# PRADUMAN-KR/Multimodal-Lip-Sync-Deepfake-Detection-System

Hardware: NVIDIA B200
Metric: windows_per_sec (higher is better)
Workload: dtype bf16

## Files before the change

multimodal-lip-sync-deepfake-detection-system_b200/csrc/bf16_path.cu:

```cuda
#include "forward_common.h"
#include "tok_front.cuh"
#include "tok_fused.cuh"
#include "token_kernels.cuh"
#include "umma_conv.cuh"
#include "stem_ring.cuh"
#include "conv_ring.cuh"

#include <cuda_fp16.h>

#include <algorithm>
#include <cstdio>
#include <cstdlib>
#include <cstring>

using namespace lsd;
using namespace lsdfw;

#define LSD_ENV(name) ([]() -> const char* { static const char* const v_ = getenv(name); return v_; }())

namespace {

uint16_t f2bf(float f) {
  uint32_t u;
  memcpy(&u, &f, 4);
  if ((u & 0x7F800000u) == 0x7F800000u) return (uint16_t)(u >> 16);
  u += 0x7FFFu + ((u >> 16) & 1u);
  return (uint16_t)(u >> 16);
}

BGroup make_group(const ConvP& c, int sh, int sw, bool merge_kt = false) {
  BGroup g;
  g.Cin = c.Cin;
  for (int a = 0; a < c.kt; ++a)
    for (int b = 0; b < c.kh; ++b)
      for (int d = 0; d < c.kw; ++d) {
        BTap t;
        t.orig = (a * c.kh + b) * c.kw + d;
        t.dt = a - c.kt / 2;
        int hp = 0, wp = 0;
        const int oh = b - c.kh / 2, ow = d - c.kw / 2;
        if (sh == 2) { hp = oh & 1; t.dh = (oh - hp) / 2; } else t.dh = oh;
        if (sw == 2) { wp = ow & 1; t.dw = (ow - wp) / 2; } else t.dw = ow;
        const int set = hp * 2 + wp;
        BBand* band = nullptr;
        for (BBand& bb : g.bands)
          if (bb.set == set && (merge_kt || bb.taps[0].dt == t.dt) && (int)bb.taps.size() < UC_MAX_TAPS) band = &bb;
        if (!band) { g.bands.push_back(BBand{set, {}}); band = &g.bands.back(); }
        band->taps.push_back(t);
      }
  g.taps_total = c.kt * c.kh * c.kw;
  g.k16 = c.Cin / 16;
  return g;
}

BGroup make_group_toeplitz(const ConvP& c, int kpix, int dw_units) {
  BGroup g;
  g.Cin = c.Cin;
  g.toeplitz = 1;
  g.k16 = kpix * 4 / 16;
  for (int a = 0; a < c.kt; ++a)
    for (int b = 0; b < c.kh; ++b) {
      BTap t;
      t.orig = a * c.kh + b;
      t.dt = a - c.kt / 2;
      const int oh = b - c.kh / 2;
      const int hp = oh & 1;
      t.dh = (oh - hp) / 2;
      t.dw = dw_units;
      BBand* band = nullptr;
      for (BBand& bb : g.bands)
        if (bb.set == hp && bb.taps[0].dt == t.dt) band = &bb;
      if (!band) { g.bands.push_back(BBand{hp, {}}); band = &g.bands.back(); }
      band->taps.push_back(t);
    }
  g.taps_total = c.kt * c.kh;
  return g;
}

struct Packer {
  lsd_handle* h;
  const std::vector<float>& f32;
  std::vector<uint16_t> w;
  std::vector<float> bias;
  int ds_sh = 2, ds_sw = 2;
  void pack_group(BGroup& g, const ConvP& c, int ntile, int part = 0) {
    g.w_off = w.size();
    const int Cout = c.Cout;
    const float* W = &f32[c.w_off];
    const float* sc = c.has_scale ? &f32[c.scale_off] : nullptr;
    g.slice_stride = (size_t)(c.Cin / 16) * g.taps_total * ntile * 16;
    for (int sl = 0; sl < Cout / ntile; ++sl)
      for (int ch = 0; ch < c.Cin / 16; ++ch)
        for (const BBand& b : g.bands)
          for (const BTap& t : b.taps)
            for (int kc = 0; kc < 2; ++kc)
              for (int nn = 0; nn < ntile; ++nn)
                for (int e = 0; e < 8; ++e) {
                  const int ci = ch * 16 + kc * 8 + e, n = sl * ntile + nn;
                  const float v = W[((size_t)t.orig * c.Cin + ci) * Cout + n] * (sc ? sc[n] : 1.0f);
                  const uint16_t hi = f2bf(v);
                  if (part == 0) w.push_back(hi);
                  else { uint32_t u = (uint32_t)hi << 16; float hf; memcpy(&hf, &u, 4); w.push_back(f2bf(v - hf)); }
                }
  }
  void add_toeplitz(const std::string& name, const std::string& key, int kpix, int dw_units, bool dup_lo = false, bool halves = false) {
    const ConvP& c = h->convs.at(key);
    BLayer L;
    L.Cout = c.Cout;
    L.ntile = c.Cout;
    L.halves = halves;
    L.groups.push_back(make_group_toeplitz(c, kpix, dw_units));
    BGroup& g = L.groups[0];
    g.w_off = w.size();
    const float* W = &f32[c.w_off];
    const float* sc = c.has_scale ? &f32[c.scale_off] : nullptr;
    const int nsl = halves ? 2 : 1, ncol = c.Cout / nsl;
    g.slice_stride = (size_t)g.k16 * g.taps_total * ncol * 16;
    for (int sl = 0; sl < nsl; ++sl)
    for (int ch = 0; ch < g.k16; ++ch)
      for (const BBand& b : g.bands)
        for (const BTap& t : b.taps)
          for (int kc = 0; kc < 2; ++kc)
            for (int n = sl * ncol; n < (sl + 1) * ncol; ++n)
              for (int e = 0; e < 8; ++e) {
                const int k = ch * 16 + kc * 8 + e, j = k / 4, kw = j - 1;
                int ci = k % 4;
                const bool lo_part = dup_lo && ci == 2;
                if (dup_lo) ci = ci < 3 ? 0 : 99;
                float v = 0.f;
                if (ci < c.Cin && kw >= 0 && kw < c.kw) v = W[((size_t)(t.orig * c.kw + kw) * c.Cin + ci) * c.Cout + n] * (sc ? sc[n] : 1.0f);
                const uint16_t hi = f2bf(v);
                if (!lo_part) w.push_back(hi);
                else { uint32_t u = (uint32_t)hi << 16; float hf; memcpy(&hf, &u, 4); w.push_back(f2bf(v - hf)); }
              }
    L.bias_off = bias.size();
    for (int i = 0; i < c.Cout; ++i) bias.push_back(f32[c.shift_off + i]);
    while (w.size() % 64) w.push_back(0);
    h->blayers[name] = L;
  }
  void add(const std::string& name, const std::string& key, int sh, int sw, const std::string& ds_key = "", int ntile = 0, bool split = false,
           bool merge_kt = false, bool halves = false) {
    const ConvP& c = h->convs.at(key);
    BLayer L;
    L.Cout = c.Cout;
    L.ntile = ntile > 0 ? ntile : c.Cout;
    L.halves = halves;
    L.groups.push_back(make_group(c, sh, sw, merge_kt));
    pack_group(L.groups[0], c, halves ? L.ntile / 2 : L.ntile);
    if (split) {
      BGroup g1 = L.groups[0]; g1.src = 2;
      BGroup g2 = make_group(c, sh, sw, merge_kt);
      pack_group(g2, c, L.ntile, 1);
      L.groups.push_back(g1);
      L.groups.push_back(g2);
    }
    L.bias_off = bias.size();
    for (int i = 0; i < c.Cout; ++i) bias.push_back(f32[c.shift_off + i]);
    if (!ds_key.empty()) {
      const ConvP& d = h->convs.at(ds_key);
      const int sh_ds = ds_sh, sw_ds = ds_sw;
      BGroup gd = make_group(d, sh_ds, sw_ds);
      gd.src = 1;
      pack_group(gd, d, L.ntile);
      L.groups.push_back(gd);
      if (split) {
        BGroup g1 = gd; g1.src = 3;
        BGroup g2 = make_group(d, sh_ds, sw_ds); g2.src = 1;
        pack_group(g2, d, L.ntile, 1);
        L.groups.push_back(g1);
        L.groups.push_back(g2);
      }
      for (int i = 0; i < c.Cout; ++i) bias[L.bias_off + i] += f32[d.shift_off + i];
    }
    while (w.size() % 64) w.push_back(0);
    h->blayers[name] = L;
  }
  void add_split(const std::string& name, const std::string& key, int ntile) {
    const ConvP& c = h->convs.at(key);
    BLayer L;
    L.Cout = c.Cout;
    L.ntile = ntile;
    BGroup g0 = make_group(c, 1, 1);
    pack_group(g0, c, ntile, 0);
    BGroup g1 = g0; g1.src = 2;
    BGroup g2 = make_group(c, 1, 1);
    pack_group(g2, c, ntile, 1);
    L.groups = {g0, g1, g2};
    L.bias_off = bias.size();
    for (int i = 0; i < c.Cout; ++i) bias.push_back(f32[c.shift_off + i]);
    while (w.size() % 64) w.push_back(0);
    h->blayers[name] = L;
  }
};

struct PBuf {
  size_t off = 0;
  int C = 0, sets = 1;
  UcGeom g;
  int64_t plane_stride = 0, set_stride = 0, origin = 0;
  size_t bytes() const { return (size_t)sets * set_stride * 2; }
};

constexpr int TILE_MAX = 1024;

PBuf make_pbuf(int C, int sets, UcGeom g) {
  PBuf b;
  b.C = C; b.sets = sets; b.g = g;
  const int64_t gf = ((int64_t)g.SL + 3 * g.RW + 16 + 7) / 8 * 8;
  const int64_t gb = gf + TILE_MAX;
  const int64_t plane_pos = (gf + g.P_total + gb + 7) / 8 * 8;
  b.origin = gf * 8;
  b.plane_stride = plane_pos * 8;
  b.set_stride = b.plane_stride * (C / 8);
  return b;
}

struct BPlan {
  Shapes s;
  Plan f32;
  std::map<std::string, PBuf> pb;
  size_t planar_begin = 0, planar_end = 0;
  UcGeom gt, g33, gta;
  void addp(const char* name, int C, int sets, UcGeom g) {
    PBuf b = make_pbuf(C, sets, g);
    f32.cursor = (f32.cursor + 255) & ~size_t(255);
    b.off = f32.cursor;
    f32.cursor += b.bytes();
    pb[name] = b;
  }
};

void build_plan(const Shapes& s, BPlan& P) {
  P.s = s;
  Plan& p = P.f32;
  const int64_t B = s.B, T = s.T, TA = s.A4;
  p.add("vid", B * T * s.H * s.W * 3);
  p.add("aud", B * s.F * s.Ta);
  p.add("v_feat", B * T * 256);
  p.add("a_feat", B * TA * 256);
  p.add("v_emb", B * T * 256);
  p.add("a_emb", B * TA * 256);
  p.add("a_int", B * T * 256);
  p.add("proj_v", B * T * 768);
  p.add("proj_a", B * T * 768);
  p.add("vcomb", B * T * 1024);
  p.add("acomb", B * T * 1024);
  p.add("a_fint", B * T * 256);
  p.add("gate_in", B * T * 512);
  p.add("gate_h", B * T * 256);
  p.add("fused", B * T * 256);
  p.add("tok", B * (T + 1) * 256);
  p.add("tok_qkv", B * (T + 1) * 768);
  p.add("comb", B * 448);
  P.planar_begin = (p.cursor + 255) & ~size_t(255);
  const int Bn = s.B, Tn = s.T;
  const UcGeom g1 = make_geom(Bn, Tn, s.H1, s.W1), g2 = make_geom(Bn, Tn, s.H2, s.W2), g3 = make_geom(Bn, Tn, s.H3, s.W3),
               g4 = make_geom(Bn, Tn, s.H4, s.W4), gd = make_geom(Bn, s.Td, s.H4, s.W4), gh = make_geom(Bn, Tn, s.Hg, s.Wg);
  const UcGeom gs = make_geom_ex(Bn, Tn, s.Hs, s.Ws, 1, 2, 0, 0, 2);
  P.addp("xs", 8, 2, gs);
  P.addp("xl", 8, 2, gs);
  P.addp("s_out", 64, 1, gs);
  P.addp("x1", 64, 1, g1);
  P.addp("l1a", 64, 1, g1);
  P.addp("y1", 64, 4, g2);
  P.addp("l2a", 128, 1, g2);
  P.addp("y2", 128, 4, g3);
  P.addp("l3a", 256, 1, g3);
  P.addp("y3", 256, 4, g4);
  P.addp("l4a", 256, 1, g4);
  P.addp("y4", 256, 1, g4);
  P.addp("art_a", 128, 1, g4);
  P.addp("art_b", 64, 1, g4);
  P.addp("delta", 256, 1, gd);
  P.addp("artd_a", 128, 1, gd);
  P.addp("artd_b", 64, 1, gd);
  P.addp("hf_f", 32, 4, gh);
  P.addp("hf_b", 64, 1, gh);
  const UcGeom as = make_geom_ex(Bn, 1, s.Fs, s.As, 0, 2, 0, 0, 4);
  auto g2d = [&](int H, int W) { return make_geom_ex(Bn, 1, H, W, 0, 1, 0, 1, 0); };
  P.addp("xa", 8, 2, as);
  for (const char* sfx : {"", "_lo"}) {
    auto nm = [&](const char* n) { return std::string(n) + sfx; };
    P.addp(nm("sa_out").c_str(), 64, 1, as);
    P.addp(nm("a1").c_str(), 64, 1, g2d(s.F1, s.A1));
    P.addp(nm("a1a").c_str(), 64, 1, g2d(s.F1, s.A1));
    P.addp(nm("ya1").c_str(), 64, 4, g2d(s.F2, s.A2));
    P.addp(nm("a2a").c_str(), 128, 1, g2d(s.F2, s.A2));
    P.addp(nm("ya2").c_str(), 128, 4, g2d(s.F3, s.A3));
    P.addp(nm("a3a").c_str(), 256, 1, g2d(s.F3, s.A3));
    P.addp(nm("ya3").c_str(), 256, 4, g2d(s.F4, s.A4));
    P.addp(nm("a4a").c_str(), 256, 1, g2d(s.F4, s.A4));
    P.addp(nm("ya4").c_str(), 256, 1, g2d(s.F4, s.A4));
  }
  P.gt = make_geom_ex(Bn, 1, 1, Tn, 0, 0, 0, 3, 0);
  P.g33 = make_geom_rows(Bn * (Tn + 1));
  P.gta = make_geom_rows(Bn * (int)TA);
  for (const char* sfx : {"", "_lo"}) {
    auto nm = [&](const char* n) { return std::string(n) + sfx; };
    P.addp(nm("afeat_p").c_str(), 256, 1, P.gta);
    for (const char* n : {"vfeat_p", "vemb_p", "aint_p", "afint_p", "att1_p", "att2_p", "blend_p", "fused_p"}) P.addp(nm(n).c_str(), 256, 1, P.gt);
    P.addp(nm("gatein_p").c_str(), 512, 1, P.gt);
    P.addp(nm("mscat_p").c_str(), 768, 1, P.gt);
    P.addp(nm("tokln_p").c_str(), 256, 1, P.g33);
    P.addp(nm("tokatt_p").c_str(), 256, 1, P.g33);
    P.addp(nm("tokff_p").c_str(), 1024, 1, P.g33);
  }
  P.planar_end = p.cursor;
}

struct BCtx {
  lsd_handle* h;
  char* ws;
  const BPlan* P;
  cudaStream_t st;
  int max_ctas = 0;
  __nv_bfloat16* base(const PBuf& b) const { return reinterpret_cast<__nv_bfloat16*>(ws + b.off); }
  __nv_bfloat16* org(const PBuf& b) const { return base(b) + b.origin; }
  float* f(const char* name) const { return reinterpret_cast<float*>(ws + P->f32.find(name)); }
  const float* W(const char* key) const { return h->warena + h->vecs.at(key); }
};

struct UArgs {
  const PBuf* in = nullptr;
  const PBuf* in_ds = nullptr;
  const PBuf* in_lo = nullptr;
  const PBuf* in_ds_lo = nullptr;
  const PBuf* res_lo = nullptr;
  const PBuf* yp_lo = nullptr;
  UcGeom og;
  int act = ACT_NONE;
  const PBuf* yp = nullptr;
  int y_plane_off = 0;
  int y_mode = -1;
  const PBuf* res = nullptr;
  float* y32 = nullptr;
  int y32_ld = 0, y32_outer_stride = -1, y32_row_off = 0;
  const float* res32 = nullptr;
  int res32_ld = 0;
};

int run_umma(const BCtx& c, const std::string& name, const UArgs& a) {
  const BLayer& L = c.h->blayers.at(name);
  const UcGeom& og = a.og;
  if (og.P_total >= ((int64_t)1 << 31) - 1024) return lsd_fail(c.h, LSD_ERR_SHAPE, "%s: more than 2^31 padded positions in one launch (reduce the batch)", name.c_str());
  UmmaConvP p;
  memset(&p, 0, sizeof(p));
  p.w = reinterpret_cast<const __nv_bfloat16*>(c.h->barena);
  p.bias = c.h->bbias + L.bias_off;
  p.Cout = L.ntile;
  const int slices = L.Cout / L.ntile;
  p.act = a.act;
  p.g = og;
  p.cta2 = L.halves ? 1 : 0;
  if (a.y_mode == UC_Y_POOL && p.cta2) return lsd_fail(c.h, LSD_ERR_UNSUPPORTED, "%s: the fused max-pool does not run on CTA pairs (LSD_UMMA_CTA2=0)", name.c_str());
  if (a.yp) {
    p.y_mode = a.y_mode >= 0 ? a.y_mode : (a.yp->sets == 4 ? UC_Y_PARITY : UC_Y_PLAIN);
    p.y = c.org(*a.yp) + (int64_t)a.y_plane_off * a.yp->plane_stride;
    p.y_plane_stride = a.yp->plane_stride; p.y_set_stride = a.yp->set_stride;
    p.g2 = a.yp->g;
    if (a.yp_lo) p.ylo = c.org(*a.yp_lo) + (int64_t)a.y_plane_off * a.yp_lo->plane_stride;
  }
  if (a.y32) {
    p.y32 = a.y32; p.y32_ld = a.y32_ld;
    p.y32_outer_stride = a.y32_outer_stride >= 0 ? a.y32_outer_stride : og.W;
    p.y32_row_off = a.y32_row_off;
  }
  if (a.res) { p.res = c.org(*a.res); p.res_plane_stride = a.res->plane_stride; }
  if (a.res_lo) p.res_lo = c.org(*a.res_lo);
  if (a.res32) { p.res32 = a.res32; p.res32_ld = a.res32_ld; }
  const int mt_cap = L.ntile <= 32 ? 8 : 4;
  const int mt2 = std::max(1, std::min(mt_cap, 256 / L.ntile));
  p.MT = std::max(1, std::min(mt_cap, 512 / L.ntile));
  const int cta_budget = (c.max_ctas > 0 && c.max_ctas < c.h->num_sms) ? c.max_ctas : c.h->num_sms;
  while (p.MT > 1 && ((og.P_total + p.MT * 128 - 1) / (p.MT * 128)) * slices < cta_budget) p.MT /= 2;
  p.nbuf = (p.MT <= mt2 && 2 * p.MT * L.ntile <= 512) ? 2 : 1;
  if (const char* e = LSD_ENV("LSD_UMMA_NBUF")) {
    const int v = atoi(e);
    if (v == 1) p.nbuf = 1;
    if (v == 2 && 2 * L.ntile <= 512) { p.nbuf = 2; p.MT = std::min(p.MT, mt2); }
  }
  p.issuers = std::min(p.MT, 4);
  if (const char* e = LSD_ENV("LSD_UMMA_ISSUERS")) { const int v = atoi(e); if (v >= 1 && v <= 4 && v <= p.MT && p.MT % v == 0 && p.MT / v <= 4) p.issuers = v; }
  uint32_t cols = 32;
  while ((int)cols < p.nbuf * p.MT * L.ntile) cols *= 2;
  p.tmem_cols = cols;
  const int S = p.MT * 128;
  int nb = 0, max_a = 0, max_taps = 0, min_k16 = 1 << 30;
  bool any_toeplitz = false;
  p.ngroups = (int)L.groups.size();
  for (int gi = 0; gi < p.ngroups; ++gi) {
    const BGroup& G = L.groups[gi];
    const PBuf* srcp = G.src == 0 ? a.in : (G.src == 1 ? a.in_ds : (G.src == 2 ? a.in_lo : a.in_ds_lo));
    if (!srcp) return lsd_fail(c.h, LSD_ERR_ARG, "%s: missing input for group %d", name.c_str(), gi);
    const PBuf& src = *srcp;
    UcGroup& ug = p.groups[gi];
    ug.band_begin = nb;
    ug.k16 = G.k16;
    ug.taps_total = G.taps_total;
    ug.w_off = (int64_t)G.w_off;
    ug.slice_stride = (int64_t)G.slice_stride;
    int tap_begin = 0;
    int wkb = 40;
    if (const char* e = LSD_ENV("LSD_UMMA_WKB")) wkb = std::max(8, atoi(e));
    const int tmax = std::max(1, std::min(UC_MAX_TAPS, (wkb * 1024) / (L.ntile * 32)));
    for (const BBand& b : G.bands) {
      const int nt = (int)b.taps.size();
      const int pieces = (nt + tmax - 1) / tmax, per = (nt + pieces - 1) / pieces;
      for (int t0 = 0; t0 < nt; t0 += per) {
        const int t1 = std::min(nt, t0 + per);
        if (nb >= UC_MAX_BANDS) return lsd_fail(c.h, LSD_ERR_UNSUPPORTED, "%s: too many bands", name.c_str());
        UcBand& ub = p.bands[nb++];
        ub.base = c.org(src) + (int64_t)b.set * src.set_stride;
        ub.plane_stride = src.plane_stride;
        ub.toeplitz = G.toeplitz;
        ub.chunk_stride = G.toeplitz ? 16 : 2 * src.plane_stride;
        int mn = INT32_MAX, mx = INT32_MIN;
        for (int j = t0; j < t1; ++j) {
          const BTap& t = b.taps[j];
          const int sft = t.dt * og.SL + t.dh * og.RW + t.dw;
          mn = std::min(mn, sft); mx = std::max(mx, sft);
        }
        ub.start = mn;
        ub.len_extra = mx - mn;
        ub.ntaps = t1 - t0;
        ub.tap_begin = tap_begin;
        for (int j = t0; j < t1; ++j) ub.rel[j - t0] = b.taps[j].dt * og.SL + b.taps[j].dh * og.RW + b.taps[j].dw - mn;
        tap_begin += ub.ntaps;
        max_a = std::max(max_a, G.toeplitz ? (S + ub.len_extra + 1 + 2 * (G.k16 - 1)) * 16 : 2 * (S + ub.len_extra) * 16);
        max_taps = std::max(max_taps, ub.ntaps);
        min_k16 = std::min(min_k16, G.k16);
        any_toeplitz = any_toeplitz || G.toeplitz;
        if (-(int64_t)ub.start * 8 > src.origin || (int64_t)mx * 8 > src.origin)
          return lsd_fail(c.h, LSD_ERR_UNSUPPORTED, "%s: guard zone too small", name.c_str());
      }
    }
    ug.band_end = nb;
  }
  p.nbands = nb;
  const int w_chunk = max_taps * (L.halves ? L.ntile / 2 : L.ntile) * 32;
  if (any_toeplitz) p.kpack = min_k16;
  else {
    bool single_band = true;
    for (int gi = 0; gi < p.ngroups; ++gi) single_band = single_band && (p.groups[gi].band_end - p.groups[gi].band_begin) == 1;
    int stage_kb = single_band ? 64 : 24;
    if (const char* e = LSD_ENV("LSD_UMMA_STAGE_KB")) stage_kb = std::max(8, atoi(e));
    p.kpack = std::max(1, std::min(std::min(8, min_k16), (stage_kb * 1024) / (max_a + w_chunk)));
  }
  p.a_stage_bytes = ((uint32_t)(any_toeplitz ? max_a : max_a * p.kpack) + 127u) & ~127u;
  p.w_stage_bytes = (uint32_t)(w_chunk * p.kpack);
  const uint32_t stage = p.a_stage_bytes + p.w_stage_bytes;
  p.nst_tile = 0;
  for (int gi = 0; gi < p.ngroups; ++gi)
    p.nst_tile += ((p.groups[gi].k16 + p.kpack - 1) / p.kpack) * (p.groups[gi].band_end - p.groups[gi].band_begin);
  const uint32_t prog_bytes = (uint32_t)p.nst_tile * (uint32_t)umma_conv_stage_desc_bytes();
  uint32_t budget = 211u * 1024u;
  if (p.y_mode == UC_Y_POOL) {
    p.pool_ring = (uint32_t)(p.MT * 128 + 128);
    uc_magic(p.pool_ring, p.pool_mR, p.pool_sR);
  }
  const uint32_t pool_bytes = (uint32_t)umma_conv_extra_smem_bytes(p);
  budget -= pool_bytes;
  if (prog_bytes + 2 * stage > budget) return lsd_fail(c.h, LSD_ERR_UNSUPPORTED, "%s: stage program of %u bytes does not fit", name.c_str(), prog_bytes);
  int stages = (int)((budget - prog_bytes) / stage);
  stages = std::max(2, std::min(stages, 8));
  if ((size_t)stages * stage + prog_bytes + pool_bytes + 1024 > 223u * 1024u) return lsd_fail(c.h, LSD_ERR_UNSUPPORTED, "%s: stage of %u bytes does not fit", name.c_str(), stage);
  p.stages = stages;
  double kflop = 0;
  for (const BGroup& G : L.groups) kflop += (double)G.taps_total * G.Cin;
  if (L.groups[0].toeplitz) { const ConvP& cp = c.h->convs.at(name); kflop = (double)cp.kt * cp.kh * cp.kw * cp.Cin; }
  if (const char* e = getenv("LSD_UMMA_SKIP")) p.skip = atoi(e);
  if (const char* why = umma_conv_config_error(p)) return lsd_fail(c.h, LSD_ERR_UNSUPPORTED, "%s: %s", name.c_str(), why);
  {
    uint64_t hkey = 1469598103934665603ull;
    static_assert(sizeof(UmmaConvP) % 8 == 0, "UmmaConvP is hashed in 8-byte words");
    const uint64_t* pw = reinterpret_cast<const uint64_t*>(&p);
    for (size_t i = 0; i < sizeof(p) / 8; ++i) { hkey ^= pw[i]; hkey *= 1099511628211ull; hkey ^= hkey >> 29; }
    auto it = c.h->prog_cache.find(hkey);
    if (it == c.h->prog_cache.end()) {
      const size_t bytes = (size_t)p.nst_tile * sizeof(UcStageDesc);
      if (!c.h->prog_arena) {
        c.h->prog_cap = 16u << 20;
        if (cudaMalloc(&c.h->prog_arena, c.h->prog_cap) != cudaSuccess) return lsd_fail(c.h, LSD_ERR_CUDA, "stage-program arena allocation failed");
        c.h->prog_cursor = 0;
      }
      if (c.h->prog_cursor + bytes > c.h->prog_cap) {
        cudaDeviceSynchronize();
        c.h->prog_cache.clear();
        c.h->prog_cursor = 0;
        ++c.h->generation;
      }
      std::vector<UcStageDesc> host((size_t)p.nst_tile);
      umma_conv_build_program(p, host.data());
      char* dst = c.h->prog_arena + c.h->prog_cursor;
      cudaError_t e = cudaMemcpy(dst, host.data(), bytes, cudaMemcpyHostToDevice);
      if (e != cudaSuccess) return lsd_fail(c.h, LSD_ERR_CUDA, "%s: stage program upload: %s", name.c_str(), cudaGetErrorString(e));
      c.h->prog_cursor += (bytes + 255) & ~size_t(255);
      it = c.h->prog_cache.emplace(hkey, dst).first;
    }
    p.prog = reinterpret_cast<const UcStageDesc*>(it->second);
  }
  static const bool dyn_tiles = LSD_ENV("LSD_UMMA_DYNAMIC") != nullptr;
  if (dyn_tiles && p.y_mode != UC_Y_POOL && !p.cta2) {
    constexpr int kMaxLayers = 512;
    if (!c.h->tile_ctr_arena) {
      if (cudaMalloc(&c.h->tile_ctr_arena, kMaxLayers * 16 * sizeof(unsigned)) != cudaSuccess ||
          cudaMemset(c.h->tile_ctr_arena, 0, kMaxLayers * 16 * sizeof(unsigned)) != cudaSuccess)
        return lsd_fail(c.h, LSD_ERR_CUDA, "tile counter allocation failed");
    }
    auto it = c.h->tile_ctr_idx.find(name);
    if (it == c.h->tile_ctr_idx.end()) {
      if ((int)c.h->tile_ctr_idx.size() >= kMaxLayers) return lsd_fail(c.h, LSD_ERR_UNSUPPORTED, "too many tcgen05 layers");
      it = c.h->tile_ctr_idx.emplace(name, (int)c.h->tile_ctr_idx.size()).first;
    }
    p.tile_ctr = c.h->tile_ctr_arena + (size_t)it->second * 16;
  }
  if (const char* e = getenv("LSD_UMMA_TRACE")) {
    static long long* dbuf = nullptr;
    if (!dbuf) cudaMalloc(&dbuf, 512);
    cudaMemsetAsync(dbuf, 0, 512, c.st);
    p.dbg = dbuf;
    launch_umma_conv(p, slices, c.st, c.h->num_sms, c.max_ctas);
    long long hv[64];
    cudaMemcpyAsync(hv, dbuf, 512, cudaMemcpyDeviceToHost, c.st);
    cudaStreamSynchronize(c.st);
    if (atoi(e) > 0)
      fprintf(stderr, "[umma] %-34s MT=%d N=%d slices=%d stages=%d kpack=%d tiles=%lld | prologue %lld, first-data %lld, mma-issued %lld, acc-done %lld, epi-done %lld, total %lld cycles\n",
              name.c_str(), p.MT, p.Cout, slices, p.stages, p.kpack, hv[7], hv[1] - hv[0], hv[2] - hv[0], hv[3] - hv[0], hv[4] - hv[0], hv[5] - hv[0], hv[6] - hv[0]);
    if (atoi(e) > 1) {
      fprintf(stderr, "        full-wait done at:");
      for (int i = 0; i < 24 && hv[8 + i]; ++i) fprintf(stderr, " %lld", hv[8 + i] - hv[0]);
      fprintf(stderr, "\n        producer issue at:");
      for (int i = 0; i < 24 && hv[32 + i]; ++i) fprintf(stderr, " %lld", hv[32 + i] - hv[0]);
      fprintf(stderr, "\n        copies issued at: ");
      for (int i = 0; i < 8 && hv[56 + i]; ++i) fprintf(stderr, " %lld", hv[56 + i] - hv[0]);
      fprintf(stderr, "\n");
    }
    return 0;
  }
  c.h->prof.begin(c.st, 2.0 * (double)og.N * og.T * og.H * og.W * L.Cout * kflop, name.rfind("visual_encoder.", 0) == 0 ? 2 : 3);
  launch_umma_conv(p, slices, c.st, c.h->num_sms, c.max_ctas);
  c.h->prof.end(c.st);
  return 0;
}

int ring_table(const BCtx& c, const UcGeom& g, bool pool, const lsd_handle::RingTab** out) {
  lsd_handle* h = c.h;
  const void* pool_to = pool ? (const void*)&g : nullptr;
  const int T = g.T, CH = (g.SL + 127) / 128;
  const int64_t G = (int64_t)g.N * CH * T;
  const int budget = (c.max_ctas > 0 && c.max_ctas < h->num_sms) ? c.max_ctas : h->num_sms;
  uint64_t key = 1469598103934665603ull;
  for (uint64_t v : {(uint64_t)g.N, (uint64_t)T, (uint64_t)g.SL, (uint64_t)g.TS, (uint64_t)g.ot, (uint64_t)budget, (uint64_t)(pool_to != nullptr)}) { key ^= v; key *= 1099511628211ull; key ^= key >> 29; }
  auto it = h->ring_tabs.find(key);
  if (it == h->ring_tabs.end()) {
    int grid = budget;
    int64_t Lr = (G + 2 * (int64_t)grid - 1) / (2 * (int64_t)grid);
    if (Lr < 8) { Lr = 8; grid = (int)((G + 2 * Lr - 1) / (2 * Lr)); }
    if (grid < 1) grid = 1;
    std::vector<std::vector<SrStep>> lists((size_t)2 * grid);
    size_t nsteps = 0;
    const int nslots = 2 * grid;
    auto add_range = [&](int sg, int64_t col, int ta, int tb) {
      const int n = (int)(col / CH), sp = (int)(col % CH);
      const int t_first = std::max(ta - 1, 0);
      for (int t_in = t_first; t_in <= tb; ++t_in) {
        SrStep st;
        st.in_pos = (int32_t)(((int64_t)n * g.TS + t_in + g.ot) * g.SL + (int64_t)sp * 128);
        const int t_out = t_in - 1;
        st.flags = SR_ACTIVE | (t_in == t_first ? SR_FIRST : 0u) | ((t_out >= ta && t_out < tb) ? SR_STORE : 0u) |
                   ((uint32_t)std::min(128, g.SL - sp * 128) << 8);
        lists[sg].push_back(st);
      }
    };
    const int64_t ncols = (int64_t)g.N * CH;
    const int64_t rounds = pool_to ? ncols / nslots : 0;
    std::vector<int> col_round((size_t)ncols, 0);
    for (int64_t r = 0; r < rounds; ++r)
      for (int sg = 0; sg < nslots; ++sg) { add_range(sg, r * nslots + sg, 0, T); col_round[(size_t)(r * nslots + sg)] = (int)r; }
    {
      const int64_t col0 = rounds * nslots, Grem = (ncols - col0) * T;
      if (pool_to) Lr = (Grem + nslots - 1) / nslots;
      for (int64_t cc = col0; cc < ncols; ++cc) col_round[(size_t)cc] = (int)rounds;
      for (int sg = 0; sg < nslots && Lr > 0; ++sg) {
        int64_t g0 = (int64_t)sg * Lr;
        const int64_t g1 = std::min(Grem, g0 + Lr);
        while (g0 < g1) {
          const int64_t col = col0 + g0 / T;
          const int ta = (int)(g0 % T), tb = (int)std::min<int64_t>(T, ta + (g1 - g0));
          add_range(sg, col, ta, tb);
          g0 += tb - ta;
        }
      }
    }
    for (int sg = 0; sg < nslots; ++sg) nsteps = std::max(nsteps, lists[sg].size());
    std::vector<SrStep> flat((size_t)2 * grid * nsteps);
    memset(flat.data(), 0, flat.size() * sizeof(SrStep));
    for (int sg = 0; sg < 2 * grid; ++sg) std::copy(lists[sg].begin(), lists[sg].end(), flat.begin() + (size_t)sg * nsteps);
    lsd_handle::RingTab tab;
    tab.nsteps = (int)nsteps; tab.grid = grid;
    if (pool_to) {
      std::vector<std::pair<int64_t, int>> order;
      for (int n = 0; n < g.N; ++n) {
        int rmax = 0;
        for (int sp = 0; sp < CH; ++sp) rmax = std::max(rmax, col_round[(size_t)n * CH + sp]);
        for (int t = 0; t < T; ++t) order.push_back({(int64_t)rmax * (T + 1) + t, n * T + t});
      }
      std::stable_sort(order.begin(), order.end(), [](const std::pair<int64_t, int>& a, const std::pair<int64_t, int>& b) { return a.first < b.first; });
      tab.nfr = (int)((order.size() + grid - 1) / grid) + 1;
      std::vector<int> fl((size_t)grid * tab.nfr, -1);
      for (size_t i = 0; i < order.size(); ++i) fl[(i % grid) * tab.nfr + i / grid] = order[i].second;
      if (cudaMalloc(&tab.frames, fl.size() * sizeof(int)) != cudaSuccess ||
          cudaMemcpy(tab.frames, fl.data(), fl.size() * sizeof(int), cudaMemcpyHostToDevice) != cudaSuccess)
        return lsd_fail(h, LSD_ERR_CUDA, "stem: pool list upload failed");
    }
    if (cudaMalloc(&tab.dev, std::max<size_t>(flat.size(), 1) * sizeof(SrStep)) != cudaSuccess ||
        cudaMemcpy(tab.dev, flat.data(), flat.size() * sizeof(SrStep), cudaMemcpyHostToDevice) != cudaSuccess)
      return lsd_fail(h, LSD_ERR_CUDA, "stem: step table upload failed");
    it = h->ring_tabs.emplace(key, tab).first;
  }
  *out = &it->second;
  return 0;
}

int run_stem_ring(const BCtx& c, const PBuf& xs, const PBuf& so, const PBuf* pool_to = nullptr) {
  lsd_handle* h = c.h;
  const UcGeom& g = xs.g;
  if (g.P_total >= ((int64_t)1 << 31) - 4096) return lsd_fail(h, LSD_ERR_SHAPE, "stem: more than 2^31 padded positions in one launch (reduce the batch)");
  const BLayer& L = h->blayers.at("visual_encoder.stem");
  StemRingP p;
  memset(&p, 0, sizeof(p));
  p.xs[0] = c.org(xs);
  p.xs[1] = c.org(xs) + xs.set_stride;
  p.w = reinterpret_cast<const __nv_bfloat16*>(h->barena) + h->stem_ring_w_off;
  p.bias = h->bbias + L.bias_off;
  p.y = c.org(so);
  p.y_plane_stride = so.plane_stride;
  p.g = g;
  p.ntap[0] = 3; p.ntap[1] = 4;
  for (int t = 0; t < 4; ++t) { p.rel[0][t] = t * g.RW; p.rel[1][t] = t * g.RW; }
  p.start[0] = -g.RW; p.start[1] = -2 * g.RW;
  p.units[0] = 128 + 2 * g.RW + 3; p.units[1] = 128 + 3 * g.RW + 3;
  if ((int64_t)(2 * g.RW + 3) * 8 > xs.origin) return lsd_fail(h, LSD_ERR_UNSUPPORTED, "stem: guard zone too small");
  const int T = g.T, CH = (g.SL + 127) / 128;
  const lsd_handle::RingTab* tab = nullptr;
  if (int trc = ring_table(c, g, pool_to != nullptr, &tab)) return trc;
  p.steps = reinterpret_cast<const SrStep*>(tab->dev);
  p.nsteps = tab->nsteps;
  p.nst = 6;
  if (const char* e = getenv("LSD_SR_SKIP")) p.skip = atoi(e);
  if (pool_to) {
    const size_t need = (size_t)g.N * T;
    if (h->ring_cnt_cap < need) {
      if (h->ring_cnt) { cudaStreamSynchronize(c.st); cudaFree(h->ring_cnt); h->ring_cnt = nullptr; ++h->generation; }
      h->ring_cnt_cap = need * 2;
      if (cudaMalloc(&h->ring_cnt, h->ring_cnt_cap * sizeof(unsigned)) != cudaSuccess) { h->ring_cnt_cap = 0; return lsd_fail(h, LSD_ERR_CUDA, "stem: frame counter allocation failed"); }
    }
    cudaMemsetAsync(h->ring_cnt, 0, need * sizeof(unsigned), c.st);
    p.frame_cnt = h->ring_cnt;
    p.pool_frames = tab->frames;
    p.pool_nfr = tab->nfr;
    p.pool_expected = 4 * CH;
    p.yp = c.org(*pool_to);
    p.yp_plane_stride = pool_to->plane_stride;
    p.gp = pool_to->g;
  }
  while (p.nst > 3 && stem_ring_smem_bytes(p) > 223u * 1024u) --p.nst;
  if (stem_ring_smem_bytes(p) > 223u * 1024u) return lsd_fail(h, LSD_ERR_UNSUPPORTED, "stem: batch too large for the ring kernel (LSD_STEM_RING=0)");
  const ConvP& cp = h->convs.at("visual_encoder.stem");
  h->prof.begin(c.st, 2.0 * (double)g.N * g.T * g.H * g.W * 64.0 * (double)cp.kt * cp.kh * cp.kw * cp.Cin, 2);
  if (getenv("LSD_SR_TRACE")) {
    static long long* dbuf = nullptr;
    constexpr int kDbg = 256 + 4 * 160;
    if (!dbuf) cudaMalloc(&dbuf, kDbg * sizeof(long long));
    cudaMemsetAsync(dbuf, 0, kDbg * sizeof(long long), c.st);
    p.dbg = dbuf;
    launch_stem_ring(p, tab->grid, c.st);
    long long hv[kDbg];
    cudaMemcpyAsync(hv, dbuf, sizeof(hv), cudaMemcpyDeviceToHost, c.st);
    cudaStreamSynchronize(c.st);
    {
      long long g0 = INT64_MAX, g1 = 0, cmin = INT64_MAX, cmax = 0, csum = 0, smax = 0;
      const int nc = std::min(tab->grid, 160);
      for (int i = 0; i < nc; ++i) g0 = std::min(g0, hv[256 + 4 * i]);
      for (int i = 0; i < nc; ++i) {
        const long long* d = hv + 256 + 4 * i;
        g1 = std::max(g1, d[1]); smax = std::max(smax, d[0] - g0);
        const long long cy = d[3] - d[2];
        cmin = std::min(cmin, cy); cmax = std::max(cmax, cy); csum += cy;
      }
      fprintf(stderr, "[sr] %d CTAs x %d steps: kernel span %.1f us (globaltimer), latest CTA start +%.1f us, CTA cycles min %lld avg %lld max %lld\n", nc,
              p.nsteps, (g1 - g0) / 1e3, smax / 1e3, cmin, csum / nc, cmax);
    }
    const long long t0 = hv[0];
    for (int k = 0; k < 32; ++k)
      fprintf(stderr, "[sr] step %2d | prod free %7lld issued %7lld | mma landed %7lld blockfree %7lld issued %7lld | epi complete %7lld back %7lld\n", k + 16,
              hv[(0 * 32 + k) * 2] - t0, hv[(0 * 32 + k) * 2 + 1] - t0, hv[(1 * 32 + k) * 2] - t0, hv[(1 * 32 + k) * 2 + 1] - t0,
              hv[(2 * 32 + k) * 2] - t0, hv[(3 * 32 + k) * 2] - t0, hv[(3 * 32 + k) * 2 + 1] - t0);
    h->prof.end(c.st);
    return 0;
  }
  launch_stem_ring(p, tab->grid, c.st);
  h->prof.end(c.st);
  return 0;
}

int run_conv_ring(const BCtx& c, const std::string& name, int which, const PBuf& x, const PBuf& y, const PBuf* res) {
  lsd_handle* h = c.h;
  const UcGeom& g = x.g;
  if (g.P_total >= ((int64_t)1 << 31) - 4096) return lsd_fail(h, LSD_ERR_SHAPE, "%s: more than 2^31 padded positions in one launch (reduce the batch)", name.c_str());
  const BLayer& L = h->blayers.at(name);
  ConvRingP p;
  memset(&p, 0, sizeof(p));
  p.x = c.org(x);
  p.x_plane_stride = x.plane_stride;
  p.w = reinterpret_cast<const __nv_bfloat16*>(h->barena) + h->l1_ring_w_off[which];
  p.bias = h->bbias + L.bias_off;
  if (res) { p.res = c.org(*res); p.res_plane_stride = res->plane_stride; }
  p.y = c.org(y);
  p.y_plane_stride = y.plane_stride; p.y_set_stride = y.set_stride;
  p.y_mode = y.sets == 4 ? UC_Y_PARITY : UC_Y_PLAIN;
  p.g = g; p.g2 = y.g;
  p.start = -(g.RW + 1);
  p.units = 128 + 2 * g.RW + 2;
  if ((int64_t)(g.RW + 1) * 8 > x.origin) return lsd_fail(h, LSD_ERR_UNSUPPORTED, "%s: guard zone too small", name.c_str());
  const lsd_handle::RingTab* tab = nullptr;
  if (int trc = ring_table(c, g, false, &tab)) return trc;
  p.steps = reinterpret_cast<const SrStep*>(tab->dev);
  p.nsteps = tab->nsteps;
  p.nst = 4;
  if (const char* e = getenv("LSD_SR_SKIP")) p.skip = atoi(e);
  while (p.nst > 1 && conv_ring_smem_bytes(p) > 223u * 1024u) --p.nst;
  if (conv_ring_smem_bytes(p) > 223u * 1024u) return lsd_fail(h, LSD_ERR_UNSUPPORTED, "%s: rows too wide / batch too large for the ring kernel (LSD_L1_RING=0)", name.c_str());
  const ConvP& cp = h->convs.at(name);
  h->prof.begin(c.st, 2.0 * (double)g.N * g.T * g.H * g.W * 64.0 * (double)cp.kt * cp.kh * cp.kw * cp.Cin, 2);
  if (getenv("LSD_CR_TRACE")) {
    static long long* dbuf = nullptr;
    if (!dbuf) cudaMalloc(&dbuf, 4 * 160 * sizeof(long long));
    cudaMemsetAsync(dbuf, 0, 4 * 160 * sizeof(long long), c.st);
    p.dbg = dbuf;
    launch_conv_ring(p, tab->grid, c.st);
    long long hv[4 * 160];
    cudaMemcpyAsync(hv, dbuf, sizeof(hv), cudaMemcpyDeviceToHost, c.st);
    cudaStreamSynchronize(c.st);
    long long g0 = INT64_MAX, g1 = 0, cmin = INT64_MAX, cmax = 0, csum = 0;
    const int nc = std::min(tab->grid, 160);
    for (int i = 0; i < nc; ++i) g0 = std::min(g0, hv[4 * i]);
    for (int i = 0; i < nc; ++i) { g1 = std::max(g1, hv[4 * i + 1]); const long long cy = hv[4 * i + 3] - hv[4 * i + 2]; cmin = std::min(cmin, cy); cmax = std::max(cmax, cy); csum += cy; }
    fprintf(stderr, "[cr] %s: %d CTAs x %d steps (nst %d): kernel span %.1f us, CTA cycles min %lld avg %lld max %lld\n", name.c_str(), nc, p.nsteps, p.nst,
            (g1 - g0) / 1e3, cmin, csum / nc, cmax);
    h->prof.end(c.st);
    return 0;
  }
  launch_conv_ring(p, tab->grid, c.st);
  h->prof.end(c.st);
  return 0;
}

#define RUN(name, ...)                            \
  do {                                            \
    UArgs a_;                                     \
    __VA_ARGS__;                                  \
    if ((rc = run_umma(b, name, a_))) return rc;  \
  } while (0)

#define RUNC(ctx, name, ...)                        \
  do {                                              \
    UArgs a_;                                       \
    __VA_ARGS__;                                    \
    if ((rc = run_umma(ctx, name, a_))) return rc;  \
  } while (0)

#define RUNS(name, ...)                            \
  do {                                             \
    UArgs a_;                                      \
    __VA_ARGS__;                                   \
    if ((rc = run_umma(bs, name, a_))) return rc;  \
  } while (0)

PlanarOut pout(const BCtx& c, const PBuf& p, const PBuf* lo = nullptr, int plane_off = 0) {
  PlanarOut o;
  o.y = c.org(p) + (int64_t)plane_off * p.plane_stride;
  o.ylo = lo ? c.org(*lo) + (int64_t)plane_off * lo->plane_stride : nullptr;
  o.plane_stride = p.plane_stride;
  if (p.g.ow > 0 && p.g.HP == 1) { o.grp = p.g.W; o.grp_stride = p.g.RW; o.off = p.g.ow; }
  else { o.grp = 0; o.grp_stride = 0; o.off = 0; }
  return o;
}

int res_stage_umma(const BCtx& b, const std::string& p, const PBuf& x, const PBuf& mid, const PBuf& y, bool has_ds, int y_mode,
                   const PBuf* x_lo = nullptr, const PBuf* mid_lo = nullptr, const PBuf* y_lo = nullptr) {
  int rc = 0;
  RUN(p + ".conv1", a_.in = &x; a_.in_lo = x_lo; a_.og = mid.g; a_.act = ACT_RELU; a_.yp = &mid; a_.yp_lo = mid_lo);
  if (has_ds) RUN(p + ".conv2", a_.in = &mid; a_.in_lo = mid_lo; a_.in_ds = &x; a_.in_ds_lo = x_lo; a_.og = mid.g; a_.act = ACT_RELU;
                  a_.yp = &y; a_.yp_lo = y_lo; a_.y_mode = y_mode);
  else RUN(p + ".conv2", a_.in = &mid; a_.in_lo = mid_lo; a_.og = mid.g; a_.act = ACT_RELU; a_.yp = &y; a_.yp_lo = y_lo; a_.y_mode = y_mode;
           a_.res = &x; a_.res_lo = x_lo);
  return 0;
}

}

static int pack_tok_fused(lsd_handle* h, const std::vector<float>& f32) {
  std::vector<TfBlock> blocks;
  tf_layer_blocks(blocks);
  std::vector<uint32_t> stage_bytes;
  for (const TfBlock& b : blocks)
    for (int k0 = 0; k0 < b.k16; k0 += b.kps) stage_bytes.push_back((uint32_t)b.kps * (uint32_t)b.N * 32u);
  std::vector<__half> w;
  std::vector<float> vec((size_t)TF_LAYERS * TF_VEC_LAYER + (size_t)(2 * TF_LAYERS + 1) * TF_D, 0.f);
  std::vector<float> cum(TF_D, 0.f);
  float* cum_out = vec.data() + (size_t)TF_LAYERS * TF_VEC_LAYER;
  for (int l = 0; l < TF_LAYERS; ++l) {
    const std::string k = "t" + std::to_string(l);
    const ConvP &cin = h->convs.at(k + ".in"), &cout = h->convs.at(k + ".out"), &cf1 = h->convs.at(k + ".ff1"), &cf2 = h->convs.at(k + ".ff2");
    const size_t w0 = w.size();
    for (const TfBlock& b : blocks) {
      const ConvP& c = b.kind == 0 ? cin : (b.kind == 1 ? cout : (b.kind == 2 ? cf1 : cf2));
      for (int k16 = 0; k16 < b.k16; ++k16)
        for (int pl = 0; pl < 2; ++pl)
          for (int n = 0; n < b.N; ++n)
            for (int e = 0; e < 8; ++e) {
              const int kk = k16 * 16 + pl * 8 + e;
              int co, ci;
              if (b.kind == 0) { co = ((n % 96) / 32) * 256 + (2 * b.idx + n / 96) * 32 + (n % 32); ci = kk; }
              else if (b.kind == 1) { co = n; ci = 64 * b.idx + kk; }
              else if (b.kind == 2) { co = 128 * b.idx + n; ci = kk; }
              else { co = n; ci = 128 * b.idx + kk; }
              w.push_back(__float2half_rn(f32[c.w_off + (size_t)ci * c.Cout + co]));
            }
    }
    if (l == 0) h->tokf_layer_bytes = (uint32_t)((w.size() - w0) * sizeof(__half));
    float* lv = vec.data() + (size_t)l * TF_VEC_LAYER;
    const char* names[4] = {".ln1.w", ".ln1.b", ".ln2.w", ".ln2.b"};
    for (int i = 0; i < 4; ++i) memcpy(lv + 256 * i, &f32[h->vecs.at(k + names[i])], 256 * sizeof(float));
    for (int n = 0; n < 768; ++n) {
      const int hp = n / 192, r = n % 192;
      lv[1024 + n] = f32[cin.shift_off + ((r % 96) / 32) * 256 + (2 * hp + r / 96) * 32 + (r % 32)];
    }
    memcpy(lv + 1024 + 768, &f32[cf1.shift_off], 1024 * sizeof(float));
    memcpy(cum_out + (size_t)(2 * l) * TF_D, cum.data(), TF_D * sizeof(float));
    for (int i = 0; i < TF_D; ++i) cum[i] += f32[cout.shift_off + i];
    memcpy(cum_out + (size_t)(2 * l + 1) * TF_D, cum.data(), TF_D * sizeof(float));
    for (int i = 0; i < TF_D; ++i) cum[i] += f32[cf2.shift_off + i];
  }
  memcpy(cum_out + (size_t)(2 * TF_LAYERS) * TF_D, cum.data(), TF_D * sizeof(float));
  h->tokf_n_stage = (int)stage_bytes.size();
  for (void* q : {(void*)h->tokf_w, (void*)h->tokf_stage_bytes, (void*)h->tokf_vec}) if (q) cudaFree(q);
  h->tokf_w = nullptr; h->tokf_stage_bytes = nullptr; h->tokf_vec = nullptr;
  cudaError_t e = cudaMalloc(&h->tokf_w, w.size() * sizeof(__half));
  if (e == cudaSuccess) e = cudaMemcpy(h->tokf_w, w.data(), w.size() * sizeof(__half), cudaMemcpyHostToDevice);
  if (e == cudaSuccess) e = cudaMalloc(&h->tokf_stage_bytes, stage_bytes.size() * sizeof(uint32_t));
  if (e == cudaSuccess) e = cudaMemcpy(h->tokf_stage_bytes, stage_bytes.data(), stage_bytes.size() * sizeof(uint32_t), cudaMemcpyHostToDevice);
  if (e == cudaSuccess) e = cudaMalloc(&h->tokf_vec, vec.size() * sizeof(float));
  if (e == cudaSuccess) e = cudaMemcpy(h->tokf_vec, vec.data(), vec.size() * sizeof(float), cudaMemcpyHostToDevice);
  if (e != cudaSuccess) return lsd_fail(h, LSD_ERR_CUDA, "pack_tok_fused: %s", cudaGetErrorString(e));
  return 0;
}

static int pack_tok_front(lsd_handle* h, const std::vector<float>& f32) {
  std::vector<__half> w;
  w.reserve((size_t)TFR_K16_TOTAL * 16 * 256);
  auto emit = [&](int k16, auto&& get) {
    for (int k = 0; k < k16; ++k)
      for (int pl = 0; pl < 2; ++pl)
        for (int n = 0; n < 256; ++n)
          for (int e = 0; e < 8; ++e) w.push_back(__float2half_rn(get(k * 16 + pl * 8 + e, n)));
  };
  const ConvP &o0 = h->convs.at("cross.v2a.out"), &o1 = h->convs.at("cross.a2v.out"), &g0 = h->convs.at("cross.gate0"),
              &fu = h->convs.at("cross.fuse"), &pp = h->convs.at("temporal.pre_scale_proj");
  for (const ConvP* o : {&o0, &o1})
    for (int hp = 0; hp < 4; ++hp) emit(4, [&](int ci, int co) { return f32[o->w_off + (size_t)(64 * hp + ci) * 256 + co]; });
  emit(32, [&](int ci, int co) { return f32[g0.w_off + (size_t)ci * 256 + co]; });
  emit(16, [&](int ci, int co) { return f32[fu.w_off + (size_t)ci * 256 + co]; });
  const int ks[3] = {3, 5, 7};
  for (int b = 0; b < 3; ++b) {
    const ConvP& c = h->convs.at("temporal.branch_k" + std::to_string(ks[b]));
    for (int j = 0; j < ks[b]; ++j)
      emit(16, [&](int ci, int co) { return f32[c.w_off + ((size_t)j * 256 + ci) * 256 + co] * (c.has_scale ? f32[c.scale_off + co] : 1.0f); });
    emit(16, [&](int ci, int co) { return f32[pp.w_off + (size_t)(256 * b + ci) * 256 + co]; });
  }
  if (w.size() != (size_t)TFR_N_STAGES * TFR_STAGE_BYTES / sizeof(__half)) return lsd_fail(h, LSD_ERR_WEIGHTS, "pack_tok_front: stream size mismatch");
  std::vector<float> vec(TFR_V_TOTAL, 0.f);
  auto cp = [&](int dst, size_t src, int n) { memcpy(vec.data() + dst, &f32[src], (size_t)n * sizeof(float)); };
  cp(TFR_V_BO0, o0.shift_off, 256); cp(TFR_V_BO1, o1.shift_off, 256); cp(TFR_V_BG0, g0.shift_off, 256);
  cp(TFR_V_WG2, h->vecs.at("cross.gate2.w"), 256); cp(TFR_V_BG2, h->vecs.at("cross.gate2.b"), 1);
  cp(TFR_V_BF, fu.shift_off, 256);
  cp(TFR_V_SH3, h->convs.at("temporal.branch_k3").shift_off, 256); cp(TFR_V_SH5, h->convs.at("temporal.branch_k5").shift_off, 256);
  cp(TFR_V_SH7, h->convs.at("temporal.branch_k7").shift_off, 256);
  cp(TFR_V_BP, pp.shift_off, 256); cp(TFR_V_CLS, h->vecs.at("temporal.cls"), 256);
  for (void* q : {(void*)h->tokfr_w, (void*)h->tokfr_vec}) if (q) cudaFree(q);
  h->tokfr_w = nullptr; h->tokfr_vec = nullptr;
  cudaError_t e = cudaMalloc(&h->tokfr_w, w.size() * sizeof(__half));
  if (e == cudaSuccess) e = cudaMemcpy(h->tokfr_w, w.data(), w.size() * sizeof(__half), cudaMemcpyHostToDevice);
  if (e == cudaSuccess) e = cudaMalloc(&h->tokfr_vec, vec.size() * sizeof(float));
  if (e == cudaSuccess) e = cudaMemcpy(h->tokfr_vec, vec.data(), vec.size() * sizeof(float), cudaMemcpyHostToDevice);
  if (e != cudaSuccess) return lsd_fail(h, LSD_ERR_CUDA, "pack_tok_front: %s", cudaGetErrorString(e));
  return 0;
}

int pack_bf16_weights(lsd_handle* h, const std::vector<float>& f32_arena) {
  Packer P{h, f32_arena, {}, {}};
  memcpy(h->lapw_host, &f32_arena[h->convs.at("art.lap").w_off], sizeof(h->lapw_host));
  h->blayers.clear();
  const int vstr[4] = {1, 2, 2, 2};
  const bool cta2 = !(LSD_ENV("LSD_UMMA_CTA2") && atoi(LSD_ENV("LSD_UMMA_CTA2")) == 0);
  for (int l = 1; l <= 4; ++l) {
    const std::string p = "visual_encoder.layer" + std::to_string(l);
    const int s = vstr[l - 1];
    int nt = l >= 3 ? 128 : 0;
    if (const char* e = getenv(l == 3 ? "LSD_UMMA_NT3" : (l == 4 ? "LSD_UMMA_NT4" : "LSD_UMMA_NTX"))) nt = atoi(e);
    const bool pairs = cta2 && l == 1;
    P.add(p + ".conv1", p + ".conv1", s, s, "", nt, false, l >= 2, pairs);
    P.ds_sh = 2; P.ds_sw = 2;
    P.add(p + ".conv2", p + ".conv2", 1, 1, l == 1 ? "" : p + ".downsample", nt, false, false, pairs);
  }
  P.add_toeplitz("visual_encoder.stem", "visual_encoder.stem", 8, 0, false, cta2);
  for (int cv = 0; cv < 2; ++cv) {
    const ConvP& c = h->convs.at(cv == 0 ? "visual_encoder.layer1.conv1" : "visual_encoder.layer1.conv2");
    h->l1_ring_w_off[cv] = 0;
    if (c.kt != 3 || c.kh != 3 || c.kw != 3 || c.Cin != 64 || c.Cout != 64) continue;
    h->l1_ring_w_off[cv] = P.w.size();
    const float* W = &f32_arena[c.w_off];
    const float* sc = c.has_scale ? &f32_arena[c.scale_off] : nullptr;
    for (int ch = 0; ch < 4; ++ch)
      for (int b = 0; b < 3; ++b)
        for (int d = 0; d < 3; ++d)
          for (int kc = 0; kc < 2; ++kc)
            for (int n = 0; n < 192; ++n)
              for (int e = 0; e < 8; ++e) {
                const int ci = ch * 16 + kc * 8 + e, a = n / 64, co = n % 64;
                P.w.push_back(f2bf(W[((size_t)((a * 3 + b) * 3 + d) * 64 + ci) * 64 + co] * (sc ? sc[co] : 1.0f)));
              }
    while (P.w.size() % 64) P.w.push_back(0);
  }
  {
    const ConvP& c = h->convs.at("visual_encoder.stem");
    h->stem_ring_w_off = 0;
    if (c.kt == 3 && c.kh == 7 && c.kw == 7 && c.Cin == 3 && c.Cout == 64) {
      h->stem_ring_w_off = P.w.size();
      const float* W = &f32_arena[c.w_off];
      const float* sc = c.has_scale ? &f32_arena[c.scale_off] : nullptr;
      for (int set = 0; set < 2; ++set)
        for (int b = 0; b < 7; ++b) {
          if (((b - 3) & 1) != set) continue;
          for (int ch = 0; ch < 2; ++ch)
            for (int kc = 0; kc < 2; ++kc)
              for (int n = 0; n < 192; ++n)
                for (int e = 0; e < 8; ++e) {
                  const int k = ch * 16 + kc * 8 + e, j = k / 4, kw = j - 1, ci = k % 4, a = n / 64, co = n % 64;
                  float v = 0.f;
                  if (ci < 3 && kw >= 0 && kw < 7) v = W[((size_t)((a * 7 + b) * 7 + kw) * 3 + ci) * 64 + co] * (sc ? sc[co] : 1.0f);
                  P.w.push_back(f2bf(v));
                }
        }
      while (P.w.size() % 64) P.w.push_back(0);
    }
  }
  P.add_toeplitz("art.hf0", "art.hf0", 4, 1);
  P.add("art.td0", "art.td0", 1, 1);
  P.add("art.td3", "art.td3", 1, 1);
  P.add("art.hf3", "art.hf3", 2, 2);
  P.add_toeplitz("audio_encoder.stem", "audio_encoder.stem", 8, 0, true);
  const int ash[4] = {1, 2, 2, 2}, asw[4] = {1, 2, 1, 1};
  for (int l = 1; l <= 4; ++l) {
    const std::string p = "audio_encoder.layer" + std::to_string(l);
    P.add(p + ".conv1", p + ".conv1", ash[l - 1], asw[l - 1], "", 0, true);
    P.ds_sh = ash[l - 1]; P.ds_sw = asw[l - 1];
    P.add(p + ".conv2", p + ".conv2", 1, 1, l == 1 ? "" : p + ".downsample", 0, true);
  }
  int wide = 128;
  if (const char* e = LSD_ENV("LSD_UMMA_NTW")) wide = atoi(e);
  int narrow = 64;
  if (const char* e = LSD_ENV("LSD_UMMA_NTN")) narrow = atoi(e);
  for (const char* k : {"projection.visual_proj", "projection.audio_proj", "cross.v2a.out", "cross.a2v.out",
                        "cross.gate0", "cross.fuse", "temporal.branch_k3", "temporal.branch_k5", "temporal.branch_k7",
                        "temporal.pre_scale_proj"})
    P.add_split(k, k, narrow);
  for (const char* k : {"cross.in_v", "cross.in_a", "cross.vcomb", "cross.acomb"}) P.add_split(k, k, wide);
  for (int l = 0; l < 4; ++l)
    for (const char* k : {".in", ".out", ".ff1", ".ff2"})
      P.add_split("t" + std::to_string(l) + k, "t" + std::to_string(l) + k, (k[1] == 'i' || (k[1] == 'f' && k[3] == '1')) ? wide : narrow);
  if (h->barena) { cudaFree(h->barena); h->barena = nullptr; }
  if (h->bbias) { cudaFree(h->bbias); h->bbias = nullptr; }
  cudaError_t e = cudaMalloc(&h->barena, P.w.size() * 2);
  if (e == cudaSuccess) e = cudaMemcpy(h->barena, P.w.data(), P.w.size() * 2, cudaMemcpyHostToDevice);
  if (e == cudaSuccess) e = cudaMalloc(&h->bbias, P.bias.size() * 4);
  if (e == cudaSuccess) e = cudaMemcpy(h->bbias, P.bias.data(), P.bias.size() * 4, cudaMemcpyHostToDevice);
  if (e != cudaSuccess) return lsd_fail(h, LSD_ERR_CUDA, "pack_bf16_weights: %s", cudaGetErrorString(e));
  if (int rc = pack_tok_fused(h, f32_arena)) return rc;
  return pack_tok_front(h, f32_arena);
}

void make_plan_bf16(lsd_handle* h, int B, int T, int H, int W, int F, int Ta, std::vector<Stage>& stages, size_t& bytes) {
  Shapes s;
  if (make_shapes(h, B, T, H, W, F, Ta, s) != 0) { bytes = 0; return; }
  BPlan P;
  build_plan(s, P);
  stages = P.f32.stages;
  bytes = P.f32.cursor;
}

struct Timeline {
  bool on = false;
  std::vector<std::pair<std::string, cudaEvent_t>> marks;
  void mark(cudaStream_t st, const char* name) {
    if (!on) return;
    cudaEvent_t e; cudaEventCreate(&e); cudaEventRecord(e, st);
    marks.emplace_back(name, e);
  }
  void dump() {
    if (!on || marks.empty()) return;
    cudaDeviceSynchronize();
    fprintf(stderr, "[timeline]");
    for (auto& m : marks) { float ms = 0; cudaEventElapsedTime(&ms, marks[0].second, m.second); fprintf(stderr, " %s=%.0f", m.first.c_str(), ms * 1000.0f); }
    fprintf(stderr, " (us)\n");
    for (auto& m : marks) cudaEventDestroy(m.second);
    marks.clear();
  }
};
static Timeline g_tl;

static int audio_encoder_bf16(const BCtx& b, const Shapes& s, bool inputs_ready, const void* audio, int adt) {
  const BPlan& P = *b.P;
  auto pbf = [&](const char* n) -> const PBuf& { return P.pb.at(n); };
  cudaStream_t st = b.st;
  int rc = 0;
  const PBuf &xa = pbf("xa"), &sao = pbf("sa_out"), &a1 = pbf("a1");
  if (inputs_ready) launch_audio_rows(b.f("aud"), LSD_F32, b.org(xa), xa.set_stride, xa.g, s.F, s.Ta, st);
  else launch_audio_rows(audio, adt, b.org(xa), xa.set_stride, xa.g, s.F, s.Ta, st);
  RUN("audio_encoder.stem", a_.in = &xa; a_.og = xa.g; a_.act = ACT_RELU; a_.yp = &sao; a_.yp_lo = &pbf("sa_out_lo"));
  launch_planar_maxpool(b.org(sao), sao.plane_stride, sao.g, b.org(a1), a1.plane_stride, a1.g, 64, st, b.org(pbf("sa_out_lo")), b.org(pbf("a1_lo")));
  if ((rc = res_stage_umma(b, "audio_encoder.layer1", a1, pbf("a1a"), pbf("ya1"), false, UC_Y_PARITY, &pbf("a1_lo"), &pbf("a1a_lo"), &pbf("ya1_lo")))) return rc;
  if ((rc = res_stage_umma(b, "audio_encoder.layer2", pbf("ya1"), pbf("a2a"), pbf("ya2"), true, UC_Y_PARITY_H, &pbf("ya1_lo"), &pbf("a2a_lo"), &pbf("ya2_lo")))) return rc;
  if ((rc = res_stage_umma(b, "audio_encoder.layer3", pbf("ya2"), pbf("a3a"), pbf("ya3"), true, UC_Y_PARITY_H, &pbf("ya2_lo"), &pbf("a3a_lo"), &pbf("ya3_lo")))) return rc;
  if ((rc = res_stage_umma(b, "audio_encoder.layer4", pbf("ya3"), pbf("a4a"), pbf("ya4"), true, UC_Y_PLAIN, &pbf("ya3_lo"), &pbf("a4a_lo"), &pbf("ya4_lo")))) return rc;
  const PBuf& ya4 = pbf("ya4");
  launch_planar_mean2(b.org(ya4), ya4.plane_stride, ya4.g, 256, b.f("a_feat"), 256, 2, pout(b, pbf("afeat_p"), &pbf("afeat_p_lo")), st,
                      b.org(pbf("ya4_lo")));
  return 0;
}

static bool token_front_enabled(int T) {
  const char* e = getenv("LSD_TOK_FRONT");
  return !(e && atoi(e) == 0) && tok_front_supported(T);
}
static int token_path_bf16(const BCtx& b, const Shapes& s, bool combined = false) {
  const BPlan& P = *b.P;
  auto pbf = [&](const char* n) -> const PBuf& { return P.pb.at(n); };
  cudaStream_t st = b.st;
  const int B = s.B, T = s.T, TA = s.A4, NT = T + 1;
  const UcGeom gt = P.gt;
  int rc = 0;
  lsd_handle* h = b.h;
  const bool par = LSD_ENV("LSD_TOK_SERIAL") == nullptr;
  if (par && !h->tok_stream[0]) {
    for (int i = 0; i < 2; ++i)
      if (cudaStreamCreateWithFlags(&h->tok_stream[i], cudaStreamNonBlocking) != cudaSuccess ||
          cudaEventCreateWithFlags(&h->ev_tok_join[i], cudaEventDisableTiming) != cudaSuccess)
        return lsd_fail(h, LSD_ERR_CUDA, "token helper stream creation failed");
    if (cudaEventCreateWithFlags(&h->ev_tok_fork, cudaEventDisableTiming) != cudaSuccess) return lsd_fail(h, LSD_ERR_CUDA, "token helper event creation failed");
  }
  BCtx b1 = b, b2 = b;
  if (par) { b1.st = h->tok_stream[0]; b2.st = h->tok_stream[1]; }
  auto fork = [&](int n) { if (par) { cudaEventRecord(h->ev_tok_fork, st); for (int i = 0; i < n; ++i) cudaStreamWaitEvent(h->tok_stream[i], h->ev_tok_fork, 0); } };
  auto join = [&](int n) { if (par) for (int i = 0; i < n; ++i) { cudaEventRecord(h->ev_tok_join[i], h->tok_stream[i]); cudaStreamWaitEvent(st, h->ev_tok_join[i], 0); } };
  float *pv = b.f("proj_v"), *pa = b.f("proj_a"), *gi = b.f("gate_in");
  if (!combined) {
    fork(1);
    launch_lerp_tokens_p(b.f("a_emb"), b.f("a_int"), B, TA, T, 256, pout(b, pbf("aint_p"), &pbf("aint_p_lo")), b1.st);
    RUNC(b1, "cross.in_a", a_.in = &pbf("aint_p"); a_.in_lo = &pbf("aint_p_lo"); a_.og = gt; a_.y32 = pa; a_.y32_ld = 768);
    RUN("cross.in_v", a_.in = &pbf("vemb_p"); a_.in_lo = &pbf("vemb_p_lo"); a_.og = gt; a_.y32 = pv; a_.y32_ld = 768);
    join(1);
  }
  g_tl.mark(st, "T:inproj");
  float* tok = b.f("tok");
  if (token_front_enabled(T)) {
    TokFrontP fp;
    memset(&fp, 0, sizeof(fp));
    if (combined) {
      fp.v_emb = b.f("vcomb"); fp.pv = fp.v_emb + 256; fp.a_int = b.f("acomb"); fp.pa = fp.a_int + 256;
      fp.ld_e = 1024; fp.ld_p = 1024;
    } else {
      fp.pv = pv; fp.pa = pa; fp.v_emb = b.f("v_emb"); fp.a_int = b.f("a_int");
      fp.ld_e = 256; fp.ld_p = 768;
    }
    fp.gi = gi; fp.fused = b.f("fused"); fp.tok = tok;
    fp.w = reinterpret_cast<const __half*>(h->tokfr_w);
    fp.vec = h->tokfr_vec;
    fp.B = B; fp.T = T;
    tok_front_geometry(T, fp.SL, fp.G, fp.KW);
    if (getenv("LSD_TOKF_TRACE")) {
      static long long* dbuf = nullptr;
      if (!dbuf) cudaMalloc(&dbuf, 256 * sizeof(long long));
      cudaMemsetAsync(dbuf, 0, 256 * sizeof(long long), st);
      fp.dbg = dbuf;
      launch_tok_front(fp, st);
      std::vector<long long> hv(256);
      cudaMemcpyAsync(hv.data(), dbuf, 256 * sizeof(long long), cudaMemcpyDeviceToHost, st);
      cudaStreamSynchronize(st);
      const long long t0 = hv[128];
      fprintf(stderr, "[tokfront] compute (start=0) then (hand-over, next arrival):");
      for (int i = 0; i < 63 && hv[128 + 2 * i + 1]; ++i) fprintf(stderr, " (%lld,%lld)", hv[128 + 2 * i + 1] - t0, hv[128 + 2 * i + 2] ? hv[128 + 2 * i + 2] - t0 : 0);
      fprintf(stderr, "\n[tokfront] mma phases (start, issue-end):");
      for (int i = 0; i < 64 && hv[2 * i + 1]; ++i) fprintf(stderr, " (%lld,%lld)", hv[2 * i] - t0, hv[2 * i + 1] - t0);
      fprintf(stderr, "\n");
      fp.dbg = nullptr;
    } else
    launch_tok_front(fp, st);
    g_tl.mark(st, "T:cross");
  } else {
  fork(1);
  launch_mha_core_p(pv, 768, pa + 256, 768, pa + 512, 768, B, T, T, 8, pout(b, pbf("att1_p"), &pbf("att1_p_lo")), st);
  RUN("cross.v2a.out", a_.in = &pbf("att1_p"); a_.in_lo = &pbf("att1_p_lo"); a_.og = gt; a_.res32 = b.f("v_emb"); a_.res32_ld = 256; a_.y32 = gi; a_.y32_ld = 512;
      a_.yp = &pbf("gatein_p"); a_.yp_lo = &pbf("gatein_p_lo"));
  launch_mha_core_p(pa, 768, pv + 256, 768, pv + 512, 768, B, T, T, 8, pout(b, pbf("att2_p"), &pbf("att2_p_lo")), b1.st);
  RUNC(b1, "cross.a2v.out", a_.in = &pbf("att2_p"); a_.in_lo = &pbf("att2_p_lo"); a_.og = gt; a_.res32 = b.f("a_int"); a_.res32_ld = 256; a_.y32 = gi + 256; a_.y32_ld = 512;
      a_.yp = &pbf("gatein_p"); a_.yp_lo = &pbf("gatein_p_lo"); a_.y_plane_off = 32);
  join(1);
  RUN("cross.gate0", a_.in = &pbf("gatein_p"); a_.in_lo = &pbf("gatein_p_lo"); a_.og = gt; a_.act = ACT_GELU; a_.y32 = b.f("gate_h"); a_.y32_ld = 256);
  launch_gate_blend_p(b.f("gate_h"), b.W("cross.gate2.w"), b.W("cross.gate2.b"), gi, 512, gi + 256, 512, B * T, 256, pout(b, pbf("blend_p"), &pbf("blend_p_lo")), st);
  RUN("cross.fuse", a_.in = &pbf("blend_p"); a_.in_lo = &pbf("blend_p_lo"); a_.og = gt; a_.act = ACT_RELU; a_.y32 = b.f("fused"); a_.y32_ld = 256; a_.yp = &pbf("fused_p"); a_.yp_lo = &pbf("fused_p_lo"));
  g_tl.mark(st, "T:cross");
  fork(2);
  RUNC(b1, "temporal.branch_k5", a_.in = &pbf("fused_p"); a_.in_lo = &pbf("fused_p_lo"); a_.og = gt; a_.act = ACT_GELU; a_.yp = &pbf("mscat_p"); a_.yp_lo = &pbf("mscat_p_lo"); a_.y_plane_off = 32);
  RUNC(b2, "temporal.branch_k3", a_.in = &pbf("fused_p"); a_.in_lo = &pbf("fused_p_lo"); a_.og = gt; a_.act = ACT_GELU; a_.yp = &pbf("mscat_p"); a_.yp_lo = &pbf("mscat_p_lo"); a_.y_plane_off = 0);
  launch_set_cls(b.W("temporal.cls"), tok, B, NT, 256, b2.st);
  RUN("temporal.branch_k7", a_.in = &pbf("fused_p"); a_.in_lo = &pbf("fused_p_lo"); a_.og = gt; a_.act = ACT_GELU; a_.yp = &pbf("mscat_p"); a_.yp_lo = &pbf("mscat_p_lo"); a_.y_plane_off = 64);
  join(2);
  RUN("temporal.pre_scale_proj", a_.in = &pbf("mscat_p"); a_.in_lo = &pbf("mscat_p_lo"); a_.og = gt; a_.res32 = b.f("fused"); a_.res32_ld = 256; a_.y32 = tok; a_.y32_ld = 256;
      a_.y32_outer_stride = NT; a_.y32_row_off = 1);
  }
  const char* fused_env = getenv("LSD_TOK_FUSED");
  const bool fused_off = fused_env && atoi(fused_env) == 0;
  if (!fused_off && tok_fused_supported(NT)) {
    TokFusedP fp;
    memset(&fp, 0, sizeof(fp));
    fp.tok = tok;
    fp.w = reinterpret_cast<const __half*>(h->tokf_w);
    fp.stage_bytes = h->tokf_stage_bytes;
    fp.n_stage_layer = h->tokf_n_stage;
    fp.layer_bytes = h->tokf_layer_bytes;
    fp.vec = h->tokf_vec;
    fp.B = B; fp.NT = NT;
    tok_fused_geometry(NT, fp.SL, fp.G, fp.KW);
    if (getenv("LSD_TOKF_TRACE")) {
      static long long* dbuf = nullptr;
      if (!dbuf) cudaMalloc(&dbuf, 384 * sizeof(long long));
      cudaMemsetAsync(dbuf, 0, 384 * sizeof(long long), st);
      fp.dbg = dbuf;
      launch_tok_fused(fp, st);
      std::vector<long long> hv(384);
      cudaMemcpyAsync(hv.data(), dbuf, 384 * sizeof(long long), cudaMemcpyDeviceToHost, st);
      cudaStreamSynchronize(st);
      const long long t0 = hv[192];
      fprintf(stderr, "[tokf] compute phases (wait-return, hand-over) cycles from start:");
      for (int i = 0; i < 96 && hv[192 + 2 * i + 1]; ++i) fprintf(stderr, " (%lld,%lld)", hv[192 + 2 * i] - t0, hv[192 + 2 * i + 1] - t0);
      fprintf(stderr, "\n[tokf] mma phases (start, issue-end):");
      for (int i = 0; i < 96 && hv[2 * i + 1]; ++i) fprintf(stderr, " (%lld,%lld)", hv[2 * i] - t0, hv[2 * i + 1] - t0);
      fprintf(stderr, "\n");
      return 0;
    }
    launch_tok_fused(fp, st);
    return 0;
  }
  const UcGeom g33 = P.g33;
  for (int l = 0; l < 4; ++l) {
    const std::string k = "t" + std::to_string(l);
    launch_layernorm_p(tok, 256, b.W((k + ".ln1.w").c_str()), b.W((k + ".ln1.b").c_str()), B * NT, 256, pout(b, pbf("tokln_p"), &pbf("tokln_p_lo")), st);
    RUN(k + ".in", a_.in = &pbf("tokln_p"); a_.in_lo = &pbf("tokln_p_lo"); a_.og = g33; a_.y32 = b.f("tok_qkv"); a_.y32_ld = 768);
    const float* qkv = b.f("tok_qkv");
    launch_mha_core_p(qkv, 768, qkv + 256, 768, qkv + 512, 768, B, NT, NT, 8, pout(b, pbf("tokatt_p"), &pbf("tokatt_p_lo")), st);
    RUN(k + ".out", a_.in = &pbf("tokatt_p"); a_.in_lo = &pbf("tokatt_p_lo"); a_.og = g33; a_.res32 = tok; a_.res32_ld = 256; a_.y32 = tok; a_.y32_ld = 256);
    launch_layernorm_p(tok, 256, b.W((k + ".ln2.w").c_str()), b.W((k + ".ln2.b").c_str()), B * NT, 256, pout(b, pbf("tokln_p"), &pbf("tokln_p_lo")), st);
    RUN(k + ".ff1", a_.in = &pbf("tokln_p"); a_.in_lo = &pbf("tokln_p_lo"); a_.og = g33; a_.act = ACT_GELU; a_.yp = &pbf("tokff_p"); a_.yp_lo = &pbf("tokff_p_lo"));
    RUN(k + ".ff2", a_.in = &pbf("tokff_p"); a_.in_lo = &pbf("tokff_p_lo"); a_.og = g33; a_.res32 = tok; a_.res32_ld = 256; a_.y32 = tok; a_.y32_ld = 256);
  }
  return 0;
}


static int ws_prepare(lsd_handle* h, const Shapes& s, const BPlan& P, char* ws, size_t ws_bytes, cudaStream_t st, int slot) {
  const int sig[6] = {s.B, s.T, s.H, s.W, s.F, s.Ta};
  WsSig& mine = h->ws_sig[slot];
  WsSig& other = h->ws_sig[slot ^ 1];
  if (other.ptr) {
    const char* o0 = reinterpret_cast<const char*>(other.ptr);
    if (o0 < ws + ws_bytes && ws < o0 + other.bytes) other.ptr = nullptr;
  }
  if (mine.ptr == ws && mine.bytes == ws_bytes && memcmp(mine.shape, sig, sizeof(sig)) == 0) return 0;
  cudaError_t e = cudaMemsetAsync(ws + P.planar_begin, 0, P.planar_end - P.planar_begin, st);
  if (e != cudaSuccess) return lsd_fail(h, LSD_ERR_CUDA, "workspace init: %s", cudaGetErrorString(e));
  mine.ptr = ws; mine.bytes = ws_bytes; memcpy(mine.shape, sig, sizeof(sig));
  return 0;
}

static int forward_bf16_impl(lsd_handle* h, const Shapes& s, float* logits, const lsd_aux* aux, char* ws, size_t ws_bytes,
                             cudaStream_t st, bool inputs_ready, const void* video, int vdt, int vlayout, const void* audio, int adt,
                             const int32_t* vstarts = nullptr, int n_frames = 0, int pipe_parity = -1) {
  BPlan P;
  build_plan(s, P);
  if (P.f32.cursor > ws_bytes) return lsd_fail(h, LSD_ERR_WORKSPACE, "workspace too small: need %zu bytes, got %zu", P.f32.cursor, ws_bytes);
  h->stages = P.f32.stages;
  h->planar_stages.clear();
  for (const auto& kv : P.pb) {
    const PBuf& b = kv.second;
    PlanarStage ps;
    ps.off = b.off; ps.C = b.C; ps.sets = b.sets; ps.plane_stride = b.plane_stride; ps.set_stride = b.set_stride; ps.origin = b.origin;
    ps.N = b.g.N; ps.T = b.g.T; ps.H = b.g.H; ps.W = b.g.W; ps.ot = b.g.ot; ps.oh = b.g.oh; ps.hp_extra = b.g.HP - b.g.H - b.g.oh;
    ps.ow = b.g.ow; ps.wp_extra = b.g.RW - b.g.W - b.g.ow;
    h->planar_stages[kv.first] = ps;
  }
  int rc0 = 0;
  if ((rc0 = ws_prepare(h, s, P, ws, ws_bytes, st, pipe_parity == 1 ? 1 : 0))) return rc0;
  BCtx b{h, ws, &P, st};
  const int B = s.B, T = s.T, TA = s.A4, NT = T + 1;
  auto& pb = P.pb;
  int rc = 0;
  if (!h->side_stream) {
    if (cudaStreamCreateWithFlags(&h->side_stream, cudaStreamNonBlocking) != cudaSuccess || cudaEventCreateWithFlags(&h->ev_fork, cudaEventDisableTiming) != cudaSuccess ||
        cudaEventCreateWithFlags(&h->ev_join, cudaEventDisableTiming) != cudaSuccess || cudaEventCreateWithFlags(&h->ev_start, cudaEventDisableTiming) != cudaSuccess ||
        cudaEventCreateWithFlags(&h->ev_audio, cudaEventDisableTiming) != cudaSuccess)
      return lsd_fail(h, LSD_ERR_CUDA, "side stream creation failed");
  }
  cudaStream_t sst = h->side_stream;
  BCtx bs{h, ws, &P, sst};
  bs.max_ctas = h->num_sms / 2;
  if (const char* e = LSD_ENV("LSD_SIDE_CTAS")) bs.max_ctas = atoi(e);
  int art_ctas = bs.max_ctas;
  if (const char* e = LSD_ENV("LSD_ART_CTAS")) art_ctas = atoi(e);
  if (const char* e = LSD_ENV("LSD_MAIN_CTAS")) { b.max_ctas = atoi(e); bs.max_ctas = h->num_sms - b.max_ctas; }
  const bool audio_early = LSD_ENV("LSD_AUDIO_LATE") == nullptr;
  const bool tcomb = token_front_enabled(T);
  auto audio_tokens = [&](const BCtx& c) -> int {
    int rc = 0;
    launch_lerp_tokens_p(c.f("a_feat"), c.f("a_fint"), B, TA, T, 256, pout(c, pb["afint_p"], &pb["afint_p_lo"]), c.st);
    RUNC(c, "cross.acomb", a_.in = &pb["afint_p"]; a_.in_lo = &pb["afint_p_lo"]; a_.og = P.gt; a_.y32 = c.f("acomb"); a_.y32_ld = 1024);
    if (aux && aux->audio_tokens) RUNC(c, "projection.audio_proj", a_.in = &pb["afeat_p"]; a_.in_lo = &pb["afeat_p_lo"]; a_.og = P.gta; a_.y32 = c.f("a_emb"); a_.y32_ld = 256);
    return 0;
  };
  g_tl.on = LSD_ENV("LSD_TIMELINE") != nullptr;
  g_tl.mark(st, "start");
  const bool audio_after_rows = LSD_ENV("LSD_AUDIO_AFTER_ROWS") && atoi(LSD_ENV("LSD_AUDIO_AFTER_ROWS")) != 0;
  if (audio_early && !audio_after_rows) {
    cudaEventRecord(h->ev_start, st);
    cudaStreamWaitEvent(sst, h->ev_start, 0);
    if ((rc = audio_encoder_bf16(bs, s, inputs_ready, audio, adt))) return rc;
    if (tcomb && (rc = audio_tokens(bs))) return rc;
    g_tl.mark(sst, "S:audio_enc");
    cudaEventRecord(h->ev_audio, sst);
  }
  const PBuf &xs = pb["xs"], &xl = pb["xl"], &so = pb["s_out"], &x1 = pb["x1"];
  const float* lapw = h->warena + h->convs.at("art.lap").w_off;
  if (vstarts) launch_video_rows(video, vdt, vlayout, lapw, h->lapw_host, b.org(xs), b.org(xl), xs.set_stride, xs.g, s.H, s.W, st, h->num_sms, vstarts, n_frames);
  else if (inputs_ready) launch_video_rows(b.f("vid"), LSD_F32, LSD_NDHWC, lapw, h->lapw_host, b.org(xs), b.org(xl), xs.set_stride, xs.g, s.H, s.W, st, h->num_sms);
  else launch_video_rows(video, vdt, vlayout, lapw, h->lapw_host, b.org(xs), b.org(xl), xs.set_stride, xs.g, s.H, s.W, st, h->num_sms);
  g_tl.mark(st, "M:video_rows");
  if (audio_early && audio_after_rows) {
    cudaEventRecord(h->ev_start, st);
    cudaStreamWaitEvent(sst, h->ev_start, 0);
    if ((rc = audio_encoder_bf16(bs, s, inputs_ready, audio, adt))) return rc;
    if (tcomb && (rc = audio_tokens(bs))) return rc;
    g_tl.mark(sst, "S:audio_enc");
    cudaEventRecord(h->ev_audio, sst);
  }
  const bool hf_early = LSD_ENV("LSD_HF_EARLY") != nullptr;
  float* comb = b.f("comb");
  PlanarOut none{nullptr, nullptr, 0, 0, 0, 0};
  const PBuf& hf = pb["hf_f"];
  if (hf_early) {
    cudaEventRecord(h->ev_fork, st);
    cudaStreamWaitEvent(sst, h->ev_fork, 0);
    RUNS("art.hf0", a_.in = &xl; a_.og = xl.g; a_.act = ACT_RELU; a_.yp = &hf);
    RUNS("art.hf3", a_.in = &hf; a_.og = hf.g; a_.act = ACT_RELU; a_.yp = &pb["hf_b"]);
    launch_planar_mean2(bs.org(pb["hf_b"]), pb["hf_b"].plane_stride, hf.g, 64, comb + 384, 448, 1, none, sst);
    g_tl.mark(sst, "S:hf3");
  }
  {
    int chunk = 0;
    if (const char* e = LSD_ENV("LSD_STEM_CHUNK")) chunk = atoi(e);
    static const bool fuse_env = LSD_ENV("LSD_STEM_POOL_FUSE") && atoi(LSD_ENV("LSD_STEM_POOL_FUSE")) != 0;
    const bool fuse_pool = fuse_env && !h->blayers.at("visual_encoder.stem").halves && !(xs.g.H & 1) && !(xs.g.W & 1) && x1.g.H * 2 == xs.g.H && x1.g.W * 2 == xs.g.W && 2 * xs.g.RW + 2 <= 128;
    static const bool ring_env = !(LSD_ENV("LSD_STEM_RING") && atoi(LSD_ENV("LSD_STEM_RING")) == 0);
    const bool ring = ring_env && h->stem_ring_w_off != 0 && !fuse_env && (chunk <= 0 || chunk >= B) && 128 + 3 * xs.g.RW + 3 <= 640;
    static const bool pool_inline = LSD_ENV("LSD_STEM_POOL_INLINE") && atoi(LSD_ENV("LSD_STEM_POOL_INLINE")) != 0;
    if (ring && pool_inline && x1.g.H * 2 == xs.g.H && x1.g.W * 2 == xs.g.W) {
      if ((rc = run_stem_ring(b, xs, so, &x1))) return rc;
      g_tl.mark(st, "M:stem");
    } else if (ring) {
      if ((rc = run_stem_ring(b, xs, so))) return rc;
      g_tl.mark(st, "M:stem");
      launch_planar_maxpool(b.org(so), so.plane_stride, so.g, b.org(x1), x1.plane_stride, x1.g, 64, st);
    } else if (fuse_pool && (chunk <= 0 || chunk >= B)) {
      RUN("visual_encoder.stem", a_.in = &xs; a_.og = xs.g; a_.act = ACT_RELU; a_.yp = &x1; a_.y_mode = UC_Y_POOL);
      g_tl.mark(st, "M:stem");
    } else if (chunk <= 0 || chunk >= B) {
      RUN("visual_encoder.stem", a_.in = &xs; a_.og = xs.g; a_.act = ACT_RELU; a_.yp = &so);
      g_tl.mark(st, "M:stem");
      launch_planar_maxpool(b.org(so), so.plane_stride, so.g, b.org(x1), x1.plane_stride, x1.g, 64, st);
    } else {
      auto view = [&](const PBuf& full, int n0, int nb) {
        PBuf v = full;
        v.g = make_geom_ex(nb, full.g.T, full.g.H, full.g.W, full.g.ot, full.g.oh, full.g.HP - full.g.H - full.g.oh, full.g.ow,
                           full.g.RW - full.g.W - full.g.ow);
        v.origin = full.origin + (int64_t)n0 * full.g.TS * full.g.SL * 8;
        return v;
      };
      for (int n0 = 0; n0 < B; n0 += chunk) {
        const int nb = std::min(chunk, B - n0);
        const PBuf xs_v = view(xs, n0, nb), so_v = view(so, n0, nb), x1_v = view(x1, n0, nb);
        RUN("visual_encoder.stem", a_.in = &xs_v; a_.og = xs_v.g; a_.act = ACT_RELU; a_.yp = &so_v);
        launch_planar_maxpool(b.org(so_v), so_v.plane_stride, so_v.g, b.org(x1_v), x1_v.plane_stride, x1_v.g, 64, st);
      }
      g_tl.mark(st, "M:stem");
    }
  }
  g_tl.mark(st, "M:maxpool");
  {
    static const bool l1_ring = LSD_ENV("LSD_L1_RING") && atoi(LSD_ENV("LSD_L1_RING")) != 0;
    if (l1_ring && h->l1_ring_w_off[0] && h->l1_ring_w_off[1] && 128 + 2 * x1.g.RW + 2 <= 512) {
      if ((rc = run_conv_ring(b, "visual_encoder.layer1.conv1", 0, x1, pb["l1a"], nullptr))) return rc;
      if ((rc = run_conv_ring(b, "visual_encoder.layer1.conv2", 1, pb["l1a"], pb["y1"], &x1))) return rc;
    } else if ((rc = res_stage_umma(b, "visual_encoder.layer1", x1, pb["l1a"], pb["y1"], false, UC_Y_PARITY))) return rc;
  }
  g_tl.mark(st, "M:layer1");
  if ((rc = res_stage_umma(b, "visual_encoder.layer2", pb["y1"], pb["l2a"], pb["y2"], true, UC_Y_PARITY))) return rc;
  g_tl.mark(st, "M:layer2");
  if ((rc = res_stage_umma(b, "visual_encoder.layer3", pb["y2"], pb["l3a"], pb["y3"], true, UC_Y_PARITY))) return rc;
  g_tl.mark(st, "M:layer3");
  if ((rc = res_stage_umma(b, "visual_encoder.layer4", pb["y3"], pb["l4a"], pb["y4"], true, UC_Y_PLAIN))) return rc;
  g_tl.mark(st, "M:layer4");
  b.max_ctas = 0;
  const PBuf& y4 = pb["y4"];
  launch_planar_mean2(b.org(y4), y4.plane_stride, y4.g, 256, b.f("v_feat"), 256, 0, pout(b, pb["vfeat_p"], &pb["vfeat_p_lo"]), st);
  cudaEventRecord(h->ev_fork, st);
  cudaStreamWaitEvent(sst, h->ev_fork, 0);
  const bool skip_art = LSD_ENV("LSD_SKIP_ART") != nullptr;
  bs.max_ctas = art_ctas;
  if (!skip_art) {
  RUNS("art.td0", a_.in = &y4; a_.og = y4.g; a_.act = ACT_RELU; a_.yp = &pb["art_a"]);
  RUNS("art.td3", a_.in = &pb["art_a"]; a_.og = y4.g; a_.act = ACT_RELU; a_.yp = &pb["art_b"]);
  launch_planar_mean2(bs.org(pb["art_b"]), pb["art_b"].plane_stride, y4.g, 64, comb + 256, 448, 1, none, sst);
  g_tl.mark(sst, "S:td_feat");
  const PBuf& dl = pb["delta"];
  if (T > 1) launch_planar_delta(bs.org(y4), y4.plane_stride, y4.g, bs.org(dl), dl.plane_stride, dl.g, 256, sst);
  RUNS("art.td0", a_.in = &dl; a_.og = dl.g; a_.act = ACT_RELU; a_.yp = &pb["artd_a"]);
  RUNS("art.td3", a_.in = &pb["artd_a"]; a_.og = dl.g; a_.act = ACT_RELU; a_.yp = &pb["artd_b"]);
  launch_planar_mean2(bs.org(pb["artd_b"]), pb["artd_b"].plane_stride, dl.g, 64, comb + 320, 448, 1, none, sst);
  g_tl.mark(sst, "S:td_delta");
  if (!hf_early) {
    const bool hf_par = LSD_ENV("LSD_HF_SERIAL") == nullptr;
    cudaStream_t hst = sst;
    if (hf_par) {
      if (!h->side2_stream) {
        if (cudaStreamCreateWithFlags(&h->side2_stream, cudaStreamNonBlocking) != cudaSuccess || cudaEventCreateWithFlags(&h->ev_join2, cudaEventDisableTiming) != cudaSuccess)
          return lsd_fail(h, LSD_ERR_CUDA, "second side stream creation failed");
      }
      hst = h->side2_stream;
      cudaStreamWaitEvent(hst, h->ev_fork, 0);
    }
    BCtx bh = bs;
    bh.st = hst;
    if (const char* e = LSD_ENV("LSD_HF_CTAS")) bh.max_ctas = atoi(e);
    RUNC(bh, "art.hf0", a_.in = &xl; a_.og = xl.g; a_.act = ACT_RELU; a_.yp = &hf);
    g_tl.mark(hst, "S:hf0");
    RUNC(bh, "art.hf3", a_.in = &hf; a_.og = hf.g; a_.act = ACT_RELU; a_.yp = &pb["hf_b"]);
    launch_planar_mean2(bh.org(pb["hf_b"]), pb["hf_b"].plane_stride, hf.g, 64, comb + 384, 448, 1, none, hst);
    g_tl.mark(hst, "S:hf3");
    if (hf_par) {
      cudaEventRecord(h->ev_join2, hst);
      cudaStreamWaitEvent(sst, h->ev_join2, 0);
    }
  }
  }
  cudaEventRecord(h->ev_join, sst);
  cudaStream_t tst = st;
  if (pipe_parity >= 0) {
    cudaEventRecord(h->ev_front[pipe_parity], st);
    cudaStreamWaitEvent(h->tail_stream, h->ev_front[pipe_parity], 0);
    tst = h->tail_stream;
  }
  {
  BCtx b{h, ws, &P, tst};
  cudaStream_t st = tst;
  if (!audio_early) { if ((rc = audio_encoder_bf16(b, s, inputs_ready, audio, adt))) return rc; }
  const UcGeom gt = P.gt;
  if (tcomb) {
    if (!audio_early) { if ((rc = audio_tokens(b))) return rc; }
    RUN("cross.vcomb", a_.in = &pb["vfeat_p"]; a_.in_lo = &pb["vfeat_p_lo"]; a_.og = gt; a_.y32 = b.f("vcomb"); a_.y32_ld = 1024);
    if (audio_early) cudaStreamWaitEvent(st, h->ev_audio, 0);
  } else {
    RUN("projection.visual_proj", a_.in = &pb["vfeat_p"]; a_.in_lo = &pb["vfeat_p_lo"]; a_.og = gt; a_.yp = &pb["vemb_p"]; a_.yp_lo = &pb["vemb_p_lo"]; a_.y32 = b.f("v_emb"); a_.y32_ld = 256);
    if (audio_early) cudaStreamWaitEvent(st, h->ev_audio, 0);
    RUN("projection.audio_proj", a_.in = &pb["afeat_p"]; a_.in_lo = &pb["afeat_p_lo"]; a_.og = P.gta; a_.y32 = b.f("a_emb"); a_.y32_ld = 256);
  }
  g_tl.mark(st, "T:proj");
  if ((rc = token_path_bf16(b, s, tcomb))) return rc;
  float* tok = b.f("tok");
  g_tl.mark(st, "T:tokens");
  cudaStreamWaitEvent(st, h->ev_join, 0);
  HeadW hw;
  auto cw = [&](const char* key) { return h->warena + h->convs.at(key).w_off; };
  auto cb = [&](const char* key) { return h->warena + h->convs.at(key).shift_off; };
  hw.w0 = cw("art.fuse0"); hw.b0 = cb("art.fuse0"); hw.w2 = cw("art.fuse2"); hw.b2 = cb("art.fuse2");
  hw.wc = cw("head.fc0"); hw.bc = cb("head.fc0");
  hw.lng = b.W("head.ln.w"); hw.lnb = b.W("head.ln.b"); hw.wo = b.W("head.out.w"); hw.bo = b.W("head.out.b");
  launch_head(tok, (int64_t)NT * 256, comb, hw, logits, B, st);
  g_tl.mark(st, "T:head");
  g_tl.dump();
  if (aux) {
    const size_t tb = (size_t)B * T * 256 * sizeof(float);
    if (aux->visual_tokens) {
      if (tcomb) launch_copy_rows(b.f("vcomb"), 1024, aux->visual_tokens, 256, B * T, 256, st);
      else cudaMemcpyAsync(aux->visual_tokens, b.f("v_emb"), tb, cudaMemcpyDeviceToDevice, st);
    }
    if (aux->audio_tokens) cudaMemcpyAsync(aux->audio_tokens, b.f("a_emb"), (size_t)B * TA * 256 * sizeof(float), cudaMemcpyDeviceToDevice, st);
    if (aux->fused_tokens) cudaMemcpyAsync(aux->fused_tokens, b.f("fused"), tb, cudaMemcpyDeviceToDevice, st);
    if (aux->cls_output) launch_copy_rows(tok, (int64_t)NT * 256, aux->cls_output, 256, B, 256, st);
  }
  if (pipe_parity >= 0) cudaEventRecord(h->ev_tail_done[pipe_parity], st);
  }
  return 0;
}

int planar_stage_read(lsd_handle* h, const char* name, const char* name_lo, const char* ws, float* out, int64_t out_elems, int Hf, int Wf,
                      cudaStream_t st) {
  auto it = h->planar_stages.find(name);
  if (it == h->planar_stages.end()) return lsd_fail(h, LSD_ERR_ARG, "unknown planar stage %s", name);
  const PlanarStage& ps = it->second;
  const PlanarStage* pl = nullptr;
  if (name_lo && *name_lo) {
    auto il = h->planar_stages.find(name_lo);
    if (il == h->planar_stages.end()) return lsd_fail(h, LSD_ERR_ARG, "unknown planar stage %s", name_lo);
    pl = &il->second;
  }
  const UcGeom g = make_geom_ex(ps.N, ps.T, ps.H, ps.W, ps.ot, ps.oh, ps.hp_extra, ps.ow, ps.wp_extra);
  if (ps.sets == 1) { Hf = ps.H; Wf = ps.W; }
  if ((int64_t)ps.N * ps.T * Hf * Wf * ps.C != out_elems) return lsd_fail(h, LSD_ERR_SHAPE, "stage %s holds %lld elements", name, (long long)ps.N * ps.T * Hf * Wf * ps.C);
  const __nv_bfloat16* x = reinterpret_cast<const __nv_bfloat16*>(ws + ps.off) + ps.origin;
  const __nv_bfloat16* xlo = pl ? reinterpret_cast<const __nv_bfloat16*>(ws + pl->off) + pl->origin : nullptr;
  launch_unpack_planar_any(x, xlo, ps.plane_stride, ps.set_stride, g, ps.C, ps.sets, Hf, Wf, out, st);
  return 0;
}

int ensure_pipeline(lsd_handle* h) {
  if (h->tail_stream) return 0;
  if (cudaStreamCreateWithFlags(&h->tail_stream, cudaStreamNonBlocking) != cudaSuccess) return lsd_fail(h, LSD_ERR_CUDA, "tail stream creation failed");
  for (int i = 0; i < 2; ++i)
    if (cudaEventCreateWithFlags(&h->ev_front[i], cudaEventDisableTiming) != cudaSuccess ||
        cudaEventCreateWithFlags(&h->ev_tail_done[i], cudaEventDisableTiming) != cudaSuccess)
      return lsd_fail(h, LSD_ERR_CUDA, "pipeline event creation failed");
  return 0;
}

static int subpath_begin(lsd_handle* h, const Shapes& s, BPlan& P, char* ws, size_t ws_bytes, cudaStream_t st) {
  build_plan(s, P);
  if (P.f32.cursor > ws_bytes) return lsd_fail(h, LSD_ERR_WORKSPACE, "workspace too small: need %zu bytes, got %zu", P.f32.cursor, ws_bytes);
  h->stages = P.f32.stages;
  if (int rc = ws_prepare(h, s, P, ws, ws_bytes, st, 0)) return rc;
  return 0;
}

size_t audio_encoder_bf16_bytes(lsd_handle* h, int B, int F, int Ta) {
  Shapes s;
  if (make_shapes(h, B, 1, 16, 16, F, Ta, s) != 0) return 0;
  BPlan P;
  build_plan(s, P);
  return P.f32.cursor + 256;
}

int audio_encoder_bf16_run(lsd_handle* h, int B, int F, int Ta, const void* audio, int adt, float* feats_out, char* ws, size_t ws_bytes,
                           cudaStream_t st) {
  Shapes s;
  int rc = make_shapes(h, B, 1, 16, 16, F, Ta, s);
  if (rc) return rc;
  BPlan P;
  if ((rc = subpath_begin(h, s, P, ws, ws_bytes, st))) return rc;
  BCtx b{h, ws, &P, st};
  if ((rc = audio_encoder_bf16(b, s, false, audio, adt))) return rc;
  cudaMemcpyAsync(feats_out, b.f("a_feat"), (size_t)B * s.A4 * 256 * sizeof(float), cudaMemcpyDeviceToDevice, st);
  return 0;
}

size_t token_path_bf16_bytes(lsd_handle* h, int B, int T, int TA) {
  Shapes s;
  if (make_shapes(h, B, T, 16, 16, 16, 8 * TA, s) != 0) return 0;
  BPlan P;
  build_plan(s, P);
  return P.f32.cursor + 256;
}

int token_path_bf16_run(lsd_handle* h, int B, int T, int TA, const float* v_emb, const float* a_emb, float* fused_out, float* cls_out,
                        char* ws, size_t ws_bytes, cudaStream_t st) {
  Shapes s;
  int rc = make_shapes(h, B, T, 16, 16, 16, 8 * TA, s);
  if (rc) return rc;
  if (s.A4 != TA) return lsd_fail(h, LSD_ERR_SHAPE, "lsd_token_path: unsupported audio token count %d", TA);
  BPlan P;
  if ((rc = subpath_begin(h, s, P, ws, ws_bytes, st))) return rc;
  BCtx b{h, ws, &P, st};
  cudaMemcpyAsync(b.f("a_emb"), a_emb, (size_t)B * TA * 256 * sizeof(float), cudaMemcpyDeviceToDevice, st);
  launch_lerp_tokens_p(v_emb, b.f("v_emb"), B, T, T, 256, pout(b, P.pb.at("vemb_p"), &P.pb.at("vemb_p_lo")), st);
  if ((rc = token_path_bf16(b, s))) return rc;
  if (fused_out) cudaMemcpyAsync(fused_out, b.f("fused"), (size_t)B * T * 256 * sizeof(float), cudaMemcpyDeviceToDevice, st);
  if (cls_out) launch_copy_rows(b.f("tok"), (int64_t)(T + 1) * 256, cls_out, 256, B, 256, st);
  return 0;
}

int forward_bf16(lsd_handle* h, int B, int T, int H, int W, int F, int Ta, const void* video, int vdt, int vlayout,
                 const void* audio, int adt, float* logits, const lsd_aux* aux, char* ws, size_t ws_bytes, cudaStream_t st,
                 bool inputs_ready) {
  Shapes s;
  int rc = make_shapes(h, B, T, H, W, F, Ta, s);
  if (rc) return rc;
  return forward_bf16_impl(h, s, logits, aux, ws, ws_bytes, st, inputs_ready, video, vdt, vlayout, audio, adt);
}

int score_batch_bf16(lsd_handle* h, const uint8_t* track, int n_frames, const int32_t* d_vstarts, const int32_t* d_astarts,
                     const float* mel_full, int Ta_full, int nb, int T, int H, int W, int F, int Ta, float* logits, char* ws,
                     size_t ws_bytes, cudaStream_t st, int pipe_parity) {
  Shapes s;
  int rc = make_shapes(h, nb, T, H, W, F, Ta, s);
  if (rc) return rc;
  BPlan P;
  build_plan(s, P);
  if (P.f32.cursor > ws_bytes) return lsd_fail(h, LSD_ERR_WORKSPACE, "workspace too small: need %zu bytes, got %zu", P.f32.cursor, ws_bytes);
  BCtx b{h, ws, &P, st};
  launch_gather_audio(mel_full, F, Ta_full, d_astarts, b.f("aud"), nb, Ta, st);
  if (video_rows_bulk_ok(track, LSD_U8, LSD_NDHWC, W))
    return forward_bf16_impl(h, s, logits, nullptr, ws, ws_bytes, st, true, track, LSD_U8, LSD_NDHWC, nullptr, 0, d_vstarts, n_frames, pipe_parity);
  launch_gather_windows_u8(track, n_frames, d_vstarts, b.f("vid"), nb, T, H * W * 3, st);
  return forward_bf16_impl(h, s, logits, nullptr, ws, ws_bytes, st, true, nullptr, 0, 0, nullptr, 0, nullptr, 0, pipe_parity);
}
```

multimodal-lip-sync-deepfake-detection-system_b200/csrc/umma_conv.cu:

```cuda
#include "umma_conv.cuh"
#include "token_kernels.cuh"

#include <algorithm>
#include <cstdio>
#include <cstdlib>
#include <cstring>

#include "lsd_kernels.h"
#include "umma.cuh"

namespace lsd {

using namespace umma;

struct F8 { float v[8]; };
__device__ __noinline__ F8 gelu8(F8 x) {
#pragma unroll
  for (int e = 0; e < 8; ++e) x.v[e] = 0.5f * x.v[e] * (1.0f + erff(x.v[e] * 0.70710678118654752f));
  return x;
}

__device__ __forceinline__ float uc_act(float v, int act) {
  if (act == ACT_RELU) return fmaxf(v, 0.0f);
  if (act == ACT_GELU) return 0.5f * v * (1.0f + erff(v * 0.70710678118654752f));
  return v;
}

__device__ __forceinline__ uint32_t uc_div(uint32_t n, uint32_t m, int s) { return (uint32_t)(((uint64_t)n * m) >> (31 + s)); }
__device__ __forceinline__ bool uc_decode(const UcGeom& g, int64_t P, int& n, int& t, int& h, int& w) {
  if (P < 0 || P >= g.P_total) return false;
  const uint32_t Pu = (uint32_t)P;
  const uint32_t S = uc_div(Pu, g.mSL, g.sSL);
  const int r = (int)(Pu - S * (uint32_t)g.SL);
  const int row = (int)uc_div((uint32_t)r, g.mRW, g.sRW), col = r - row * g.RW;
  n = (int)uc_div(S, g.mTS, g.sTS);
  t = (int)(S - (uint32_t)n * (uint32_t)g.TS) - g.ot;
  h = row - g.oh; w = col - g.ow;
  return (unsigned)t < (unsigned)g.T && (unsigned)h < (unsigned)g.H && (unsigned)w < (unsigned)g.W && n < g.N;
}

__device__ __forceinline__ int64_t uc_flat(const UcGeom& g, int n, int t, int h, int w) {
  return (((int64_t)n * g.TS + t + g.ot) * g.HP + h + g.oh) * g.RW + w + g.ow;
}

__device__ __forceinline__ uint4 pack8(const float* v) {
  uint4 o;
  __nv_bfloat162* ob = reinterpret_cast<__nv_bfloat162*>(&o);
#pragma unroll
  for (int e = 0; e < 4; ++e) ob[e] = __floats2bfloat162_rn(v[2 * e], v[2 * e + 1]);
  return o;
}
__device__ __forceinline__ uint4 pack8_relu(const float* v) {
  uint4 o;
  uint32_t* ow = reinterpret_cast<uint32_t*>(&o);
#pragma unroll
  for (int e = 0; e < 4; ++e) asm("cvt.rn.relu.bf16x2.f32 %0, %1, %2;" : "=r"(ow[e]) : "f"(v[2 * e + 1]), "f"(v[2 * e]));
  return o;
}
__device__ __forceinline__ void unpack8(const uint4& r, float* v) {
  const __nv_bfloat162* rb = reinterpret_cast<const __nv_bfloat162*>(&r);
#pragma unroll
  for (int e = 0; e < 4; ++e) { const float2 f = __bfloat1622float2(rb[e]); v[2 * e] = f.x; v[2 * e + 1] = f.y; }
}

constexpr int UC_TQ = 8;
constexpr int UC_CTR_DONE = 8;
constexpr int UC_THREADS = 512;
constexpr int UC_PROD_WARPS = 4, UC_MMA_WARP0 = 4, UC_MMA_WARPS = 4, UC_EPI_WARP0 = 8, UC_EPI_WARPS = 8;

#define UC_MMA(...) do { if constexpr (CTA2) mma2_bf16_ss_pred(__VA_ARGS__); else mma_bf16_ss_pred(__VA_ARGS__); } while (0)
#define UC_COMMIT(...) do { if constexpr (CTA2) mma2_commit_pred(__VA_ARGS__); else mma_commit_pred(__VA_ARGS__); } while (0)
template <int MODE>
__global__ void __launch_bounds__(UC_THREADS, 1) umma_conv_kernel(const __grid_constant__ UmmaConvP p) {
  constexpr bool GENERIC = MODE == 1, POOL = MODE == 2, CTA2 = MODE == 3;
  extern __shared__ __align__(1024) uint8_t smem[];
  __shared__ uint64_t full_bar[8], empty_bar[8], tfull_bar[2], tempty_bar[2];
  __shared__ uint64_t full2_bar[8], tempty2_bar[2];
  __shared__ uint64_t tq_full[UC_TQ], tq_empty[UC_TQ];
  __shared__ int tq_tile[UC_TQ];
  __shared__ uint32_t tmem_base_s;
  __shared__ __align__(16) float bias_s[256];
  const int tid = threadIdx.x, warp = tid >> 5, lane = tid & 31;
  const bool dbg = p.dbg != nullptr && blockIdx.x == 0 && blockIdx.y == 0;
  if (dbg && tid == 0) p.dbg[0] = clock64();
  const int S = p.MT * 128;
  const uint32_t stage_bytes = p.a_stage_bytes + p.w_stage_bytes;
  const int num_tiles = (int)((p.g.P_total + S - 1) / S);
  const uint32_t cta_rank = CTA2 ? cluster_ctarank() : 0u;
  const int slice = blockIdx.y, ch0 = slice * p.Cout;
  const int bcols = CTA2 ? p.Cout >> 1 : p.Cout;
  const uint32_t buf_cols = (uint32_t)(p.MT * p.Cout);
  int tile_first = blockIdx.x, tile_step = gridDim.x, tile_end = num_tiles;
  int64_t pbase = 0, emit_lo = 0, emit_hi = 0;
  if constexpr (POOL) {
    const int64_t per = (p.g.P_total + gridDim.x - 1) / gridDim.x;
    emit_lo = min((int64_t)blockIdx.x * per, p.g.P_total);
    emit_hi = min(emit_lo + per, p.g.P_total);
    pbase = max((int64_t)0, emit_lo - (2 * p.g.RW + 2));
    tile_first = 0; tile_step = 1;
    tile_end = emit_hi > emit_lo ? (int)((emit_hi - pbase + S - 1) / S) : 0;
  }
  if constexpr (CTA2) {
    tile_first = blockIdx.x >> 1; tile_step = gridDim.x >> 1; tile_end = (num_tiles + 1) >> 1;
  }
  auto tile_p0 = [&](int tile) -> int64_t {
    if constexpr (CTA2) return (int64_t)min(2 * tile + (int)cta_rank, num_tiles - 1) * S;
    return pbase + (int64_t)tile * S;
  };
  const int tile_start = tile_first < tile_end ? tile_first : -1;

  const int n_issuers = p.issuers;
  if (tid == 0) {
    for (int i = 0; i < p.stages; ++i) { mbar_init(&full_bar[i], 1); mbar_init(&empty_bar[i], n_issuers); }
    for (int i = 0; i < 2; ++i) { mbar_init(&tfull_bar[i], n_issuers); mbar_init(&tempty_bar[i], UC_EPI_WARPS); mbar_init(&tempty2_bar[i], UC_EPI_WARPS); }
    for (int i = 0; i < p.stages; ++i) mbar_init(&full2_bar[i], 1);
    for (int i = 0; i < UC_TQ; ++i) { mbar_init(&tq_full[i], 1); mbar_init(&tq_empty[i], (uint32_t)(min(UC_PROD_WARPS, p.stages) - 1 + n_issuers + UC_EPI_WARPS)); }
    fence_barrier_init();
  }
  if (warp == UC_EPI_WARP0) {
    if constexpr (CTA2) { tmem_alloc2(&tmem_base_s, p.tmem_cols); tmem_relinquish2(); }
    else { tmem_alloc(&tmem_base_s, p.tmem_cols); tmem_relinquish(); }
  }
  for (int i = tid; i < p.Cout; i += UC_THREADS) bias_s[i] = p.bias ? p.bias[ch0 + i] : 0.0f;
  uint8_t* const bias_a = smem + (size_t)p.stages * stage_bytes + (((size_t)p.nst_tile * sizeof(UcStageDesc) + 127) & ~(size_t)127);
  uint8_t* const bias_b = bias_a + 2048;
  uint8_t* const lean_end = bias_b + (size_t)bcols * 32u;
  if constexpr (!GENERIC) {
    for (int i = tid; i < 128; i += UC_THREADS) reinterpret_cast<uint4*>(bias_a)[i] = make_uint4(0x3F803F80u, 0x00003F80u, 0u, 0u);
    for (int i = tid; i < 2 * bcols; i += UC_THREADS) {
      uint4 o = make_uint4(0u, 0u, 0u, 0u);
      if (i < bcols && p.bias) {
        const float b = p.bias[ch0 + (int)cta_rank * bcols + i];
        const __nv_bfloat16 hi = __float2bfloat16_rn(b);
        const float r1 = b - __bfloat162float(hi);
        const __nv_bfloat16 mid = __float2bfloat16_rn(r1);
        const __nv_bfloat16 lo = __float2bfloat16_rn(r1 - __bfloat162float(mid));
        o.x = (uint32_t)__bfloat16_as_ushort(hi) | ((uint32_t)__bfloat16_as_ushort(mid) << 16);
        o.y = (uint32_t)__bfloat16_as_ushort(lo);
      }
      reinterpret_cast<uint4*>(bias_b)[i] = o;
    }
    fence_proxy_async_smem();
  }
  UcStageDesc* prog = reinterpret_cast<UcStageDesc*>(smem + (size_t)p.stages * stage_bytes);
  {
    const uint4* psrc = reinterpret_cast<const uint4*>(p.prog);
    uint4* pdst = reinterpret_cast<uint4*>(prog);
    for (int i = tid; i < p.nst_tile * 4; i += UC_THREADS) pdst[i] = psrc[i];
  }
  tc_fence_before();
  if constexpr (CTA2) cluster_sync_all();
  else __syncthreads();
  tc_fence_after();
  const uint32_t tmem_base = tmem_base_s;
  if (dbg && tid == 0) p.dbg[1] = clock64();
  const bool dyn = p.tile_ctr != nullptr;
  auto tq_read = [&](int seq) -> int {
    const int slot = (seq - 1) % UC_TQ;
    mbar_wait(&tq_full[slot], (uint32_t)((seq - 1) / UC_TQ) & 1u);
    const int t = *reinterpret_cast<volatile int*>(&tq_tile[slot]);
    __syncwarp();
    if (lane == 0) mbar_arrive(&tq_empty[slot]);
    return t;
  };

  if (warp < UC_PROD_WARPS) {
    const int npw = min(UC_PROD_WARPS, p.stages);
    if (warp >= npw) goto done;
    const uint32_t smem_base = smem_u32(smem);
    const uint64_t slice64 = CTA2 ? (uint64_t)cta_rank : (uint64_t)slice;
    int k = 0;
    int seq = 0;
    for (int tile = tile_start; tile >= 0; k += p.nst_tile) {
      unsigned claim = 0;
      if (dyn && warp == 0 && lane == 0) claim = atomicAdd(p.tile_ctr + slice, 1u);
      const uint64_t p0_bytes = (uint64_t)tile_p0(tile) * 16u;
      for (int si = ((warp - k) % npw + npw) % npw; si < p.nst_tile; si += npw) {
        const int kk = k + si;
        const int stage = kk % p.stages;
        const uint32_t ph = (uint32_t)(kk / p.stages) & 1u;
        const UcStageDesc& d = prog[si];
        const uint32_t counts = d.counts;
        const uint32_t n_a = counts & 0xffu, n_all = n_a + ((counts >> 8) & 0xffu);
        const bool is_a = (uint32_t)lane < n_a;
        const bool mine = (uint32_t)lane < n_all;
        const uint32_t j = is_a ? ((uint32_t)lane >> 1) : ((uint32_t)lane - n_a);
        const uint32_t sa = smem_base + (uint32_t)stage * stage_bytes;
        const uint64_t gsrc = is_a ? d.a_src + p0_bytes + (uint64_t)j * d.chunk_stride_b + (uint64_t)(lane & 1) * d.plane_stride_b
                                   : d.w_src + slice64 * d.w_slice_stride_b + (uint64_t)j * (uint64_t)d.w_src_step;
        const uint32_t dst = is_a ? sa + (uint32_t)lane * d.bytesA : sa + p.a_stage_bytes + j * d.w_dst_step;
        const uint32_t nbytes = is_a ? d.bytesA : d.w_copy_bytes;
        const uint32_t tx_bytes = d.tx_bytes;
        mbar_wait(&empty_bar[stage], ph ^ 1u);
        if (dbg && lane == 0 && tile == (int)blockIdx.x && si < 24) p.dbg[32 + si] = clock64();
        if (lane == 0) mbar_arrive_expect_tx(&full_bar[stage], tx_bytes);
        __syncwarp();
        if (mine) bulk_s2(dst, reinterpret_cast<const void*>(gsrc), nbytes, &full_bar[stage]);
        __syncwarp();
        if (dbg && lane == 0 && tile == (int)blockIdx.x && si < 8) p.dbg[56 + si] = clock64();
      }
      ++seq;
      if (!dyn) {
        tile += tile_step;
        if (tile >= tile_end) tile = -1;
      } else if (warp == 0) {
        int nt = 0;
        if (lane == 0) {
          nt = (int)gridDim.x + (int)claim;
          if (nt >= num_tiles) nt = -1;
          const int slot = (seq - 1) % UC_TQ;
          mbar_wait(&tq_empty[slot], ((uint32_t)((seq - 1) / UC_TQ) & 1u) ^ 1u);
          *reinterpret_cast<volatile int*>(&tq_tile[slot]) = nt;
          mbar_arrive(&tq_full[slot]);
        }
        tile = __shfl_sync(0xffffffffu, nt, 0);
      } else {
        tile = tq_read(seq);
      }
    }
  } else if (warp < UC_MMA_WARP0 + UC_MMA_WARPS) {
    if (warp - UC_MMA_WARP0 >= n_issuers) goto done;
    if constexpr (CTA2) {
      if (cta_rank != 0) {
        if (warp != UC_MMA_WARP0) goto done;
        int stage = 0;
        uint32_t ph = 0;
        for (int tile = tile_first; tile < tile_end; tile += tile_step)
          for (int si = 0; si < p.nst_tile; ++si) {
            mbar_wait(&full_bar[stage], ph);
            if (lane == 0) mbar_arrive_cluster(mapa_shared(smem_u32(&full2_bar[stage]), 0u));
            __syncwarp();
            if (++stage == p.stages) { stage = 0; ph ^= 1u; }
          }
        goto done;
      }
    }
    const int warp_u = __shfl_sync(0xffffffffu, warp, 0);
    const int mt_n = p.MT / n_issuers;
    const int mt_lo = (warp_u - UC_MMA_WARP0) * mt_n;
    const uint32_t idesc = idesc_bf16(CTA2 ? 256 : 128, p.Cout);
    const uint32_t smem_base = smem_u32(smem);
    const uint64_t desc_hi64 = ((uint64_t)8 << 32) | ((uint64_t)1 << 46);
    const uint32_t b_lbo = (uint32_t)bcols << 16;
    const uint32_t tap_w = (uint32_t)bcols * 2u;
    const uint32_t leader = elect_one() ? 1u : 0u;
    int stage = 0, lt = 0, dbg_it = 0;
    uint32_t ph = 0;
    for (int tile = tile_first; tile < tile_end; ++lt, tile = dyn ? (__any_sync(0xffffffffu, tq_read(lt) >= 0) ? 0 : tile_end) : tile + tile_step) {
      const int buf = p.nbuf == 2 ? (lt & 1) : 0;
      const uint32_t use = p.nbuf == 2 ? ((uint32_t)lt >> 1) : (uint32_t)lt;
      const uint32_t tb = tmem_base + (uint32_t)buf * buf_cols + (uint32_t)(mt_lo * p.Cout);
      mbar_wait(&tempty_bar[buf], (use & 1u) ^ 1u);
      if constexpr (CTA2) mbar_wait_cluster(&tempty2_bar[buf], (use & 1u) ^ 1u);
      tc_fence_after();
      uint32_t acc = 0;
      if constexpr (!GENERIC) {
        const uint64_t da = desc_hi64 | (uint64_t)(smem_u32(bias_a) >> 4);
        const uint64_t db = desc_hi64 | (uint64_t)((smem_u32(bias_b) >> 4) | b_lbo);
        UC_MMA(tb, da, db, idesc, 0u, leader);
        if (mt_n > 1) UC_MMA(tb + (uint32_t)p.Cout, da, db, idesc, 0u, leader);
        if (mt_n > 2) {
          UC_MMA(tb + 2u * (uint32_t)p.Cout, da, db, idesc, 0u, leader);
          UC_MMA(tb + 3u * (uint32_t)p.Cout, da, db, idesc, 0u, leader);
        }
        acc = 1u;
      }
      for (int gi = 0; gi < p.ngroups; ++gi) {
        const int k16 = p.groups[gi].k16, b0 = p.groups[gi].band_begin, b1 = p.groups[gi].band_end;
        for (int c0 = 0; c0 < k16; c0 += p.kpack) {
          const int nc = min(p.kpack, k16 - c0);
          for (int b = b0; b < b1; ++b) {
            const UcBand& bd = p.bands[b];
            const int ntaps = bd.ntaps;
            const uint32_t unitsA = (uint32_t)(S + bd.len_extra);
            const uint32_t a_lbo = (bd.toeplitz ? 1u : unitsA) << 16;
            const uint32_t a_chunk = bd.toeplitz ? 2u : 2u * unitsA;
            const uint32_t w_chunk = (uint32_t)ntaps * tap_w;
            mbar_wait(&full_bar[stage], ph);
            if constexpr (CTA2) mbar_wait_cluster(&full2_bar[stage], ph);
            tc_fence_after();
            if (dbg && warp == UC_MMA_WARP0 && lane == 0 && acc == 0 && lt == 0) p.dbg[2] = clock64();
            if (dbg && warp == UC_MMA_WARP0 && lane == 0 && lt == 0 && dbg_it < 24) p.dbg[8 + dbg_it++] = clock64();
            const uint32_t sa = ((smem_base + (uint32_t)stage * stage_bytes) >> 4) + (uint32_t)mt_lo * 128u;
            const uint32_t sw = ((smem_base + (uint32_t)stage * stage_bytes + p.a_stage_bytes) >> 4) | b_lbo;
            if (ntaps == 1) {
              uint32_t at = (sa | a_lbo) + (uint32_t)bd.rel[0], wj = sw;
#pragma unroll 1
              for (int j = 0; j < nc; ++j, at += a_chunk, wj += w_chunk) {
                const uint64_t da = desc_hi64 | (uint64_t)at, db = desc_hi64 | (uint64_t)wj;
                UC_MMA(tb, da, db, idesc, acc, leader);
                if (mt_n > 1) UC_MMA(tb + (uint32_t)p.Cout, da + 128u, db, idesc, acc, leader);
                acc = 1u;
              }
            } else
            for (int j = 0; j < nc; ++j) {
              const uint32_t aj = (sa + (uint32_t)j * a_chunk) | a_lbo;
              uint32_t wj = sw + (uint32_t)j * w_chunk;
#pragma unroll 1
              for (int tp = 0; tp < ntaps; ++tp) {
                const uint32_t at = aj + (uint32_t)bd.rel[tp];
                const uint64_t da = desc_hi64 | (uint64_t)at, db = desc_hi64 | (uint64_t)wj;
                UC_MMA(tb, da, db, idesc, acc, leader);
                if (mt_n > 1) UC_MMA(tb + (uint32_t)p.Cout, da + 128u, db, idesc, acc, leader);
                if (mt_n > 2) {
                  UC_MMA(tb + 2u * (uint32_t)p.Cout, da + 256u, db, idesc, acc, leader);
                  UC_MMA(tb + 3u * (uint32_t)p.Cout, da + 384u, db, idesc, acc, leader);
                }
                acc = 1u;
                wj += tap_w;
              }
            }
            UC_COMMIT(&empty_bar[stage], leader);
            if (++stage == p.stages) { stage = 0; ph ^= 1u; }
          }
        }
      }
      UC_COMMIT(&tfull_bar[buf], leader);
      if (dbg && warp == UC_MMA_WARP0 && lane == 0 && lt == 0) p.dbg[3] = clock64();
    }
  } else {
    const int quarter = warp & 3;
    const int half = (warp - UC_EPI_WARP0) >> 2;
    const float act_lo = p.act == ACT_RELU ? 0.0f : -INFINITY;
    const int rowt = quarter * 32 + lane;
    int lt = 0;
    uint8_t* const ring = lean_end;
    int2* const pool_dst = reinterpret_cast<int2*>(ring + (size_t)p.pool_ring * 128u);
    for (int tile = tile_start; tile >= 0; ++lt, tile = dyn ? tq_read(lt) : (tile + tile_step < tile_end ? tile + tile_step : -1)) {
      const int buf = p.nbuf == 2 ? (lt & 1) : 0;
      const uint32_t use = p.nbuf == 2 ? ((uint32_t)lt >> 1) : (uint32_t)lt;
      const uint32_t tb = tmem_base + (uint32_t)buf * buf_cols + ((uint32_t)(quarter * 32) << 16);
      const int64_t P0 = tile_p0(tile);
      mbar_wait(&tfull_bar[buf], use & 1u);
      tc_fence_after();
      if (dbg && warp == UC_EPI_WARP0 && lane == 0 && lt == 0) p.dbg[4] = clock64();
      const bool split_m = !GENERIC && p.MT >= 2;
      const bool split_c = !split_m && (GENERIC || (p.Cout & 63) == 0);
      const int m_end = (!split_m && (!split_c || POOL) && half == 1) ? 0 : p.MT;
      for (int m = split_m ? half : 0; m < m_end; m += split_m ? 2 : 1) {
        const int64_t P = P0 + (int64_t)m * 128 + rowt;
        int n = 0, t = 0, h = 0, w = 0;
        const bool valid = (p.skip & 8) ? true : uc_decode(p.g, P, n, t, h, w);
        const bool inrange = P < p.g.P_total;
        const int64_t outer = valid ? ((int64_t)n * p.g.T + t) * p.g.H + h : 0;
        int64_t dst = P * 8;
        if (valid && p.y_mode == UC_Y_PARITY)
          dst = (int64_t)((h & 1) * 2 + (w & 1)) * p.y_set_stride + uc_flat(p.g2, n, t, h >> 1, w >> 1) * 8;
        else if (valid && p.y_mode == UC_Y_PARITY_H)
          dst = (int64_t)((h & 1) * 2) * p.y_set_stride + uc_flat(p.g2, n, t, h >> 1, w) * 8;
        const bool store_planar = ((p.y_mode == UC_Y_PLAIN && inrange) || (p.y_mode >= UC_Y_PARITY && valid)) && !(p.skip & 4);
        const int cbeg = split_c ? half * (p.Cout >> 1) : 0, cend = split_c ? cbeg + (p.Cout >> 1) : p.Cout;
        if constexpr (POOL) {
          const uint32_t rel = (uint32_t)(P - pbase);
          const uint32_t slot = rel - uc_div(rel, p.pool_mR, p.pool_sR) * p.pool_ring;
          const bool emit = valid && (h & 1) && (w & 1) && P >= emit_lo && P < emit_hi;
          pool_dst[m * 128 + rowt] = make_int2(emit ? (int)uc_flat(p.g2, n, t, h >> 1, w >> 1) : -1, (int)slot);
          uint8_t* const rrow = ring + (size_t)slot * 128u;
          const uint32_t sw = slot & 7u;
          const uint32_t vmask = valid ? 0xffffffffu : 0u;
          uint32_t ta = tb + (uint32_t)(m * p.Cout);
#pragma unroll 1
          for (int c = 0; c < 64; c += 32, ta += 32) {
            float v[32];
            tmem_ld32(ta, v);
            tmem_ld_wait();
#pragma unroll
            for (int q = 0; q < 4; ++q) {
              uint4 o = pack8_relu(v + 8 * q);
              o.x &= vmask; o.y &= vmask; o.z &= vmask; o.w &= vmask;
              if (!(p.skip & 32)) *reinterpret_cast<uint4*>(rrow + ((((uint32_t)(c >> 3) + q) ^ sw) << 4)) = o;
            }
          }
        } else if constexpr (!GENERIC) {
          char* yp = reinterpret_cast<char*>(p.y + (int64_t)((ch0 + cbeg) >> 3) * p.y_plane_stride + dst);
          const char* rp = reinterpret_cast<const char*>(p.res + (int64_t)((ch0 + cbeg) >> 3) * p.res_plane_stride + P * 8);
          const int64_t yps = p.y_plane_stride * 2, rps = p.res_plane_stride * 2;
          const bool has_res = p.res != nullptr;
          const bool relu = p.act == ACT_RELU;
          const uint32_t vmask = valid ? 0xffffffffu : 0u;
          uint32_t ta = tb + (uint32_t)(m * p.Cout + cbeg);
#pragma unroll 1
          for (int c = cbeg; c < cend; c += 32, yp += 4 * yps, rp += 4 * rps, ta += 32) {
            float v[32];
            uint4 rr[4];
            tmem_ld32(ta, v);
            if (has_res) {
#pragma unroll
              for (int q = 0; q < 4; ++q) rr[q] = valid ? *reinterpret_cast<const uint4*>(rp + q * rps) : make_uint4(0, 0, 0, 0);
            }
            tmem_ld_wait();
            if (has_res) {
#pragma unroll
              for (int q = 0; q < 4; ++q) {
                float f[8];
                unpack8(rr[q], f);
#pragma unroll
                for (int e = 0; e < 8; ++e) v[8 * q + e] += f[e];
              }
            }
            if (store_planar) {
#pragma unroll
              for (int q = 0; q < 4; ++q) {
                uint4 o = relu ? pack8_relu(v + 8 * q) : pack8(v + 8 * q);
                o.x &= vmask; o.y &= vmask; o.z &= vmask; o.w &= vmask;
                *reinterpret_cast<uint4*>(yp + q * yps) = o;
              }
            }
          }
        } else {
        const float* r32row = p.res32 ? p.res32 + (outer * p.g.W + w) * p.res32_ld + ch0 : nullptr;
        float* y32row = p.y32 ? p.y32 + (outer * p.y32_outer_stride + w + p.y32_row_off) * p.y32_ld + ch0 : nullptr;
        const bool use_res = valid && p.res != nullptr, use_lo = use_res && p.res_lo != nullptr, use_r32 = valid && p.res32 != nullptr;
#pragma unroll 1
        for (int c0 = cbeg; c0 < cend; c0 += 32) {
          float v[32];
          uint4 pre[8];
          tmem_ld32(tb + (uint32_t)(m * p.Cout + c0), v);
          if (use_res) {
            const int64_t roff = (int64_t)((ch0 + c0) >> 3) * p.res_plane_stride + P * 8;
#pragma unroll
            for (int q = 0; q < 4; ++q) pre[q] = *reinterpret_cast<const uint4*>(p.res + roff + (int64_t)q * p.res_plane_stride);
            if (use_lo) {
#pragma unroll
              for (int q = 0; q < 4; ++q) pre[4 + q] = *reinterpret_cast<const uint4*>(p.res_lo + roff + (int64_t)q * p.res_plane_stride);
            }
          } else if (use_r32) {
#pragma unroll
            for (int q = 0; q < 8; ++q) pre[q] = *reinterpret_cast<const uint4*>(r32row + c0 + 4 * q);
          }
          tmem_ld_wait();
#pragma unroll
          for (int q = 0; q < 4; ++q) {
            const int c = c0 + 8 * q;
            F8 x;
#pragma unroll
            for (int e = 0; e < 8; ++e) x.v[e] = v[8 * q + e];
            if (valid) {
              const float4 b0 = *reinterpret_cast<const float4*>(&bias_s[c]);
              const float4 b1 = *reinterpret_cast<const float4*>(&bias_s[c + 4]);
              x.v[0] += b0.x; x.v[1] += b0.y; x.v[2] += b0.z; x.v[3] += b0.w; x.v[4] += b1.x; x.v[5] += b1.y; x.v[6] += b1.z; x.v[7] += b1.w;
              if (use_res) {
                float f[8];
                unpack8(pre[q], f);
#pragma unroll
                for (int e = 0; e < 8; ++e) x.v[e] += f[e];
                if (use_lo) {
                  unpack8(pre[4 + q], f);
#pragma unroll
                  for (int e = 0; e < 8; ++e) x.v[e] += f[e];
                }
              } else if (use_r32) {
                const uint4 q0 = pre[2 * q], q1 = pre[2 * q + 1];
                x.v[0] += __uint_as_float(q0.x); x.v[1] += __uint_as_float(q0.y); x.v[2] += __uint_as_float(q0.z); x.v[3] += __uint_as_float(q0.w);
                x.v[4] += __uint_as_float(q1.x); x.v[5] += __uint_as_float(q1.y); x.v[6] += __uint_as_float(q1.z); x.v[7] += __uint_as_float(q1.w);
              }
              if (p.act == ACT_GELU) {
                x = gelu8(x);
              } else {
#pragma unroll
                for (int e = 0; e < 8; ++e) x.v[e] = fmaxf(x.v[e], act_lo);
              }
              if (y32row) {
                float4* o = reinterpret_cast<float4*>(y32row + c);
                o[0] = make_float4(x.v[0], x.v[1], x.v[2], x.v[3]);
                o[1] = make_float4(x.v[4], x.v[5], x.v[6], x.v[7]);
              }
            } else {
#pragma unroll
              for (int e = 0; e < 8; ++e) x.v[e] = 0.0f;
            }
            if (store_planar) {
              const uint4 hi4 = pack8(x.v);
              const int64_t off = (int64_t)((ch0 + c) >> 3) * p.y_plane_stride + dst;
              *reinterpret_cast<uint4*>(p.y + off) = hi4;
              if (p.ylo) {
                float hf[8];
                unpack8(hi4, hf);
#pragma unroll
                for (int e = 0; e < 8; ++e) hf[e] = x.v[e] - hf[e];
                *reinterpret_cast<uint4*>(p.ylo + off) = pack8(hf);
              }
            }
          }
        }
        }
      }
      tc_fence_before();
      __syncwarp();
      if (lane == 0) {
        if (CTA2 && cta_rank != 0) mbar_arrive_cluster(mapa_shared(smem_u32(&tempty2_bar[buf]), 0u));
        else mbar_arrive(&tempty_bar[buf]);
      }
      if constexpr (POOL) {
        asm volatile("bar.sync 1, 256;" ::: "memory");
        const int etid = tid - UC_EPI_WARP0 * 32;
        const int RW = p.g.RW, R = (int)p.pool_ring, sS = 31 - __clz(S);
        for (int idx = etid; idx < ((p.skip & 16) ? 0 : S * 8); idx += UC_EPI_WARPS * 32) {
          const int pos = idx & (S - 1), q = idx >> sS;
          const int2 d = pool_dst[pos];
          if (d.x < 0) continue;
          __nv_bfloat162 mx[4];
#pragma unroll
          for (int e = 0; e < 4; ++e) mx[e] = __floats2bfloat162_rn(0.0f, 0.0f);
#pragma unroll
          for (int a = 0; a < 3; ++a)
#pragma unroll
            for (int bb = 0; bb < 3; ++bb) {
              int sn = d.y - a * RW - bb;
              sn += sn < 0 ? R : 0;
              const uint4 r = *reinterpret_cast<const uint4*>(ring + (size_t)sn * 128u + (((uint32_t)q ^ ((uint32_t)sn & 7u)) << 4));
              const __nv_bfloat162* rb = reinterpret_cast<const __nv_bfloat162*>(&r);
#pragma unroll
              for (int e = 0; e < 4; ++e) mx[e] = __hmax2(mx[e], rb[e]);
            }
          *reinterpret_cast<uint4*>(p.y + (int64_t)((ch0 >> 3) + q) * p.y_plane_stride + (int64_t)d.x * 8) = *reinterpret_cast<const uint4*>(mx);
        }
        asm volatile("bar.sync 1, 256;" ::: "memory");
      }
      if (dbg && warp == UC_EPI_WARP0 && lane == 0 && lt == 0) p.dbg[5] = clock64();
    }
  }
done:
  tc_fence_before();
  if constexpr (CTA2) cluster_sync_all();
  else __syncthreads();
  if (warp == UC_EPI_WARP0) {
    if constexpr (CTA2) tmem_dealloc2(tmem_base, p.tmem_cols);
    else tmem_dealloc(tmem_base, p.tmem_cols);
  }
  if (dyn && tid == 0) {
    __threadfence();
    const unsigned n_ctas = gridDim.x * gridDim.y;
    if (atomicAdd(p.tile_ctr + UC_CTR_DONE, 1u) == n_ctas - 1) {
      for (unsigned y = 0; y < gridDim.y; ++y) p.tile_ctr[y] = 0;
      p.tile_ctr[UC_CTR_DONE] = 0;
      __threadfence();
    }
  }
  if (dbg && tid == 0) { p.dbg[6] = clock64(); p.dbg[7] = num_tiles; }
}

void umma_conv_build_program(const UmmaConvP& p, UcStageDesc* out) {
  const int S = p.MT * 128;
  const int bcols = p.cta2 ? p.Cout / 2 : p.Cout;
  int s = 0;
  for (int gi = 0; gi < p.ngroups; ++gi) {
    const UcGroup& g = p.groups[gi];
    for (int c0 = 0; c0 < g.k16; c0 += p.kpack) {
      const int nc = std::min(p.kpack, g.k16 - c0);
      for (int b = g.band_begin; b < g.band_end; ++b, ++s) {
        const UcBand& bd = p.bands[b];
        UcStageDesc d;
        const uint32_t bytesW = (uint32_t)bd.ntaps * (uint32_t)bcols * 32u;
        d.bytesA = bd.toeplitz ? (uint32_t)(S + bd.len_extra + 1 + 2 * (nc - 1)) * 16u : (uint32_t)(S + bd.len_extra) * 16u;
        uint32_t n_a = bd.toeplitz ? 1u : 2u * (uint32_t)nc;
        const bool w_merged = (g.band_end - g.band_begin) == 1;
        uint32_t n_w = w_merged ? 1u : (uint32_t)nc;
        d.w_copy_bytes = w_merged ? (uint32_t)nc * bytesW : bytesW;
        d.w_dst_step = bytesW;
        if (p.skip & 1) n_a = 0;
        if (p.skip & 2) n_w = 0;
        d.tx_bytes = n_a * d.bytesA + (n_w ? (uint32_t)nc * bytesW : 0u);
        d.a_src = reinterpret_cast<uint64_t>(bd.base + (int64_t)c0 * bd.chunk_stride + (int64_t)bd.start * 8);
        d.chunk_stride_b = (uint64_t)bd.chunk_stride * 2u;
        d.plane_stride_b = (uint64_t)bd.plane_stride * 2u;
        d.w_src = reinterpret_cast<uint64_t>(p.w + g.w_off + ((int64_t)c0 * g.taps_total + bd.tap_begin) * (int64_t)bcols * 16);
        d.w_slice_stride_b = (uint64_t)g.slice_stride * 2u;
        d.w_src_step = (uint32_t)g.taps_total * (uint32_t)bcols * 32u;
        d.counts = n_a | (n_w << 8) | ((uint32_t)b << 16) | ((uint32_t)nc << 24);
        out[s] = d;
      }
    }
  }
}

size_t umma_conv_smem_bytes(const UmmaConvP& p) {
  size_t b = (size_t)p.stages * (p.a_stage_bytes + p.w_stage_bytes) + (size_t)p.nst_tile * sizeof(UcStageDesc) + 1024;
  return b + umma_conv_extra_smem_bytes(p);
}
int umma_conv_stage_desc_bytes() { return (int)sizeof(UcStageDesc); }
size_t umma_conv_pool_smem_bytes(int MT) { return (size_t)(MT * 128 + 128) * 128u + (size_t)MT * 128 * sizeof(int2); }
static bool uc_is_generic(const UmmaConvP& p);
size_t umma_conv_extra_smem_bytes(const UmmaConvP& p) {
  if (uc_is_generic(p)) return 0;
  size_t b = 128 + 2048 + (size_t)(p.cta2 ? p.Cout / 2 : p.Cout) * 32u;
  if (p.y_mode == UC_Y_POOL) b += 128 + umma_conv_pool_smem_bytes(p.MT);
  return b;
}

static bool uc_is_generic(const UmmaConvP& p) {
  return p.y32 || p.res32 || p.ylo || p.res_lo || p.act == ACT_GELU || p.y_mode == UC_Y_NONE || (p.Cout & 31);
}
const char* umma_conv_config_error(const UmmaConvP& p) {
  if (2 * p.kpack + p.kpack > 32) return "K chunks per stage exceed the producer lanes";
  if (p.res && p.res32) return "bf16 and fp32 residuals are mutually exclusive";
  if (uc_is_generic(p) && (p.Cout & 63)) return "the generic epilogue needs a column slice that is a multiple of 64";
  if (p.MT / p.issuers > 4 || p.MT % p.issuers) return "unsupported M-tiles per issuing warp";
  if (p.cta2 && (uc_is_generic(p) || p.y_mode == UC_Y_POOL || (p.Cout & 31) || p.tile_ctr)) return "CTA pairs need the lean epilogue, a multiple of 32 columns and the static tile walk";
  if (p.y_mode == UC_Y_POOL) {
    if (uc_is_generic(p) || p.res || p.act != ACT_RELU || p.Cout != 64 || p.tile_ctr) return "fused max-pool needs the lean epilogue, ReLU, 64 columns and the static tile walk";
    if ((p.g.H & 1) || (p.g.W & 1) || p.g2.H * 2 != p.g.H || p.g2.W * 2 != p.g.W || 2 * p.g.RW + 2 > 128) return "fused max-pool: unsupported geometry";
    if (p.pool_ring != (uint32_t)(p.MT * 128 + 128) || (p.MT & (p.MT - 1))) return "fused max-pool: ring size mismatch";
  }
  return nullptr;
}

cudaError_t umma_conv_device_init() {
  cudaError_t e = cudaFuncSetAttribute(umma_conv_kernel<0>, cudaFuncAttributeMaxDynamicSharedMemorySize, 223 * 1024);
  if (e == cudaSuccess) e = cudaFuncSetAttribute(umma_conv_kernel<1>, cudaFuncAttributeMaxDynamicSharedMemorySize, 223 * 1024);
  if (e == cudaSuccess) e = cudaFuncSetAttribute(umma_conv_kernel<2>, cudaFuncAttributeMaxDynamicSharedMemorySize, 223 * 1024);
  if (e == cudaSuccess) e = cudaFuncSetAttribute(umma_conv_kernel<3>, cudaFuncAttributeMaxDynamicSharedMemorySize, 223 * 1024);
  if (e == cudaSuccess) e = video_rows_device_init();
  return e;
}

void launch_umma_conv(const UmmaConvP& p, int n_slices, cudaStream_t s, int num_sms, int max_ctas) {
  if (const char* why = umma_conv_config_error(p)) { fprintf(stderr, "umma_conv: %s\n", why); abort(); }
  const int S = p.MT * 128;
  const int tiles = (int)((p.g.P_total + S - 1) / S);
  const int budget = (max_ctas > 0 && max_ctas < num_sms) ? max_ctas : num_sms;
  int gx = (budget + n_slices - 1) / n_slices;
  gx = gx < 1 ? 1 : (gx > tiles ? tiles : gx);
  const bool generic = uc_is_generic(p);
  if (p.cta2) {
    if (n_slices != 1) { fprintf(stderr, "umma_conv: CTA pairs take one column slice\n"); abort(); }
    const int pairs = (tiles + 1) / 2;
    int gp = budget / 2;
    gp = gp < 1 ? 1 : (gp > pairs ? pairs : gp);
    cudaLaunchConfig_t cfg = {};
    cfg.gridDim = dim3(2 * gp, 1, 1);
    cfg.blockDim = dim3(UC_THREADS, 1, 1);
    cfg.dynamicSmemBytes = umma_conv_smem_bytes(p);
    cfg.stream = s;
    cudaLaunchAttribute at[1];
    at[0].id = cudaLaunchAttributeClusterDimension;
    at[0].val.clusterDim.x = 2; at[0].val.clusterDim.y = 1; at[0].val.clusterDim.z = 1;
    cfg.attrs = at; cfg.numAttrs = 1;
    cudaLaunchKernelEx(&cfg, umma_conv_kernel<3>, p);
    count_launch();
    return;
  }
  if (generic) umma_conv_kernel<1><<<dim3(gx, n_slices), UC_THREADS, umma_conv_smem_bytes(p), s>>>(p);
  else if (p.y_mode == UC_Y_POOL) umma_conv_kernel<2><<<dim3(gx, n_slices), UC_THREADS, umma_conv_smem_bytes(p), s>>>(p);
  else umma_conv_kernel<0><<<dim3(gx, n_slices), UC_THREADS, umma_conv_smem_bytes(p), s>>>(p);
  count_launch();
}

__global__ void pack_planar_kernel(const float* __restrict__ x, __nv_bfloat16* __restrict__ y, int64_t plane_stride, int64_t set_stride,
                                   UcGeom g, UcGeom g2, int C, int parity, int64_t total) {
  const int64_t i = (int64_t)blockIdx.x * blockDim.x + threadIdx.x;
  if (i >= total) return;
  const int64_t npos = (int64_t)g.N * g.T * g.H * g.W;
  const int chunk = (int)(i / npos);
  int64_t r = i - (int64_t)chunk * npos;
  const int w = (int)(r % g.W); r /= g.W;
  const int h = (int)(r % g.H); r /= g.H;
  const int t = (int)(r % g.T);
  const int n = (int)(r / g.T);
  const float* src = x + ((((int64_t)n * g.T + t) * g.H + h) * g.W + w) * C + chunk * 8;
  float v[8];
#pragma unroll
  for (int e = 0; e < 8; ++e) v[e] = src[e];
  int64_t dst;
  if (parity) dst = (int64_t)((h & 1) * 2 + (w & 1)) * set_stride + uc_flat(g2, n, t, h >> 1, w >> 1) * 8;
  else dst = uc_flat(g, n, t, h, w) * 8;
  *reinterpret_cast<uint4*>(y + (int64_t)chunk * plane_stride + dst) = pack8(v);
}
void launch_pack_planar(const float* x, __nv_bfloat16* y, int64_t plane_stride, int64_t set_stride, UcGeom g, UcGeom g2, int C,
                        int parity, cudaStream_t s) {
  const int64_t total = (int64_t)g.N * g.T * g.H * g.W * (C / 8);
  if (total == 0) return;
  pack_planar_kernel<<<(unsigned)((total + 255) / 256), 256, 0, s>>>(x, y, plane_stride, set_stride, g, g2, C, parity, total);
  count_launch();
}

__global__ void unpack_planar_kernel(const __nv_bfloat16* __restrict__ x, int64_t plane_stride, UcGeom g, int C, float* __restrict__ y,
                                     int ld, int64_t total) {
  const int64_t i = (int64_t)blockIdx.x * blockDim.x + threadIdx.x;
  if (i >= total) return;
  const int nch = C / 8;
  const int chunk = (int)(i % nch);
  int64_t r = i / nch;
  const int64_t row = r;
  const int w = (int)(r % g.W); r /= g.W;
  const int h = (int)(r % g.H); r /= g.H;
  const int t = (int)(r % g.T);
  const int n = (int)(r / g.T);
  const uint4 v = *reinterpret_cast<const uint4*>(x + (int64_t)chunk * plane_stride + uc_flat(g, n, t, h, w) * 8);
  float f[8];
  unpack8(v, f);
  float4* o = reinterpret_cast<float4*>(y + row * ld + chunk * 8);
  o[0] = make_float4(f[0], f[1], f[2], f[3]);
  o[1] = make_float4(f[4], f[5], f[6], f[7]);
}
void launch_unpack_planar(const __nv_bfloat16* x, int64_t plane_stride, UcGeom g, int C, float* y, int ld, cudaStream_t s) {
  const int64_t total = (int64_t)g.N * g.T * g.H * g.W * (C / 8);
  if (total == 0) return;
  unpack_planar_kernel<<<(unsigned)((total + 255) / 256), 256, 0, s>>>(x, plane_stride, g, C, y, ld, total);
  count_launch();
}

__global__ void unpack_planar_any_kernel(const __nv_bfloat16* __restrict__ x, const __nv_bfloat16* __restrict__ xlo, int64_t plane_stride,
                                         int64_t set_stride, UcGeom g, int C, int sets, int Hf, int Wf, float* __restrict__ y, int64_t total) {
  const int64_t i = (int64_t)blockIdx.x * blockDim.x + threadIdx.x;
  if (i >= total) return;
  const int nch = C / 8;
  const int chunk = (int)(i % nch);
  int64_t r = i / nch;
  const int64_t row = r;
  const int w = (int)(r % Wf); r /= Wf;
  const int h = (int)(r % Hf); r /= Hf;
  const int t = (int)(r % g.T);
  const int n = (int)(r / g.T);
  int64_t src;
  if (sets == 1) src = uc_flat(g, n, t, h, w) * 8;
  else if (Wf == g.W) src = (int64_t)((h & 1) * 2) * set_stride + uc_flat(g, n, t, h >> 1, w) * 8;
  else src = (int64_t)((h & 1) * 2 + (w & 1)) * set_stride + uc_flat(g, n, t, h >> 1, w >> 1) * 8;
  src += (int64_t)chunk * plane_stride;
  float f[8];
  unpack8(*reinterpret_cast<const uint4*>(x + src), f);
  if (xlo) {
    float fl[8];
    unpack8(*reinterpret_cast<const uint4*>(xlo + src), fl);
#pragma unroll
    for (int e = 0; e < 8; ++e) f[e] += fl[e];
  }
  float4* o = reinterpret_cast<float4*>(y + row * C + chunk * 8);
  o[0] = make_float4(f[0], f[1], f[2], f[3]);
  o[1] = make_float4(f[4], f[5], f[6], f[7]);
}
void launch_unpack_planar_any(const __nv_bfloat16* x, const __nv_bfloat16* xlo, int64_t plane_stride, int64_t set_stride, UcGeom g, int C, int sets,
                              int Hf, int Wf, float* y, cudaStream_t s) {
  const int64_t total = (int64_t)g.N * g.T * Hf * Wf * (C / 8);
  if (total == 0) return;
  unpack_planar_any_kernel<<<(unsigned)((total + 255) / 256), 256, 0, s>>>(x, xlo, plane_stride, set_stride, g, C, sets, Hf, Wf, y, total);
  count_launch();
}

__global__ void planar_mean_kernel(const __nv_bfloat16* __restrict__ x, int64_t plane_stride, UcGeom g, float* __restrict__ y, int ld,
                                   int per_window) {
  __shared__ float part[256][9];
  const int row = blockIdx.x, chunk = blockIdx.y, tid = threadIdx.x;
  const int count = per_window ? g.T * g.H * g.W : g.H * g.W;
  const int n = per_window ? row : row / g.T;
  const int t0 = per_window ? 0 : row % g.T;
  float acc[8] = {0, 0, 0, 0, 0, 0, 0, 0};
  for (int i = tid; i < count; i += blockDim.x) {
    const int w = i % g.W;
    const int r = i / g.W;
    const int h = r % g.H;
    const int t = t0 + r / g.H;
    const uint4 v = *reinterpret_cast<const uint4*>(x + (int64_t)chunk * plane_stride + uc_flat(g, n, t, h, w) * 8);
    float f[8];
    unpack8(v, f);
#pragma unroll
    for (int e = 0; e < 8; ++e) acc[e] += f[e];
  }
#pragma unroll
  for (int e = 0; e < 8; ++e) part[tid][e] = acc[e];
  __syncthreads();
  for (int sft = blockDim.x >> 1; sft > 0; sft >>= 1) {
    if (tid < sft) {
#pragma unroll
      for (int e = 0; e < 8; ++e) part[tid][e] += part[tid + sft][e];
    }
    __syncthreads();
  }
  if (tid < 8) y[(int64_t)row * ld + chunk * 8 + tid] = part[0][tid] / (float)count;
}
void launch_planar_mean(const __nv_bfloat16* x, int64_t plane_stride, UcGeom g, int C, float* y, int ld, int per_window, cudaStream_t s) {
  const int rows = per_window ? g.N : g.N * g.T;
  if (rows == 0) return;
  const int count = per_window ? g.T * g.H * g.W : g.H * g.W;
  int threads = 32;
  while (threads < 256 && threads < count) threads <<= 1;
  planar_mean_kernel<<<dim3(rows, C / 8), threads, 0, s>>>(x, plane_stride, g, y, ld, per_window);
  count_launch();
}

__global__ void planar_delta_kernel(const __nv_bfloat16* __restrict__ x, int64_t xs, UcGeom g, __nv_bfloat16* __restrict__ d, int64_t ds,
                                    UcGeom gd, int64_t total) {
  const int64_t i = (int64_t)blockIdx.x * blockDim.x + threadIdx.x;
  if (i >= total) return;
  const int64_t npos = (int64_t)gd.N * gd.T * gd.H * gd.W;
  const int chunk = (int)(i / npos);
  int64_t r = i - (int64_t)chunk * npos;
  const int w = (int)(r % gd.W); r /= gd.W;
  const int h = (int)(r % gd.H); r /= gd.H;
  const int t = (int)(r % gd.T);
  const int n = (int)(r / gd.T);
  float a[8], b[8], o[8];
  unpack8(*reinterpret_cast<const uint4*>(x + (int64_t)chunk * xs + uc_flat(g, n, t + 1, h, w) * 8), a);
  unpack8(*reinterpret_cast<const uint4*>(x + (int64_t)chunk * xs + uc_flat(g, n, t, h, w) * 8), b);
#pragma unroll
  for (int e = 0; e < 8; ++e) o[e] = a[e] - b[e];
  *reinterpret_cast<uint4*>(d + (int64_t)chunk * ds + uc_flat(gd, n, t, h, w) * 8) = pack8(o);
}
void launch_planar_delta(const __nv_bfloat16* x, int64_t x_plane_stride, UcGeom g, __nv_bfloat16* d, int64_t d_plane_stride, UcGeom gd,
                         int C, cudaStream_t s) {
  const int64_t total = (int64_t)gd.N * gd.T * gd.H * gd.W * (C / 8);
  if (total == 0) return;
  planar_delta_kernel<<<(unsigned)((total + 255) / 256), 256, 0, s>>>(x, x_plane_stride, g, d, d_plane_stride, gd, total);
  count_launch();
}

__global__ void __launch_bounds__(256) planar_maxpool_kernel(const __nv_bfloat16* __restrict__ x, int64_t xs, UcGeom gi, __nv_bfloat16* __restrict__ y,
                                                             int64_t ys, UcGeom go, const __nv_bfloat16* __restrict__ xlo,
                                                             __nv_bfloat16* __restrict__ ylo) {
  const int frame = blockIdx.x, chunk = blockIdx.y;
  const int n = frame / go.T, t = frame - n * go.T;
  const int lane = threadIdx.x & 31, warp = threadIdx.x >> 5, nwarps = blockDim.x >> 5;
  const __nv_bfloat16* xc = x + (int64_t)chunk * xs + uc_flat(gi, n, t, 0, 0) * 8;
  const __nv_bfloat16* xlc = xlo ? xlo + (int64_t)chunk * xs + uc_flat(gi, n, t, 0, 0) * 8 : nullptr;
  __nv_bfloat16* yc = y + (int64_t)chunk * ys + uc_flat(go, n, t, 0, 0) * 8;
  __nv_bfloat16* ylc = ylo ? ylo + (int64_t)chunk * ys + uc_flat(go, n, t, 0, 0) * 8 : nullptr;
  auto ld = [&](int pos, float* f) {
    unpack8(*reinterpret_cast<const uint4*>(xc + pos * 8), f);
    if (xlc) {
      float fl[8];
      unpack8(*reinterpret_cast<const uint4*>(xlc + pos * 8), fl);
#pragma unroll
      for (int e = 0; e < 8; ++e) f[e] += fl[e];
    }
  };
  const int nseg = (gi.W + 31) >> 5;
  const int npairs = go.H * nseg;
  for (int pair = warp; pair < npairs; pair += nwarps) {
    const int h = pair / nseg, seg = pair - h * nseg;
    const int c = seg * 32 + lane;
    float mv[8], ml[8];
#pragma unroll
    for (int e = 0; e < 8; ++e) mv[e] = ml[e] = -INFINITY;
    const bool extra_left = lane == 0 && seg > 0;
#pragma unroll
    for (int dh = 0; dh < 3; ++dh) {
      const int hi = 2 * h - 1 + dh;
      if ((unsigned)hi >= (unsigned)gi.H) continue;
      float f[8];
      if (c < gi.W) {
        ld(hi * gi.RW + c, f);
#pragma unroll
        for (int e = 0; e < 8; ++e) mv[e] = fmaxf(mv[e], f[e]);
      }
      if (extra_left) {
        ld(hi * gi.RW + c - 1, f);
#pragma unroll
        for (int e = 0; e < 8; ++e) ml[e] = fmaxf(ml[e], f[e]);
      }
    }
    const int w = seg * 16 + lane;
    float m[8];
#pragma unroll
    for (int e = 0; e < 8; ++e) {
      const float a = __shfl_sync(0xffffffffu, mv[e], (2 * lane) & 31);
      const float b = __shfl_sync(0xffffffffu, mv[e], (2 * lane + 1) & 31);
      const float cl = __shfl_sync(0xffffffffu, mv[e], (2 * lane - 1) & 31);
      const float left = lane == 0 ? ml[e] : cl;
      m[e] = fmaxf(fmaxf(a, b), left);
    }
    if (lane < 16 && w < go.W) {
      const int dst = (h * go.RW + w) * 8;
      const uint4 hi4 = pack8(m);
      *reinterpret_cast<uint4*>(yc + dst) = hi4;
      if (ylc) {
        float hf[8], lo[8];
        unpack8(hi4, hf);
#pragma unroll
        for (int e = 0; e < 8; ++e) lo[e] = m[e] - hf[e];
        *reinterpret_cast<uint4*>(ylc + dst) = pack8(lo);
      }
    }
  }
}
__global__ void __launch_bounds__(256) planar_maxpool_bf16_kernel(const __nv_bfloat16* __restrict__ x, int64_t xs, UcGeom gi,
                                                                  __nv_bfloat16* __restrict__ y, int64_t ys, UcGeom go) {
  const int frame = blockIdx.x, chunk = blockIdx.y;
  const int n = frame / go.T, t = frame - n * go.T;
  const int lane = threadIdx.x & 31, warp = threadIdx.x >> 5, nwarps = blockDim.x >> 5;
  const uint4* xc = reinterpret_cast<const uint4*>(x + (int64_t)chunk * xs + uc_flat(gi, n, t, 0, 0) * 8);
  uint4* yc = reinterpret_cast<uint4*>(y + (int64_t)chunk * ys + uc_flat(go, n, t, 0, 0) * 8);
  const uint32_t NINF2 = 0xFF80FF80u;
  auto mx4 = [](uint4 a, uint4 b) {
    uint4 r;
    __nv_bfloat162 t0 = __hmax2(*reinterpret_cast<__nv_bfloat162*>(&a.x), *reinterpret_cast<__nv_bfloat162*>(&b.x));
    __nv_bfloat162 t1 = __hmax2(*reinterpret_cast<__nv_bfloat162*>(&a.y), *reinterpret_cast<__nv_bfloat162*>(&b.y));
    __nv_bfloat162 t2 = __hmax2(*reinterpret_cast<__nv_bfloat162*>(&a.z), *reinterpret_cast<__nv_bfloat162*>(&b.z));
    __nv_bfloat162 t3 = __hmax2(*reinterpret_cast<__nv_bfloat162*>(&a.w), *reinterpret_cast<__nv_bfloat162*>(&b.w));
    r.x = *reinterpret_cast<uint32_t*>(&t0); r.y = *reinterpret_cast<uint32_t*>(&t1);
    r.z = *reinterpret_cast<uint32_t*>(&t2); r.w = *reinterpret_cast<uint32_t*>(&t3);
    return r;
  };
  const int nseg = (gi.W + 31) >> 5;
  const int npairs = go.H * nseg;
  for (int pair = warp; pair < npairs; pair += nwarps) {
    const int h = pair / nseg, seg = pair - h * nseg;
    const int c = seg * 32 + lane;
    uint4 mv = make_uint4(NINF2, NINF2, NINF2, NINF2), ml = mv;
    const bool extra_left = lane == 0 && seg > 0;
#pragma unroll
    for (int dh = 0; dh < 3; ++dh) {
      const int hi = 2 * h - 1 + dh;
      if ((unsigned)hi >= (unsigned)gi.H) continue;
      if (c < gi.W) mv = mx4(mv, xc[hi * gi.RW + c]);
      if (extra_left) ml = mx4(ml, xc[hi * gi.RW + c - 1]);
    }
    const int sa = (2 * lane) & 31, sb = (2 * lane + 1) & 31, sc = (2 * lane - 1) & 31;
    uint4 a, b, cl;
    a.x = __shfl_sync(0xffffffffu, mv.x, sa); a.y = __shfl_sync(0xffffffffu, mv.y, sa);
    a.z = __shfl_sync(0xffffffffu, mv.z, sa); a.w = __shfl_sync(0xffffffffu, mv.w, sa);
    b.x = __shfl_sync(0xffffffffu, mv.x, sb); b.y = __shfl_sync(0xffffffffu, mv.y, sb);
    b.z = __shfl_sync(0xffffffffu, mv.z, sb); b.w = __shfl_sync(0xffffffffu, mv.w, sb);
    cl.x = __shfl_sync(0xffffffffu, mv.x, sc); cl.y = __shfl_sync(0xffffffffu, mv.y, sc);
    cl.z = __shfl_sync(0xffffffffu, mv.z, sc); cl.w = __shfl_sync(0xffffffffu, mv.w, sc);
    if (lane == 0) cl = ml;
    const int w = seg * 16 + lane;
    if (lane < 16 && w < go.W) yc[h * go.RW + w] = mx4(mx4(a, b), cl);
  }
}

__global__ void __launch_bounds__(192) planar_maxpool_direct_kernel(const __nv_bfloat16* __restrict__ x, int64_t xs, UcGeom gi,
                                                                    __nv_bfloat16* __restrict__ y, int64_t ys, UcGeom go) {
  const int frame = blockIdx.x, chunk = blockIdx.y;
  const int n = frame / go.T, t = frame - n * go.T;
  const uint4* xc = reinterpret_cast<const uint4*>(x + (int64_t)chunk * xs + uc_flat(gi, n, t, 0, 0) * 8);
  uint4* yc = reinterpret_cast<uint4*>(y + (int64_t)chunk * ys + uc_flat(go, n, t, 0, 0) * 8);
  const uint32_t NINF2 = 0xFF80FF80u;
  const int total = go.H * go.W;
  for (int o = threadIdx.x; o < total; o += blockDim.x) {
    const int h = o / go.W, w = o - h * go.W;
    uint4 v[9];
#pragma unroll
    for (int dh = 0; dh < 3; ++dh)
#pragma unroll
      for (int dw = 0; dw < 3; ++dw) {
        const int hi = 2 * h - 1 + dh, wi = 2 * w - 1 + dw;
        v[dh * 3 + dw] = ((unsigned)hi < (unsigned)gi.H && (unsigned)wi < (unsigned)gi.W) ? xc[hi * gi.RW + wi] : make_uint4(NINF2, NINF2, NINF2, NINF2);
      }
    uint32_t* m = reinterpret_cast<uint32_t*>(&v[0]);
#pragma unroll
    for (int k = 1; k < 9; ++k) {
      const uint32_t* r = reinterpret_cast<const uint32_t*>(&v[k]);
#pragma unroll
      for (int e = 0; e < 4; ++e) {
        const __nv_bfloat162 q = __hmax2(*reinterpret_cast<const __nv_bfloat162*>(&m[e]), *reinterpret_cast<const __nv_bfloat162*>(&r[e]));
        m[e] = *reinterpret_cast<const uint32_t*>(&q);
      }
    }
    yc[h * go.RW + w] = v[0];
  }
}

void launch_planar_maxpool(const __nv_bfloat16* x, int64_t x_plane_stride, UcGeom gi, __nv_bfloat16* y, int64_t y_plane_stride, UcGeom go,
                           int C, cudaStream_t s, const __nv_bfloat16* xlo, __nv_bfloat16* ylo) {
  const int frames = go.N * go.T;
  if (frames == 0 || go.H * go.W == 0) return;
  static const bool warp_rows = getenv("LSD_POOL_WARP_ROWS") != nullptr;
  if (!xlo && !ylo && !warp_rows) planar_maxpool_direct_kernel<<<dim3((unsigned)frames, (unsigned)(C / 8)), 192, 0, s>>>(x, x_plane_stride, gi, y, y_plane_stride, go);
  else if (!xlo && !ylo) planar_maxpool_bf16_kernel<<<dim3((unsigned)frames, (unsigned)(C / 8)), 256, 0, s>>>(x, x_plane_stride, gi, y, y_plane_stride, go);
  else planar_maxpool_kernel<<<dim3((unsigned)frames, (unsigned)(C / 8)), 256, 0, s>>>(x, x_plane_stride, gi, y, y_plane_stride, go, xlo, ylo);
  count_launch();
}

constexpr int VR_ROWS = 8;
template <typename T> __device__ __forceinline__ float vr_norm(float x) { return x; }
template <> __device__ __forceinline__ float vr_norm<uint8_t>(float x) { return x / 255.0f; }
template <typename T, int LAYOUT>
__global__ void __launch_bounds__(256) video_rows_kernel(const T* __restrict__ video, const float* __restrict__ lapw,
                                                         __nv_bfloat16* __restrict__ xs, __nv_bfloat16* __restrict__ xl, int64_t set_stride,
                                                         UcGeom g, int Tn, int H, int W, int bands, float inv_div) {
  extern __shared__ float tile[];
  const int tx = threadIdx.x, ty = threadIdx.y;
  const int WP2 = W + 2, per_c = (VR_ROWS + 2) * WP2;
  const int band = blockIdx.x % bands;
  const int nt = blockIdx.x / bands;
  const int t = nt % Tn, n = nt / Tn;
  const int h0 = band * VR_ROWS;
  __shared__ float lw[81];
  if (ty == 0 && tx < 27) { lw[tx] = lapw[tx]; lw[tx + 27] = lapw[tx + 27]; lw[tx + 54] = lapw[tx + 54]; }
  for (int r = ty; r < VR_ROWS + 2; r += 8) {
    const int hh = h0 + r - 1;
    const bool rin = (unsigned)hh < (unsigned)H;
    if (LAYOUT == 0) {
      const T* rp0 = video + ((((int64_t)n * 3) * Tn + t) * H + (rin ? hh : 0)) * W;
      const int64_t cstride = (int64_t)Tn * H * W;
      for (int col0 = 0; col0 < WP2; col0 += 128) {
        float vals[3][4];
#pragma unroll
        for (int c = 0; c < 3; ++c)
#pragma unroll
          for (int k = 0; k < 4; ++k) {
            const int ww = col0 + tx + 32 * k - 1;
            vals[c][k] = (rin && (unsigned)ww < (unsigned)W) ? vr_norm<T>((float)rp0[c * cstride + ww]) : 0.f;
          }
#pragma unroll
        for (int c = 0; c < 3; ++c)
#pragma unroll
          for (int k = 0; k < 4; ++k) {
            const int col = col0 + tx + 32 * k;
            if (col < WP2) tile[c * per_c + r * WP2 + col] = vals[c][k];
          }
      }
    } else {
      const T* rp = video + (((int64_t)nt * H + (rin ? hh : 0)) * W) * 3;
      for (int e0 = 0; e0 < 3 * WP2; e0 += 256) {
        float vals[8];
#pragma unroll
        for (int k = 0; k < 8; ++k) {
          const int e = e0 + tx + 32 * k, col = e / 3, c = e - col * 3, ww = col - 1;
          vals[k] = (rin && e < 3 * WP2 && (unsigned)ww < (unsigned)W) ? vr_norm<T>((float)rp[ww * 3 + c]) : 0.f;
        }
#pragma unroll
        for (int k = 0; k < 8; ++k) {
          const int e = e0 + tx + 32 * k, col = e / 3, c = e - col * 3;
          if (e < 3 * WP2) tile[c * per_c + r * WP2 + col] = vals[k];
        }
      }
    }
  }
// ... 431 lines not shown
```

multimodal-lip-sync-deepfake-detection-system_b200/csrc/umma_conv.cuh:

```cuda
#pragma once
#include <cuda_bf16.h>
#include <cuda_runtime.h>
#include <stdint.h>

namespace lsd {

constexpr int UC_MAX_BANDS = 16;
constexpr int UC_MAX_TAPS = 12;
constexpr int UC_MAX_GROUPS = 6;

struct UcBand {
  const __nv_bfloat16* base;
  int64_t plane_stride;
  int64_t chunk_stride;
  int start;
  int len_extra;
  int ntaps;
  int tap_begin;
  int toeplitz;
  int rel[UC_MAX_TAPS];
};

struct UcGroup {
  int band_begin, band_end;
  int k16;
  int taps_total;
  int64_t w_off;
  int64_t slice_stride;
};

enum UcOut { UC_Y_NONE = 0, UC_Y_PLAIN = 1, UC_Y_PARITY = 2, UC_Y_PARITY_H = 3, UC_Y_POOL = 4 };

struct UcGeom {
  int N, T, H, W;
  int TS, ot, HP, oh, RW, ow, SL;
  int64_t P_total;
  uint32_t mSL, mRW, mTS;
  int sSL, sRW, sTS;
};

inline void uc_magic(uint32_t d, uint32_t& m, int& s) {
  s = 0;
  while (((uint64_t)1 << s) < d) ++s;
  m = (uint32_t)((((uint64_t)1 << (31 + s)) / d) + 1);
}

struct alignas(16) UcStageDesc {
  uint64_t a_src;
  uint64_t w_src;
  uint64_t chunk_stride_b;
  uint64_t plane_stride_b;
  uint64_t w_slice_stride_b;
  uint32_t bytesA;
  uint32_t w_copy_bytes;
  uint32_t w_dst_step;
  uint32_t w_src_step;
  uint32_t tx_bytes;
  uint32_t counts;
};
static_assert(sizeof(UcStageDesc) == 64, "UcStageDesc must be 64 bytes");

struct UmmaConvP {
  const __nv_bfloat16* w;
  const float* bias;
  const __nv_bfloat16* res;
  const __nv_bfloat16* res_lo;
  int64_t res_plane_stride;
  const float* res32;
  int res32_ld;
  __nv_bfloat16* y;
  __nv_bfloat16* ylo;
  int64_t y_plane_stride, y_set_stride;
  int y_mode;
  float* y32;
  int y32_ld;
  int y32_outer_stride, y32_row_off;
  int act;
  int Cout;
  int MT, stages, ngroups, nbands;
  int issuers;
  int nbuf;
  long long* dbg;
  unsigned* tile_ctr;
  const UcStageDesc* prog;
  int nst_tile;
  int skip;
  int kpack;
  uint32_t a_stage_bytes, w_stage_bytes, tmem_cols;
  uint32_t pool_ring, pool_mR;
  int pool_sR;
  int cta2;
  UcGeom g;
  UcGeom g2;
  UcGroup groups[UC_MAX_GROUPS];
  UcBand bands[UC_MAX_BANDS];
};

size_t umma_conv_smem_bytes(const UmmaConvP& p);
int umma_conv_stage_desc_bytes();
size_t umma_conv_extra_smem_bytes(const UmmaConvP& p);
size_t umma_conv_pool_smem_bytes(int MT);
void umma_conv_build_program(const UmmaConvP& p, UcStageDesc* out);
const char* umma_conv_config_error(const UmmaConvP& p);
void launch_umma_conv(const UmmaConvP& p, int n_slices, cudaStream_t s, int num_sms, int max_ctas = 0);
cudaError_t umma_conv_device_init();
cudaError_t video_rows_device_init();

void launch_pack_planar(const float* x, __nv_bfloat16* y, int64_t plane_stride, int64_t set_stride, UcGeom g, UcGeom g2, int C,
                        int parity, cudaStream_t s);
void launch_unpack_planar(const __nv_bfloat16* x, int64_t plane_stride, UcGeom g, int C, float* y, int ld, cudaStream_t s);
void launch_unpack_planar_any(const __nv_bfloat16* x, const __nv_bfloat16* xlo, int64_t plane_stride, int64_t set_stride, UcGeom g, int C, int sets,
                              int Hf, int Wf, float* y, cudaStream_t s);
void launch_planar_mean(const __nv_bfloat16* x, int64_t plane_stride, UcGeom g, int C, float* y, int ld, int per_window, cudaStream_t s);
void launch_planar_delta(const __nv_bfloat16* x, int64_t x_plane_stride, UcGeom g, __nv_bfloat16* d, int64_t d_plane_stride, UcGeom gd,
                         int C, cudaStream_t s);
void launch_planar_maxpool(const __nv_bfloat16* x, int64_t x_plane_stride, UcGeom gi, __nv_bfloat16* y, int64_t y_plane_stride, UcGeom go,
                           int C, cudaStream_t s, const __nv_bfloat16* xlo = nullptr, __nv_bfloat16* ylo = nullptr);

void launch_video_rows(const void* video, int dtype, int layout, const float* lapw, const float* lapw_host, __nv_bfloat16* xs, __nv_bfloat16* xl,
                       int64_t set_stride, UcGeom g, int H, int W, cudaStream_t s, int num_sms, const int32_t* starts = nullptr, int n_frames = 0);
bool video_rows_bulk_ok(const void* video, int dtype, int layout, int W);

inline UcGeom make_geom_ex(int N, int T, int H, int W, int tpad, int oh, int hp_extra, int ow, int wp_extra) {
  UcGeom g;
  g.N = N; g.T = T; g.H = H; g.W = W;
  g.TS = T + tpad; g.ot = tpad;
  g.HP = H + oh + hp_extra; g.oh = oh;
  g.RW = W + ow + wp_extra; g.ow = ow;
  g.SL = g.HP * g.RW;
  g.P_total = ((int64_t)N * g.TS + tpad) * g.SL;
  uc_magic((uint32_t)g.SL, g.mSL, g.sSL);
  uc_magic((uint32_t)g.RW, g.mRW, g.sRW);
  uc_magic((uint32_t)g.TS, g.mTS, g.sTS);
  return g;
}
inline UcGeom make_geom(int N, int T, int H, int W) { return make_geom_ex(N, T, H, W, 1, 1, 0, 1, 0); }
inline UcGeom make_geom_rows(int rows) { return make_geom_ex(1, 1, 1, rows, 0, 0, 0, 0, 0); }

}
```

Baseline: 24710.

## Fold small spatial maps of layer3/layer4 into per-position conv slices

For residual stages whose spatial map is tiny (H*W ≤ 36), activations are stored as one set per spatial position and each output position becomes its own slice. Each slice gets its own stage program that issues only the in-bounds taps. The (batch,time) axis becomes the GEMM row dimension, and the kernel's main loop batches temporal taps per stage. This aims to stop wasting MMA rows and loads on padded halo positions in the late, small-map layers. In exchange it adds many more slices and larger per-launch parameters, and the stage-program arena grows.

```diff
diff --git a/multimodal-lip-sync-deepfake-detection-system_b200/csrc/bf16_path.cu b/multimodal-lip-sync-deepfake-detection-system_b200/csrc/bf16_path.cu
--- a/multimodal-lip-sync-deepfake-detection-system_b200/csrc/bf16_path.cu
+++ b/multimodal-lip-sync-deepfake-detection-system_b200/csrc/bf16_path.cu
@@ -9,9 +9,11 @@
 #include <cuda_fp16.h>
 
 #include <algorithm>
+#include <array>
 #include <cstdio>
 #include <cstdlib>
 #include <cstring>
+#include <functional>
 
 using namespace lsd;
 using namespace lsdfw;
@@ -175,6 +177,37 @@
     while (w.size() % 64) w.push_back(0);
     h->blayers[name] = L;
   }
+  void add_fold(const std::string& name, const std::string& key, const std::string& ds_key, int ntile) {
+    const ConvP& c = h->convs.at(key);
+    if (c.kt != 3 || c.kh != 3 || c.kw != 3 || c.Cout % ntile) return;
+    BLayer L;
+    L.Cout = c.Cout;
+    L.ntile = ntile;
+    BGroup g;
+    g.Cin = c.Cin;
+    g.taps_total = 27;
+    g.k16 = c.Cin / 16;
+    for (int b = 0; b < 3; ++b)
+      for (int d = 0; d < 3; ++d) {
+        BBand band{b * 3 + d, {}};
+        for (int a = 0; a < 3; ++a) band.taps.push_back(BTap{(a * 3 + b) * 3 + d, a - 1, b - 1, d - 1});
+        g.bands.push_back(band);
+      }
+    pack_group(g, c, ntile);
+    L.groups.push_back(g);
+    L.bias_off = bias.size();
+    for (int i = 0; i < c.Cout; ++i) bias.push_back(f32[c.shift_off + i]);
+    if (!ds_key.empty()) {
+      const ConvP& d = h->convs.at(ds_key);
+      BGroup gd = make_group(d, 1, 1);
+      gd.src = 1;
+      pack_group(gd, d, ntile);
+      L.groups.push_back(gd);
+      for (int i = 0; i < c.Cout; ++i) bias[L.bias_off + i] += f32[d.shift_off + i];
+    }
+    while (w.size() % 64) w.push_back(0);
+    h->blayers[name] = L;
+  }
   void add_split(const std::string& name, const std::string& key, int ntile) {
     const ConvP& c = h->convs.at(key);
     BLayer L;
@@ -215,8 +248,14 @@
   return b;
 }
 
+bool fold_route(int H, int W) {
+  static const bool off = LSD_ENV("LSD_FOLD") && atoi(LSD_ENV("LSD_FOLD")) == 0;
+  return !off && H * W <= 36;
+}
+
 struct BPlan {
   Shapes s;
+  bool fold3 = false, fold4 = false;
   Plan f32;
   std::map<std::string, PBuf> pb;
   size_t planar_begin = 0, planar_end = 0;
@@ -264,10 +303,13 @@
   P.addp("l1a", 64, 1, g1);
   P.addp("y1", 64, 4, g2);
   P.addp("l2a", 128, 1, g2);
-  P.addp("y2", 128, 4, g3);
-  P.addp("l3a", 256, 1, g3);
-  P.addp("y3", 256, 4, g4);
-  P.addp("l4a", 256, 1, g4);
+  P.fold3 = fold_route(s.H3, s.W3);
+  P.fold4 = fold_route(s.H4, s.W4);
+  const UcGeom gr = make_geom_ex(Bn, Tn, 1, 1, 1, 0, 0, 0, 0);
+  if (P.fold3) P.addp("y2", 128, s.H2 * s.W2, gr); else P.addp("y2", 128, 4, g3);
+  if (P.fold3) P.addp("l3a", 256, s.H3 * s.W3, gr); else P.addp("l3a", 256, 1, g3);
+  if (P.fold4) P.addp("y3", 256, s.H3 * s.W3, gr); else P.addp("y3", 256, 4, g4);
+  if (P.fold4) P.addp("l4a", 256, s.H4 * s.W4, gr); else P.addp("l4a", 256, 1, g4);
   P.addp("y4", 256, 1, g4);
   P.addp("art_a", 128, 1, g4);
   P.addp("art_b", 64, 1, g4);
@@ -339,6 +381,39 @@
   int res32_ld = 0;
 };
 
+int stage_program(const BCtx& c, const std::string& name, UmmaConvP& p, const std::function<void(std::vector<UcStageDesc>&)>& build,
+                  std::initializer_list<uint64_t> salt = {}) {
+  uint64_t hkey = 1469598103934665603ull;
+  for (uint64_t v : salt) { hkey ^= v; hkey *= 1099511628211ull; hkey ^= hkey >> 29; }
+  static_assert(sizeof(UmmaConvP) % 8 == 0, "UmmaConvP is hashed in 8-byte words");
+  const uint64_t* pw = reinterpret_cast<const uint64_t*>(&p);
+  for (size_t i = 0; i < sizeof(p) / 8; ++i) { hkey ^= pw[i]; hkey *= 1099511628211ull; hkey ^= hkey >> 29; }
+  auto it = c.h->prog_cache.find(hkey);
+  if (it == c.h->prog_cache.end()) {
+    std::vector<UcStageDesc> host;
+    build(host);
+    const size_t bytes = host.size() * sizeof(UcStageDesc);
+    if (!c.h->prog_arena) {
+      c.h->prog_cap = 64u << 20;
+      if (cudaMalloc(&c.h->prog_arena, c.h->prog_cap) != cudaSuccess) return lsd_fail(c.h, LSD_ERR_CUDA, "stage-program arena allocation failed");
+      c.h->prog_cursor = 0;
+    }
+    if (c.h->prog_cursor + bytes > c.h->prog_cap) {
+      cudaDeviceSynchronize();
+      c.h->prog_cache.clear();
+      c.h->prog_cursor = 0;
+      ++c.h->generation;
+    }
+    char* dst = c.h->prog_arena + c.h->prog_cursor;
+    cudaError_t e = cudaMemcpy(dst, host.data(), bytes, cudaMemcpyHostToDevice);
+    if (e != cudaSuccess) return lsd_fail(c.h, LSD_ERR_CUDA, "%s: stage program upload: %s", name.c_str(), cudaGetErrorString(e));
+    c.h->prog_cursor += (bytes + 255) & ~size_t(255);
+    it = c.h->prog_cache.emplace(hkey, dst).first;
+  }
+  p.prog = reinterpret_cast<const UcStageDesc*>(it->second);
+  return 0;
+}
+
 int run_umma(const BCtx& c, const std::string& name, const UArgs& a) {
   const BLayer& L = c.h->blayers.at(name);
   const UcGeom& og = a.og;
@@ -358,6 +433,7 @@
     p.y = c.org(*a.yp) + (int64_t)a.y_plane_off * a.yp->plane_stride;
     p.y_plane_stride = a.yp->plane_stride; p.y_set_stride = a.yp->set_stride;
     p.g2 = a.yp->g;
+    p.ymap_W = og.W;
     if (a.yp_lo) p.ylo = c.org(*a.yp_lo) + (int64_t)a.y_plane_off * a.yp_lo->plane_stride;
   }
   if (a.y32) {
@@ -470,35 +546,8 @@
   if (L.groups[0].toeplitz) { const ConvP& cp = c.h->convs.at(name); kflop = (double)cp.kt * cp.kh * cp.kw * cp.Cin; }
   if (const char* e = getenv("LSD_UMMA_SKIP")) p.skip = atoi(e);
   if (const char* why = umma_conv_config_error(p)) return lsd_fail(c.h, LSD_ERR_UNSUPPORTED, "%s: %s", name.c_str(), why);
-  {
-    uint64_t hkey = 1469598103934665603ull;
-    static_assert(sizeof(UmmaConvP) % 8 == 0, "UmmaConvP is hashed in 8-byte words");
-    const uint64_t* pw = reinterpret_cast<const uint64_t*>(&p);
-    for (size_t i = 0; i < sizeof(p) / 8; ++i) { hkey ^= pw[i]; hkey *= 1099511628211ull; hkey ^= hkey >> 29; }
-    auto it = c.h->prog_cache.find(hkey);
-    if (it == c.h->prog_cache.end()) {
-      const size_t bytes = (size_t)p.nst_tile * sizeof(UcStageDesc);
-      if (!c.h->prog_arena) {
-        c.h->prog_cap = 16u << 20;
-        if (cudaMalloc(&c.h->prog_arena, c.h->prog_cap) != cudaSuccess) return lsd_fail(c.h, LSD_ERR_CUDA, "stage-program arena allocation failed");
-        c.h->prog_cursor = 0;
-      }
-      if (c.h->prog_cursor + bytes > c.h->prog_cap) {
-        cudaDeviceSynchronize();
-        c.h->prog_cache.clear();
-        c.h->prog_cursor = 0;
-        ++c.h->generation;
-      }
-      std::vector<UcStageDesc> host((size_t)p.nst_tile);
-      umma_conv_build_program(p, host.data());
-      char* dst = c.h->prog_arena + c.h->prog_cursor;
-      cudaError_t e = cudaMemcpy(dst, host.data(), bytes, cudaMemcpyHostToDevice);
-      if (e != cudaSuccess) return lsd_fail(c.h, LSD_ERR_CUDA, "%s: stage program upload: %s", name.c_str(), cudaGetErrorString(e));
-      c.h->prog_cursor += (bytes + 255) & ~size_t(255);
-      it = c.h->prog_cache.emplace(hkey, dst).first;
-    }
-    p.prog = reinterpret_cast<const UcStageDesc*>(it->second);
-  }
+  if (int rc = stage_program(c, name, p, [&](std::vector<UcStageDesc>& v) { v.resize((size_t)p.nst_tile); umma_conv_build_program(p, v.data()); }))
+    return rc;
   static const bool dyn_tiles = LSD_ENV("LSD_UMMA_DYNAMIC") != nullptr;
   if (dyn_tiles && p.y_mode != UC_Y_POOL && !p.cta2) {
     constexpr int kMaxLayers = 512;
@@ -798,6 +847,128 @@
   return 0;
 }
 
+int run_umma_fold(const BCtx& c, const std::string& name, const PBuf& x, int Hi, int Wi, int stride, const PBuf* x_ds, int Hd, int Wd,
+                  int Ho, int Wo, const PBuf& yp, int y_mode) {
+  const auto itL = c.h->blayers.find(name + "#fold");
+  if (itL == c.h->blayers.end()) return lsd_fail(c.h, LSD_ERR_UNSUPPORTED, "%s: no weights packed for the folded route (LSD_FOLD=0)", name.c_str());
+  const BLayer& L = itL->second;
+  const UcGeom& og = x.g;
+  if (og.P_total >= ((int64_t)1 << 31) - 1024) return lsd_fail(c.h, LSD_ERR_SHAPE, "%s: more than 2^31 rows in one launch (reduce the batch)", name.c_str());
+  if ((L.groups.size() == 2) != (x_ds != nullptr) || x.sets != Hi * Wi || (x_ds && x_ds->sets != Hd * Wd))
+    return lsd_fail(c.h, LSD_ERR_ARG, "%s: folded inputs do not match the layer", name.c_str());
+  UmmaConvP p;
+  memset(&p, 0, sizeof(p));
+  p.w = reinterpret_cast<const __nv_bfloat16*>(c.h->barena);
+  p.bias = c.h->bbias + L.bias_off;
+  p.Cout = L.ntile;
+  p.act = ACT_RELU;
+  p.g = og;
+  p.fold = 1;
+  p.y_mode = y_mode;
+  p.y = c.org(yp);
+  p.y_plane_stride = yp.plane_stride; p.y_set_stride = yp.set_stride;
+  p.g2 = yp.g;
+  p.ymap_W = Wo;
+  int mt = 2;
+  if (const char* e = LSD_ENV("LSD_FOLD_MT")) mt = std::max(1, std::min(4, atoi(e)));
+  p.MT = (int)std::max<int64_t>(1, std::min<int64_t>(mt, (og.P_total + 127) / 128));
+  p.nbuf = 1;
+  p.issuers = std::min(p.MT, 4);
+  uint32_t cols = 32;
+  while ((int)cols < p.MT * L.ntile) cols *= 2;
+  p.tmem_cols = cols;
+  const int S = p.MT * 128;
+  const PBuf* srcs[2] = {&x, x_ds};
+  p.ngroups = (int)L.groups.size();
+  p.nbands = p.ngroups;
+  int max_a = 0, max_w = 0, min_k16 = 1 << 30;
+  for (int gi = 0; gi < p.ngroups; ++gi) {
+    const BGroup& G = L.groups[gi];
+    UcGroup& ug = p.groups[gi];
+    ug.band_begin = gi; ug.band_end = gi + 1;
+    ug.k16 = G.k16; ug.taps_total = G.taps_total;
+    ug.w_off = (int64_t)G.w_off; ug.slice_stride = (int64_t)G.slice_stride;
+    UcBand& ub = p.bands[gi];
+    const PBuf& src = *srcs[gi];
+    ub.base = c.org(src);
+    ub.plane_stride = src.plane_stride;
+    ub.chunk_stride = 2 * src.plane_stride;
+    ub.ntaps = gi == 0 ? 3 : 1;
+    ub.start = gi == 0 ? -1 : 0;
+    ub.len_extra = gi == 0 ? 2 : 0;
+    for (int j = 0; j < ub.ntaps; ++j) ub.rel[j] = j;
+    if ((int64_t)8 > src.origin) return lsd_fail(c.h, LSD_ERR_UNSUPPORTED, "%s: guard zone too small", name.c_str());
+    max_a = std::max(max_a, 2 * (S + ub.len_extra) * 16);
+    max_w = std::max(max_w, ub.ntaps * L.ntile * 32);
+    min_k16 = std::min(min_k16, G.k16);
+  }
+  p.kpack = std::max(1, std::min(std::min(8, min_k16), (48 * 1024) / (max_a + max_w)));
+  p.a_stage_bytes = ((uint32_t)(max_a * p.kpack) + 127u) & ~127u;
+  p.w_stage_bytes = (uint32_t)(max_w * p.kpack);
+  const int cslices = L.Cout / L.ntile;
+  std::vector<std::array<int, 3>> pos;
+  auto inb = [&](int o, int k, int n) { const int i = stride * o + k - 1; return i >= 0 && i < n; };
+  for (int ho = 0; ho < Ho; ++ho)
+    for (int wo = 0; wo < Wo; ++wo) {
+      int nq = 0;
+      for (int kh = 0; kh < 3; ++kh)
+        for (int kw = 0; kw < 3; ++kw) nq += inb(ho, kh, Hi) && inb(wo, kw, Wi);
+      pos.push_back({-nq, ho, wo});
+    }
+  std::stable_sort(pos.begin(), pos.end(), [](const std::array<int, 3>& a, const std::array<int, 3>& b) { return a[0] < b[0]; });
+  const int nslices = (int)pos.size() * cslices;
+  if (nslices > UC_MAX_FSLICES || Ho > 255 || Wo > 255) return lsd_fail(c.h, LSD_ERR_UNSUPPORTED, "%s: map too large for the folded route", name.c_str());
+  auto chunks = [&](int k16) { return (k16 + p.kpack - 1) / p.kpack; };
+  int off = 0;
+  for (int i = 0; i < nslices; ++i) {
+    const auto& q = pos[(size_t)(i / cslices)];
+    const int nst = -q[0] * chunks(p.groups[0].k16) + (x_ds ? chunks(p.groups[1].k16) : 0);
+    p.fslice[i] = UcFoldSlice{(uint16_t)off, (uint16_t)nst, (uint8_t)q[1], (uint8_t)q[2], (uint8_t)(i % cslices), 0};
+    p.nst_tile = std::max(p.nst_tile, nst);
+    off += nst;
+  }
+  if (off > 65535) return lsd_fail(c.h, LSD_ERR_UNSUPPORTED, "%s: folded stage programs too long", name.c_str());
+  const uint32_t stage = p.a_stage_bytes + p.w_stage_bytes;
+  const uint32_t prog_bytes = (uint32_t)p.nst_tile * (uint32_t)umma_conv_stage_desc_bytes();
+  const uint32_t budget = 211u * 1024u - (uint32_t)umma_conv_extra_smem_bytes(p);
+  if (prog_bytes + 2 * stage > budget) return lsd_fail(c.h, LSD_ERR_UNSUPPORTED, "%s: stage program of %u bytes does not fit", name.c_str(), prog_bytes);
+  p.stages = std::max(2, std::min((int)((budget - prog_bytes) / stage), 8));
+  if (const char* e = getenv("LSD_UMMA_SKIP")) p.skip = atoi(e);
+  if (const char* why = umma_conv_config_error(p)) return lsd_fail(c.h, LSD_ERR_UNSUPPORTED, "%s: %s", name.c_str(), why);
+  auto build = [&](std::vector<UcStageDesc>& v) {
+    for (int i = 0; i < nslices; ++i) {
+      const UcFoldSlice& f = p.fslice[i];
+      for (int kh = 0; kh < 3; ++kh)
+        for (int kw = 0; kw < 3; ++kw) {
+          if (!inb(f.h, kh, Hi) || !inb(f.w, kw, Wi)) continue;
+          UcBand bq = p.bands[0];
+          bq.base = c.org(x) + (int64_t)((stride * f.h + kh - 1) * Wi + stride * f.w + kw - 1) * x.set_stride;
+          bq.tap_begin = (kh * 3 + kw) * 3;
+          for (int c0 = 0; c0 < p.groups[0].k16; c0 += p.kpack) v.push_back(umma_conv_stage(p, p.groups[0], bq, 0, c0, f.col));
+        }
+      if (x_ds) {
+        UcBand bd = p.bands[1];
+        bd.base = c.org(*x_ds) + (int64_t)(2 * f.h * Wd + 2 * f.w) * x_ds->set_stride;
+        for (int c0 = 0; c0 < p.groups[1].k16; c0 += p.kpack) v.push_back(umma_conv_stage(p, p.groups[1], bd, 1, c0, f.col));
+      }
+    }
+  };
+  if (int rc = stage_program(c, name + "#fold", p, build, {(uint64_t)Hi, (uint64_t)Wi, (uint64_t)stride, (uint64_t)Hd, (uint64_t)Wd,
+                                                          (uint64_t)x.set_stride, (uint64_t)(x_ds ? x_ds->set_stride : 0)})) return rc;
+  double kflop = 0;
+  for (const BGroup& G : L.groups) kflop += (double)G.taps_total * G.Cin;
+  c.h->prof.begin(c.st, 2.0 * (double)og.N * og.T * Ho * Wo * L.Cout * kflop, 2);
+  launch_umma_conv(p, nslices, c.st, c.h->num_sms, c.max_ctas);
+  c.h->prof.end(c.st);
+  return 0;
+}
+
+int res_stage_fold(const BCtx& b, const std::string& p, const PBuf& x, int Hi, int Wi, const PBuf& mid, int Ho, int Wo, const PBuf& y, int y_mode) {
+  int rc = 0;
+  if ((rc = run_umma_fold(b, p + ".conv1", x, Hi, Wi, 2, nullptr, 0, 0, Ho, Wo, mid, UC_Y_FOLD))) return rc;
+  return run_umma_fold(b, p + ".conv2", mid, Ho, Wo, 1, &x, Hi, Wi, Ho, Wo, y, y_mode);
+}
+
 }
 
 static int pack_tok_fused(lsd_handle* h, const std::vector<float>& f32) {
@@ -913,6 +1084,12 @@
     P.add(p + ".conv1", p + ".conv1", s, s, "", nt, false, l >= 2, pairs);
     P.ds_sh = 2; P.ds_sw = 2;
     P.add(p + ".conv2", p + ".conv2", 1, 1, l == 1 ? "" : p + ".downsample", nt, false, false, pairs);
+    if (l >= 3) {
+      int fnt = 128;
+      if (const char* e = LSD_ENV("LSD_FOLD_NT")) fnt = atoi(e) == 256 ? 256 : 128;
+      P.add_fold(p + ".conv1#fold", p + ".conv1", "", fnt);
+      P.add_fold(p + ".conv2#fold", p + ".conv2", p + ".downsample", fnt);
+    }
   }
   P.add_toeplitz("visual_encoder.stem", "visual_encoder.stem", 8, 0, false, cta2);
   for (int cv = 0; cv < 2; ++cv) {
@@ -1323,11 +1500,15 @@
     } else if ((rc = res_stage_umma(b, "visual_encoder.layer1", x1, pb["l1a"], pb["y1"], false, UC_Y_PARITY))) return rc;
   }
   g_tl.mark(st, "M:layer1");
-  if ((rc = res_stage_umma(b, "visual_encoder.layer2", pb["y1"], pb["l2a"], pb["y2"], true, UC_Y_PARITY))) return rc;
+  if ((rc = res_stage_umma(b, "visual_encoder.layer2", pb["y1"], pb["l2a"], pb["y2"], true, P.fold3 ? UC_Y_FOLD : UC_Y_PARITY))) return rc;
   g_tl.mark(st, "M:layer2");
-  if ((rc = res_stage_umma(b, "visual_encoder.layer3", pb["y2"], pb["l3a"], pb["y3"], true, UC_Y_PARITY))) return rc;
+  if (P.fold3) rc = res_stage_fold(b, "visual_encoder.layer3", pb["y2"], s.H2, s.W2, pb["l3a"], s.H3, s.W3, pb["y3"], UC_Y_FOLD);
+  else rc = res_stage_umma(b, "visual_encoder.layer3", pb["y2"], pb["l3a"], pb["y3"], true, P.fold4 ? UC_Y_FOLD : UC_Y_PARITY);
+  if (rc) return rc;
   g_tl.mark(st, "M:layer3");
-  if ((rc = res_stage_umma(b, "visual_encoder.layer4", pb["y3"], pb["l4a"], pb["y4"], true, UC_Y_PLAIN))) return rc;
+  if (P.fold4) rc = res_stage_fold(b, "visual_encoder.layer4", pb["y3"], s.H3, s.W3, pb["l4a"], s.H4, s.W4, pb["y4"], UC_Y_MAP);
+  else rc = res_stage_umma(b, "visual_encoder.layer4", pb["y3"], pb["l4a"], pb["y4"], true, UC_Y_PLAIN);
+  if (rc) return rc;
   g_tl.mark(st, "M:layer4");
   b.max_ctas = 0;
   const PBuf& y4 = pb["y4"];
diff --git a/multimodal-lip-sync-deepfake-detection-system_b200/csrc/umma_conv.cu b/multimodal-lip-sync-deepfake-detection-system_b200/csrc/umma_conv.cu
--- a/multimodal-lip-sync-deepfake-detection-system_b200/csrc/umma_conv.cu
+++ b/multimodal-lip-sync-deepfake-detection-system_b200/csrc/umma_conv.cu
@@ -87,7 +87,10 @@
   const uint32_t stage_bytes = p.a_stage_bytes + p.w_stage_bytes;
   const int num_tiles = (int)((p.g.P_total + S - 1) / S);
   const uint32_t cta_rank = CTA2 ? cluster_ctarank() : 0u;
-  const int slice = blockIdx.y, ch0 = slice * p.Cout;
+  const int slice = blockIdx.y;
+  const bool fold = p.fold != 0;
+  const int nst = fold ? (int)p.fslice[slice].nst : p.nst_tile;
+  const int ch0 = (fold ? (int)p.fslice[slice].col : slice) * p.Cout;
   const int bcols = CTA2 ? p.Cout >> 1 : p.Cout;
   const uint32_t buf_cols = (uint32_t)(p.MT * p.Cout);
   int tile_first = blockIdx.x, tile_step = gridDim.x, tile_end = num_tiles;
@@ -144,9 +147,9 @@
   }
   UcStageDesc* prog = reinterpret_cast<UcStageDesc*>(smem + (size_t)p.stages * stage_bytes);
   {
-    const uint4* psrc = reinterpret_cast<const uint4*>(p.prog);
+    const uint4* psrc = reinterpret_cast<const uint4*>(p.prog + (fold ? (int)p.fslice[slice].prog_off : 0));
     uint4* pdst = reinterpret_cast<uint4*>(prog);
-    for (int i = tid; i < p.nst_tile * 4; i += UC_THREADS) pdst[i] = psrc[i];
+    for (int i = tid; i < nst * 4; i += UC_THREADS) pdst[i] = psrc[i];
   }
   tc_fence_before();
   if constexpr (CTA2) cluster_sync_all();
@@ -171,11 +174,11 @@
     const uint64_t slice64 = CTA2 ? (uint64_t)cta_rank : (uint64_t)slice;
     int k = 0;
     int seq = 0;
-    for (int tile = tile_start; tile >= 0; k += p.nst_tile) {
+    for (int tile = tile_start; tile >= 0; k += nst) {
       unsigned claim = 0;
       if (dyn && warp == 0 && lane == 0) claim = atomicAdd(p.tile_ctr + slice, 1u);
       const uint64_t p0_bytes = (uint64_t)tile_p0(tile) * 16u;
-      for (int si = ((warp - k) % npw + npw) % npw; si < p.nst_tile; si += npw) {
+      for (int si = ((warp - k) % npw + npw) % npw; si < nst; si += npw) {
         const int kk = k + si;
         const int stage = kk % p.stages;
         const uint32_t ph = (uint32_t)(kk / p.stages) & 1u;
@@ -226,7 +229,7 @@
         int stage = 0;
         uint32_t ph = 0;
         for (int tile = tile_first; tile < tile_end; tile += tile_step)
-          for (int si = 0; si < p.nst_tile; ++si) {
+          for (int si = 0; si < nst; ++si) {
             mbar_wait(&full_bar[stage], ph);
             if (lane == 0) mbar_arrive_cluster(mapa_shared(smem_u32(&full2_bar[stage]), 0u));
             __syncwarp();
@@ -265,55 +268,51 @@
         }
         acc = 1u;
       }
-      for (int gi = 0; gi < p.ngroups; ++gi) {
-        const int k16 = p.groups[gi].k16, b0 = p.groups[gi].band_begin, b1 = p.groups[gi].band_end;
-        for (int c0 = 0; c0 < k16; c0 += p.kpack) {
-          const int nc = min(p.kpack, k16 - c0);
-          for (int b = b0; b < b1; ++b) {
-            const UcBand& bd = p.bands[b];
-            const int ntaps = bd.ntaps;
-            const uint32_t unitsA = (uint32_t)(S + bd.len_extra);
-            const uint32_t a_lbo = (bd.toeplitz ? 1u : unitsA) << 16;
-            const uint32_t a_chunk = bd.toeplitz ? 2u : 2u * unitsA;
-            const uint32_t w_chunk = (uint32_t)ntaps * tap_w;
-            mbar_wait(&full_bar[stage], ph);
-            if constexpr (CTA2) mbar_wait_cluster(&full2_bar[stage], ph);
-            tc_fence_after();
-            if (dbg && warp == UC_MMA_WARP0 && lane == 0 && acc == 0 && lt == 0) p.dbg[2] = clock64();
-            if (dbg && warp == UC_MMA_WARP0 && lane == 0 && lt == 0 && dbg_it < 24) p.dbg[8 + dbg_it++] = clock64();
-            const uint32_t sa = ((smem_base + (uint32_t)stage * stage_bytes) >> 4) + (uint32_t)mt_lo * 128u;
-            const uint32_t sw = ((smem_base + (uint32_t)stage * stage_bytes + p.a_stage_bytes) >> 4) | b_lbo;
-            if (ntaps == 1) {
-              uint32_t at = (sa | a_lbo) + (uint32_t)bd.rel[0], wj = sw;
+      for (int si = 0; si < nst; ++si) {
+        const uint32_t counts = __shfl_sync(0xffffffffu, prog[si].counts, 0);
+        const int b = (int)((counts >> 16) & 0xffu), nc = (int)(counts >> 24);
+        const UcBand& bd = p.bands[b];
+        const int ntaps = bd.ntaps;
+        const uint32_t unitsA = (uint32_t)(S + bd.len_extra);
+        const uint32_t a_lbo = (bd.toeplitz ? 1u : unitsA) << 16;
+        const uint32_t a_chunk = bd.toeplitz ? 2u : 2u * unitsA;
+        const uint32_t w_chunk = (uint32_t)ntaps * tap_w;
+        mbar_wait(&full_bar[stage], ph);
+        if constexpr (CTA2) mbar_wait_cluster(&full2_bar[stage], ph);
+        tc_fence_after();
+        if (dbg && warp == UC_MMA_WARP0 && lane == 0 && acc == 0 && lt == 0) p.dbg[2] = clock64();
+        if (dbg && warp == UC_MMA_WARP0 && lane == 0 && lt == 0 && dbg_it < 24) p.dbg[8 + dbg_it++] = clock64();
+        const uint32_t sa = ((smem_base + (uint32_t)stage * stage_bytes) >> 4) + (uint32_t)mt_lo * 128u;
+        const uint32_t sw = ((smem_base + (uint32_t)stage * stage_bytes + p.a_stage_bytes) >> 4) | b_lbo;
+        if (ntaps == 1) {
+          uint32_t at = (sa | a_lbo) + (uint32_t)bd.rel[0], wj = sw;
 #pragma unroll 1
-              for (int j = 0; j < nc; ++j, at += a_chunk, wj += w_chunk) {
-                const uint64_t da = desc_hi64 | (uint64_t)at, db = desc_hi64 | (uint64_t)wj;
-                UC_MMA(tb, da, db, idesc, acc, leader);
-                if (mt_n > 1) UC_MMA(tb + (uint32_t)p.Cout, da + 128u, db, idesc, acc, leader);
-                acc = 1u;
-              }
-            } else
-            for (int j = 0; j < nc; ++j) {
-              const uint32_t aj = (sa + (uint32_t)j * a_chunk) | a_lbo;
-              uint32_t wj = sw + (uint32_t)j * w_chunk;
+          for (int j = 0; j < nc; ++j, at += a_chunk, wj += w_chunk) {
+            const uint64_t da = desc_hi64 | (uint64_t)at, db = desc_hi64 | (uint64_t)wj;
+            UC_MMA(tb, da, db, idesc, acc, leader);
+            if (mt_n > 1) UC_MMA(tb + (uint32_t)p.Cout, da + 128u, db, idesc, acc, leader);
+            acc = 1u;
+          }
+        } else
+        for (int j = 0; j < nc; ++j) {
+          const uint32_t aj = (sa + (uint32_t)j * a_chunk) | a_lbo;
+          uint32_t wj = sw + (uint32_t)j * w_chunk;
 #pragma unroll 1
-              for (int tp = 0; tp < ntaps; ++tp) {
-                const uint32_t at = aj + (uint32_t)bd.rel[tp];
-                const uint64_t da = desc_hi64 | (uint64_t)at, db = desc_hi64 | (uint64_t)wj;
-                UC_MMA(tb, da, db, idesc, acc, leader);
-                if (mt_n > 1) UC_MMA(tb + (uint32_t)p.Cout, da + 128u, db, idesc, acc, leader);
-                if (mt_n > 2) {
-                  UC_MMA(tb + 2u * (uint32_t)p.Cout, da + 256u, db, idesc, acc, leader);
-                  UC_MMA(tb + 3u * (uint32_t)p.Cout, da + 384u, db, idesc, acc, leader);
-                }
-                acc = 1u;
-                wj += tap_w;
-              }
+          for (int tp = 0; tp < ntaps; ++tp) {
+            const uint32_t at = aj + (uint32_t)bd.rel[tp];
+            const uint64_t da = desc_hi64 | (uint64_t)at, db = desc_hi64 | (uint64_t)wj;
+            UC_MMA(tb, da, db, idesc, acc, leader);
+            if (mt_n > 1) UC_MMA(tb + (uint32_t)p.Cout, da + 128u, db, idesc, acc, leader);
+            if (mt_n > 2) {
+              UC_MMA(tb + 2u * (uint32_t)p.Cout, da + 256u, db, idesc, acc, leader);
+              UC_MMA(tb + 3u * (uint32_t)p.Cout, da + 384u, db, idesc, acc, leader);
             }
-            UC_COMMIT(&empty_bar[stage], leader);
-            if (++stage == p.stages) { stage = 0; ph ^= 1u; }
+            acc = 1u;
+            wj += tap_w;
           }
         }
+        UC_COMMIT(&empty_bar[stage], leader);
+        if (++stage == p.stages) { stage = 0; ph ^= 1u; }
       }
       UC_COMMIT(&tfull_bar[buf], leader);
       if (dbg && warp == UC_MMA_WARP0 && lane == 0 && lt == 0) p.dbg[3] = clock64();
@@ -341,6 +340,7 @@
         const int64_t P = P0 + (int64_t)m * 128 + rowt;
         int n = 0, t = 0, h = 0, w = 0;
         const bool valid = (p.skip & 8) ? true : uc_decode(p.g, P, n, t, h, w);
+        if (fold) { h = p.fslice[slice].h; w = p.fslice[slice].w; }
         const bool inrange = P < p.g.P_total;
         const int64_t outer = valid ? ((int64_t)n * p.g.T + t) * p.g.H + h : 0;
         int64_t dst = P * 8;
@@ -348,6 +348,10 @@
           dst = (int64_t)((h & 1) * 2 + (w & 1)) * p.y_set_stride + uc_flat(p.g2, n, t, h >> 1, w >> 1) * 8;
         else if (valid && p.y_mode == UC_Y_PARITY_H)
           dst = (int64_t)((h & 1) * 2) * p.y_set_stride + uc_flat(p.g2, n, t, h >> 1, w) * 8;
+        else if (valid && p.y_mode == UC_Y_FOLD)
+          dst = (int64_t)(h * p.ymap_W + w) * p.y_set_stride + uc_flat(p.g2, n, t, 0, 0) * 8;
+        else if (valid && p.y_mode == UC_Y_MAP)
+          dst = uc_flat(p.g2, n, t, h, w) * 8;
         const bool store_planar = ((p.y_mode == UC_Y_PLAIN && inrange) || (p.y_mode >= UC_Y_PARITY && valid)) && !(p.skip & 4);
         const int cbeg = split_c ? half * (p.Cout >> 1) : 0, cend = split_c ? cbeg + (p.Cout >> 1) : p.Cout;
         if constexpr (POOL) {
@@ -540,37 +544,38 @@
   if (dbg && tid == 0) { p.dbg[6] = clock64(); p.dbg[7] = num_tiles; }
 }
 
-void umma_conv_build_program(const UmmaConvP& p, UcStageDesc* out) {
+UcStageDesc umma_conv_stage(const UmmaConvP& p, const UcGroup& g, const UcBand& bd, int band, int c0, int col) {
   const int S = p.MT * 128;
   const int bcols = p.cta2 ? p.Cout / 2 : p.Cout;
+  const int nc = std::min(p.kpack, g.k16 - c0);
+  UcStageDesc d;
+  const uint32_t bytesW = (uint32_t)bd.ntaps * (uint32_t)bcols * 32u;
+  d.bytesA = bd.toeplitz ? (uint32_t)(S + bd.len_extra + 1 + 2 * (nc - 1)) * 16u : (uint32_t)(S + bd.len_extra) * 16u;
+  uint32_t n_a = bd.toeplitz ? 1u : 2u * (uint32_t)nc;
+  const bool w_merged = bd.ntaps == g.taps_total;
+  uint32_t n_w = w_merged ? 1u : (uint32_t)nc;
+  d.w_copy_bytes = w_merged ? (uint32_t)nc * bytesW : bytesW;
+  d.w_dst_step = bytesW;
+  if (p.skip & 1) n_a = 0;
+  if (p.skip & 2) n_w = 0;
+  d.tx_bytes = n_a * d.bytesA + (n_w ? (uint32_t)nc * bytesW : 0u);
+  d.a_src = reinterpret_cast<uint64_t>(bd.base + (int64_t)c0 * bd.chunk_stride + (int64_t)bd.start * 8);
+  d.chunk_stride_b = (uint64_t)bd.chunk_stride * 2u;
+  d.plane_stride_b = (uint64_t)bd.plane_stride * 2u;
+  d.w_src = reinterpret_cast<uint64_t>(p.w + g.w_off + (col > 0 ? (int64_t)col * g.slice_stride : 0) +
+                                       ((int64_t)c0 * g.taps_total + bd.tap_begin) * (int64_t)bcols * 16);
+  d.w_slice_stride_b = col >= 0 ? 0u : (uint64_t)g.slice_stride * 2u;
+  d.w_src_step = (uint32_t)g.taps_total * (uint32_t)bcols * 32u;
+  d.counts = n_a | (n_w << 8) | ((uint32_t)band << 16) | ((uint32_t)nc << 24);
+  return d;
+}
+
+void umma_conv_build_program(const UmmaConvP& p, UcStageDesc* out) {
   int s = 0;
   for (int gi = 0; gi < p.ngroups; ++gi) {
     const UcGroup& g = p.groups[gi];
-    for (int c0 = 0; c0 < g.k16; c0 += p.kpack) {
-      const int nc = std::min(p.kpack, g.k16 - c0);
-      for (int b = g.band_begin; b < g.band_end; ++b, ++s) {
-        const UcBand& bd = p.bands[b];
-        UcStageDesc d;
-        const uint32_t bytesW = (uint32_t)bd.ntaps * (uint32_t)bcols * 32u;
-        d.bytesA = bd.toeplitz ? (uint32_t)(S + bd.len_extra + 1 + 2 * (nc - 1)) * 16u : (uint32_t)(S + bd.len_extra) * 16u;
-        uint32_t n_a = bd.toeplitz ? 1u : 2u * (uint32_t)nc;
-        const bool w_merged = (g.band_end - g.band_begin) == 1;
-        uint32_t n_w = w_merged ? 1u : (uint32_t)nc;
-        d.w_copy_bytes = w_merged ? (uint32_t)nc * bytesW : bytesW;
-        d.w_dst_step = bytesW;
-        if (p.skip & 1) n_a = 0;
-        if (p.skip & 2) n_w = 0;
-        d.tx_bytes = n_a * d.bytesA + (n_w ? (uint32_t)nc * bytesW : 0u);
-        d.a_src = reinterpret_cast<uint64_t>(bd.base + (int64_t)c0 * bd.chunk_stride + (int64_t)bd.start * 8);
-        d.chunk_stride_b = (uint64_t)bd.chunk_stride * 2u;
-        d.plane_stride_b = (uint64_t)bd.plane_stride * 2u;
-        d.w_src = reinterpret_cast<uint64_t>(p.w + g.w_off + ((int64_t)c0 * g.taps_total + bd.tap_begin) * (int64_t)bcols * 16);
-        d.w_slice_stride_b = (uint64_t)g.slice_stride * 2u;
-        d.w_src_step = (uint32_t)g.taps_total * (uint32_t)bcols * 32u;
-        d.counts = n_a | (n_w << 8) | ((uint32_t)b << 16) | ((uint32_t)nc << 24);
-        out[s] = d;
-      }
-    }
+    for (int c0 = 0; c0 < g.k16; c0 += p.kpack)
+      for (int b = g.band_begin; b < g.band_end; ++b) out[s++] = umma_conv_stage(p, g, p.bands[b], b, c0);
   }
 }
 
@@ -596,6 +601,8 @@
   if (p.res && p.res32) return "bf16 and fp32 residuals are mutually exclusive";
   if (uc_is_generic(p) && (p.Cout & 63)) return "the generic epilogue needs a column slice that is a multiple of 64";
   if (p.MT / p.issuers > 4 || p.MT % p.issuers) return "unsupported M-tiles per issuing warp";
+  if (p.fold && (uc_is_generic(p) || p.cta2 || p.tile_ctr || p.y_mode == UC_Y_POOL || p.res || p.MT > 4))
+    return "folded convolutions need the lean epilogue, no residual, single CTAs, at most 4 M-tiles and the static tile walk";
   if (p.cta2 && (uc_is_generic(p) || p.y_mode == UC_Y_POOL || (p.Cout & 31) || p.tile_ctr)) return "CTA pairs need the lean epilogue, a multiple of 32 columns and the static tile walk";
   if (p.y_mode == UC_Y_POOL) {
     if (uc_is_generic(p) || p.res || p.act != ACT_RELU || p.Cout != 64 || p.tile_ctr) return "fused max-pool needs the lean epilogue, ReLU, 64 columns and the static tile walk";
@@ -640,6 +647,7 @@
     count_launch();
     return;
   }
+  if (p.fold) gx = tiles;
   if (generic) umma_conv_kernel<1><<<dim3(gx, n_slices), UC_THREADS, umma_conv_smem_bytes(p), s>>>(p);
   else if (p.y_mode == UC_Y_POOL) umma_conv_kernel<2><<<dim3(gx, n_slices), UC_THREADS, umma_conv_smem_bytes(p), s>>>(p);
   else umma_conv_kernel<0><<<dim3(gx, n_slices), UC_THREADS, umma_conv_smem_bytes(p), s>>>(p);
@@ -714,6 +722,7 @@
   const int n = (int)(r / g.T);
   int64_t src;
   if (sets == 1) src = uc_flat(g, n, t, h, w) * 8;
+  else if (g.SL == 1 && sets == Hf * Wf) src = (int64_t)(h * Wf + w) * set_stride + uc_flat(g, n, t, 0, 0) * 8;
   else if (Wf == g.W) src = (int64_t)((h & 1) * 2) * set_stride + uc_flat(g, n, t, h >> 1, w) * 8;
   else src = (int64_t)((h & 1) * 2 + (w & 1)) * set_stride + uc_flat(g, n, t, h >> 1, w >> 1) * 8;
   src += (int64_t)chunk * plane_stride;
diff --git a/multimodal-lip-sync-deepfake-detection-system_b200/csrc/umma_conv.cuh b/multimodal-lip-sync-deepfake-detection-system_b200/csrc/umma_conv.cuh
--- a/multimodal-lip-sync-deepfake-detection-system_b200/csrc/umma_conv.cuh
+++ b/multimodal-lip-sync-deepfake-detection-system_b200/csrc/umma_conv.cuh
@@ -29,7 +29,14 @@
   int64_t slice_stride;
 };
 
-enum UcOut { UC_Y_NONE = 0, UC_Y_PLAIN = 1, UC_Y_PARITY = 2, UC_Y_PARITY_H = 3, UC_Y_POOL = 4 };
+enum UcOut { UC_Y_NONE = 0, UC_Y_PLAIN = 1, UC_Y_PARITY = 2, UC_Y_PARITY_H = 3, UC_Y_POOL = 4, UC_Y_FOLD = 5, UC_Y_MAP = 6 };
+
+constexpr int UC_MAX_FSLICES = 96;
+struct UcFoldSlice {
+  uint16_t prog_off, nst;
+  uint8_t h, w;
+  uint8_t col, pad_;
+};
 
 struct UcGeom {
   int N, T, H, W;
@@ -94,6 +101,9 @@
   UcGeom g2;
   UcGroup groups[UC_MAX_GROUPS];
   UcBand bands[UC_MAX_BANDS];
+  int ymap_W;
+  int fold;
+  UcFoldSlice fslice[UC_MAX_FSLICES];
 };
 
 size_t umma_conv_smem_bytes(const UmmaConvP& p);
@@ -101,6 +111,7 @@
 size_t umma_conv_extra_smem_bytes(const UmmaConvP& p);
 size_t umma_conv_pool_smem_bytes(int MT);
 void umma_conv_build_program(const UmmaConvP& p, UcStageDesc* out);
+UcStageDesc umma_conv_stage(const UmmaConvP& p, const UcGroup& g, const UcBand& bd, int band, int c0, int col = -1);
 const char* umma_conv_config_error(const UmmaConvP& p);
 void launch_umma_conv(const UmmaConvP& p, int n_slices, cudaStream_t s, int num_sms, int max_ctas = 0);
 cudaError_t umma_conv_device_init();
```

After: 25780, median of 6. +4.3%, better.
